# ecmwf-ifs/ectrans

Hardware: AMD Instinct MI355X
Metric: dir+inv transform-pairs/sec, TCo1279 137L x 10 fields; spectral-norm rel-error (higher is better)
Workload: dtype f64

## Files before the change

ectrans_amd/csrc/ectrans_mi.hip:

```cpp
#include <atomic>
#include <chrono>
#include <cmath>
#include <cstdarg>
#include <cstdio>
#include <map>
#include <memory>
#include <string>
#include <vector>

#include <fcntl.h>
#include <sys/mman.h>
#include <sys/stat.h>
#include <unistd.h>

#include "../../include/ectrans_mi.h"
#include "emi_kernels.h"
#include "emi_setup.h"
#include <dlfcn.h>

struct EmiRoctx {
  int (*push)(const char *) = nullptr;
  int (*pop)() = nullptr;
  bool tried = false;
  void load() {
    tried = true;
#ifndef EMI_CPU_EMU
    const char *e = getenv("EMI_ROCTX");
    if (e && atoi(e) == 0) return;
    void *h = dlopen("librocprofiler-sdk-roctx.so", RTLD_NOW | RTLD_GLOBAL);
    if (!h) h = dlopen("librocprofiler-sdk-roctx.so.1", RTLD_NOW | RTLD_GLOBAL);
    if (!h) h = dlopen("libroctx64.so", RTLD_NOW | RTLD_GLOBAL);
    if (!h) return;
    push = (int (*)(const char *))dlsym(h, "roctxRangePushA");
    pop = (int (*)())dlsym(h, "roctxRangePop");
    if (!push || !pop) push = nullptr, pop = nullptr;
#endif
  }
};
static EmiRoctx g_roctx;
struct EmiRange {
  bool on;
  explicit EmiRange(const char *label) {
    if (!g_roctx.tried) g_roctx.load();
    on = g_roctx.push != nullptr;
    if (on) g_roctx.push(label);
  }
  ~EmiRange() {
    if (on) g_roctx.pop();
  }
};
extern "C" int emi_roctx_active(void) {
  if (!g_roctx.tried) g_roctx.load();
  return g_roctx.push != nullptr;
}
static const char *const EMI_LBL_SETUP = "SETUP_TRANS    - Setup ecTrans handle", *const EMI_LBL_SULEG = "SULEG          - Comp. of Leg. poly.",
                         *const EMI_LBL_INV = "INV_TRANS      - Inverse transform", *const EMI_LBL_DIR = "DIR_TRANS      - Direct transform",
                         *const EMI_LBL_LTINV = "LTINV_CTL      - Inv. Legendre transform", *const EMI_LBL_LTDIR = "LTDIR_CTL      - Dir. Legendre transform",
                         *const EMI_LBL_FTDIR = "FTDIR_CTL      - Dir. Fourier transform", *const EMI_LBL_FTINV = "FTINV_CTL      - Inv. Fourier transform",
                         *const EMI_LBL_TRMTOL = "LTINV_CTL      - M to L transposition", *const EMI_LBL_TRLTOM = "LTDIR_CTL      - L to M transposition";

#ifdef EMI_CPU_EMU
thread_local EmuCtx *emu_ctx = nullptr;
#endif

static char g_err[1024] = "";
void emi_set_error(const char *fmt, ...) {
  va_list ap;
  va_start(ap, fmt);
  vsnprintf(g_err, sizeof(g_err), fmt, ap);
  va_end(ap);
}
extern "C" const char *emi_last_error(void) { return g_err; }

#define EMI_FAIL(code, ...)     \
  do {                          \
    emi_set_error(__VA_ARGS__); \
    return (code);              \
  } while (0)

#ifndef EMI_CPU_EMU
static void (*g_oom_hook)() = nullptr;
int emi_dev_malloc(void **p, size_t bytes) {
  if (hipMalloc(p, bytes ? bytes : 16) == hipSuccess) return 0;
  (void)hipGetLastError();
  if (g_oom_hook) g_oom_hook();
  EMI_CHECK(hipMalloc(p, bytes ? bytes : 16));
  return 0;
}
int emi_dev_free(void *p) {
  if (p) EMI_CHECK(hipFree(p));
  return 0;
}
int emi_dev_memset(void *p, int v, size_t bytes, emi_stream_t s) {
  EMI_CHECK(hipMemsetAsync(p, v, bytes, s));
  return 0;
}
int emi_h2d(void *d, const void *s, size_t b, emi_stream_t st) {
  EMI_CHECK(hipMemcpyAsync(d, s, b, hipMemcpyHostToDevice, st));
  return 0;
}
int emi_d2h(void *d, const void *s, size_t b, emi_stream_t st) {
  EMI_CHECK(hipMemcpyAsync(d, s, b, hipMemcpyDeviceToHost, st));
  return 0;
}
int emi_d2d(void *d, const void *s, size_t b, emi_stream_t st) {
  EMI_CHECK(hipMemcpyAsync(d, s, b, hipMemcpyDeviceToDevice, st));
  return 0;
}
int emi_stream_sync(emi_stream_t s) {
  EMI_CHECK(hipStreamSynchronize(s));
  return 0;
}
int emi_mem_info(size_t *f, size_t *t) {
  EMI_CHECK(hipMemGetInfo(f, t));
  return 0;
}
#else
int emi_dev_malloc(void **p, size_t bytes) {
  *p = aligned_alloc(64, ((bytes ? bytes : 16) + 63) / 64 * 64);
  return *p ? 0 : -1;
}
int emi_dev_free(void *p) {
  free(p);
  return 0;
}
int emi_dev_memset(void *p, int v, size_t bytes, emi_stream_t) {
  memset(p, v, bytes);
  return 0;
}
int emi_h2d(void *d, const void *s, size_t b, emi_stream_t) {
  memcpy(d, s, b);
  return 0;
}
int emi_d2h(void *d, const void *s, size_t b, emi_stream_t) {
  memcpy(d, s, b);
  return 0;
}
int emi_d2d(void *d, const void *s, size_t b, emi_stream_t) {
  memmove(d, s, b);
  return 0;
}
int emi_stream_sync(emi_stream_t) { return 0; }
int emi_mem_info(size_t *f, size_t *t) {
  *f = (size_t)8 << 30;
  *t = (size_t)8 << 30;
  return 0;
}
#endif

#include "emi_stage.h"
#ifndef EMI_CPU_EMU
static const bool g_oom_hook_set = (g_oom_hook = emi_stage::trim, true);
#endif

extern "C" int emi_ptr_space(const void *p) {
#ifdef EMI_CPU_EMU
  (void)p;
  return EMI_MEM_HOST;
#else
  if (!p) return EMI_MEM_HOST;
  hipPointerAttribute_t at;
  if (hipPointerGetAttributes(&at, p) != hipSuccess) {
    (void)hipGetLastError();
    return EMI_MEM_HOST;
  }
  return (at.type == hipMemoryTypeDevice || at.type == hipMemoryTypeManaged || at.type == hipMemoryTypeArray) ? EMI_MEM_DEVICE : EMI_MEM_HOST;
#endif
}
static int agree_on_mixed_arrays(const char *who, int ndev, int nhost);
static int resolve_space(const char *who, int mem_space, std::initializer_list<const void *> arrays, int *out, bool collective = false) {
  if (mem_space == EMI_MEM_HOST || mem_space == EMI_MEM_DEVICE) {
    *out = mem_space;
    return 0;
  }
  if (mem_space != EMI_MEM_AUTO) EMI_FAIL(EMI_ERR_ARG, "%s: mem_space = %d (EMI_MEM_HOST, EMI_MEM_DEVICE or EMI_MEM_AUTO)", who, mem_space);
  int ndev = 0, nhost = 0;
  for (const void *q : arrays)
    if (q) (emi_ptr_space(q) == EMI_MEM_DEVICE ? ndev : nhost)++;
  if (collective) {
    if (agree_on_mixed_arrays(who, ndev, nhost)) return EMI_ERR_ARG;
  } else if (ndev && nhost) {
    EMI_FAIL(EMI_ERR_ARG, "%s: %d ARRAYS OF THE CALL ARE IN DEVICE MEMORY AND %d IN HOST MEMORY (all of them must live in one place)", who, ndev, nhost);
  }
  *out = ndev ? EMI_MEM_DEVICE : EMI_MEM_HOST;
  return 0;
}

template <class T>
static int upload(const std::vector<T> &h, T **d) {
  void *p = nullptr;
  if (emi_dev_malloc(&p, h.size() * sizeof(T))) return -1;
  if ((!h.empty() && emi_h2d(p, h.data(), h.size() * sizeof(T), 0)) || emi_stream_sync(0)) {
    emi_dev_free(p);
    return -1;
  }
  *d = (T *)p;
  return 0;
}
struct DevAllocs {
  std::vector<void *> list;
  DevAllocs() = default;
  DevAllocs(const DevAllocs &) = delete;
  DevAllocs &operator=(const DevAllocs &) = delete;
  ~DevAllocs() {
    for (void *p : list) emi_dev_free(p);
  }
  int alloc(void **p, size_t bytes) {
    if (emi_dev_malloc(p, bytes)) return -1;
    list.push_back(*p);
    return 0;
  }
};
template <class T, class F>
static int upload(DevAllocs &owner, const std::vector<T> &h, F *field) {
  T *d = nullptr;
  if (upload(h, &d)) return -1;
  owner.list.push_back(d);
  *field = d;
  return 0;
}

#define EMI_LAUNCH_P(esz, kern, grid, block, lds, st, ...)                     \
  do {                                                                         \
    if ((esz) == 8) {                                                          \
      typedef double RT;                                                       \
      EMI_LAUNCH(emi_f64::kern, grid, block, lds, st, __VA_ARGS__);            \
    } else {                                                                   \
      typedef float RT;                                                        \
      EMI_LAUNCH(emi_f32::kern, grid, block, lds, st, __VA_ARGS__);            \
    }                                                                          \
  } while (0)

struct FftClass {
  int nthr = 0, fbk = 0;
  int hot = 0;
  int r16 = 0;
  int split = 0;
  int mr = 0;
  int gmem = 0;
  long long gm_elems = 0;
  std::vector<int> lats;
  int *d_lats = nullptr;
  FftRowDev *d_rows = nullptr;
  size_t lds = 0;
};
struct LegMaps {
  int2 *d_inv = nullptr, *d_dir = nullptr, *d_inv_wide = nullptr, *d_dir_wide = nullptr;
  long long n_inv = 0, n_dir = 0, n_inv_wide = 0, n_dir_wide = 0;
};

struct Plan {
  Plan() = default;
  Plan(const Plan &) = delete;
  Plan &operator=(const Plan &) = delete;
  ~Plan();
  int nsmax = 0, ndgl = 0, ndgnh = 0;
  bool reduced = false;
  bool ldll = false, shiftll = false;
  bool lam = false;
  int lam_n = 0, kdgux = 0;
  double exwn = 0.0, eywn = 0.0;
  std::vector<int> kntmp;
  std::vector<int> l_kntmp, nesm0;
  LamDev lamdev{};
  int lam_nthr = 0;
  size_t lam_lds = 0;
  double ra = 6371229.0;
  std::vector<int> nloen, nmen, ndglu, procm;
  std::vector<int> latlo;
  std::vector<double> rmu, rw, racthe, cos2;
  int ngptotg = 0, nspec2g = 0;
  int nproc = 1, me = 0;
  int nprv = 1, mev = 0;
  std::vector<int> vlat;
  int vfirst(int w, int v) const { return nprv > 1 ? vlat[(size_t)w * nprv + v] : latlo[w]; }
  int vlast(int w, int v) const { return nprv > 1 ? vlat[(size_t)w * nprv + v + 1] : latlo[w + 1]; }
  long long vpoints(int w, int v) const {
    long long c = 0;
    for (int j = vfirst(w, v); j < vlast(w, v); j++) c += nloen[j];
    return c;
  }
  long long voffset(int v) const {
    long long c = 0;
    for (int j = latlo[me]; j < vfirst(me, v); j++) c += nloen[j];
    return c;
  }
  int nump = 0, nlat = 0, lat0 = 0;
  int ngptot = 0, nspec2 = 0;
  std::vector<int> mval, nasm0;
  std::vector<int> l_nmen, l_gpoff, l_fbase;
  std::vector<int> wbase, wrows, ldp, ldk, lattile_pref, ktile_pref, lbase;
  std::vector<long long> offS, offA, offTS, offTA;
  long long frows = 0, lrows = 0, wrows_total = 0, p_elems = 0, pt_elems = 0;
  std::vector<long long> leg_rows, leg_disp, fft_rows, fft_disp;
  EmiGeomDev g{};
  DevAllocs dev_allocs;
  int esz = 8;
  char *d_P = nullptr, *d_PT = nullptr;
  std::vector<FftPlanDev> fplans;
  std::vector<int> planid;
  FftTabDev ftab{};
  std::vector<FftClass> fclass;
  std::map<int, LegMaps> legmaps;
  char *d_W = nullptr, *d_FBL = nullptr, *d_FBF = nullptr;
  size_t cap_W = 0, cap_FBL = 0, cap_FBF = 0;
  void *d_desc = nullptr;
  size_t cap_desc = 0;
  char *d_fftscr = nullptr;
  size_t cap_fftscr = 0;
#ifndef EMI_CPU_EMU
  hipEvent_t ev_done = nullptr;
#endif
  bool ev_valid = false;
};

Plan::~Plan() {
#ifndef EMI_CPU_EMU
  if (ev_done) (void)hipEventDestroy(ev_done);
#endif
  emi_dev_free(d_W);
  emi_dev_free(d_FBL);
  if (d_FBF != d_FBL) emi_dev_free(d_FBF);
  emi_dev_free(d_desc);
  emi_dev_free(d_fftscr);
}

static int roundup(int a, int b) { return (a + b - 1) / b * b; }
static int test_paths() {
  const char *e = getenv("EMI_TEST_PATHS");
  return e ? atoi(e) : 0;
}
static_assert(LG_LDS_BYTES_DIR + 1024 + 64 <= 65536, "k_leg_dir: stage image + epilogue table above 64 KiB, two workgroups per CU no longer fit");
static size_t leg_dir_lds_bytes(const Plan &P) {
  return (size_t)LG_LDS_BYTES_DIR * P.esz / 8 + 1024 + 64;
}

static int plan_begin(Plan &P, emi_stream_t st) {
#ifndef EMI_CPU_EMU
  if (P.ev_valid) EMI_CHECK(hipStreamWaitEvent(st, P.ev_done, 0));
#else
  (void)P;
  (void)st;
#endif
  return 0;
}
static int plan_end(Plan &P, emi_stream_t st) {
#ifndef EMI_CPU_EMU
  if (!P.ev_done) EMI_CHECK(hipEventCreateWithFlags(&P.ev_done, hipEventDisableTiming));
  EMI_CHECK(hipEventRecord(P.ev_done, st));
  P.ev_valid = true;
#else
  (void)P;
  (void)st;
#endif
  return 0;
}
static const char *emi_rt_errstr(int rc) {
#ifndef EMI_CPU_EMU
  return hipGetErrorString((hipError_t)rc);
#else
  (void)rc;
  return "";
#endif
}
static int plan_quiesce(Plan &P) {
#ifndef EMI_CPU_EMU
  if (P.ev_valid) return (int)hipEventSynchronize(P.ev_done);
#else
  (void)P;
#endif
  return 0;
}

static struct {
  bool init = false;
  int max_resol = 1;
  double ra = 6371229.0;
  int nproc = 1, myproc = 1;
  int nproc_all = 1, myproc_all = 1, nprtrv = 1, mysetv = 1, nprtrv_preset = 0;
  std::vector<std::unique_ptr<Plan>> plans;
  int max_batch = 0;
  int profile = 0;
  emi_alltoallv_fn a2a = nullptr;
  void *a2a_user = nullptr;
  emi_bcast_fn hc_bcast = nullptr;
  emi_allgatherv_fn hc_gather = nullptr;
  void *hc_user = nullptr;
} G;

static Plan *get_plan(int kresol) {
  if (!G.init || kresol < 1 || kresol > (int)G.plans.size()) return nullptr;
  return G.plans[kresol - 1].get();
}

extern "C" int emi_set_nprtrv(int nprtrv) {
  if (G.init) EMI_FAIL(EMI_ERR_STATE, "emi_set_nprtrv: after SETUP_TRANS0");
  if (nprtrv < 1) EMI_FAIL(EMI_ERR_ARG, "emi_set_nprtrv: NPRTRV = %d", nprtrv);
  G.nprtrv_preset = nprtrv;
  return EMI_SUCCESS;
}
extern "C" int emi_init(const emi_init_t *cfg) {
  if (G.init) return EMI_SUCCESS;
  emi_init_t c{};
  if (cfg) c = *cfg;
  G.max_resol = c.kmax_resol > 0 ? c.kmax_resol : 1;
  G.ra = c.prad > 0 ? c.prad : 6371229.0;
  G.nproc_all = c.nproc > 0 ? c.nproc : 1;
  G.myproc_all = c.myproc > 0 ? c.myproc : 1;
  if (G.myproc_all > G.nproc_all) EMI_FAIL(EMI_ERR_ARG, "emi_init: myproc %d > nproc %d", G.myproc_all, G.nproc_all);
  G.nprtrv = c.nprtrv > 0 ? c.nprtrv : (G.nprtrv_preset > 0 ? G.nprtrv_preset : 1);
  if (G.nproc_all % G.nprtrv != 0)
    EMI_FAIL(EMI_ERR_ARG, "SUMP_TRANS0: NPROC INCONSISTENT WITH NPRTRW (NPROC = %d is not a multiple of NPRTRV = %d)", G.nproc_all, G.nprtrv);
  G.nproc = G.nproc_all / G.nprtrv;
  G.myproc = (G.myproc_all - 1) / G.nprtrv + 1;
  G.mysetv = (G.myproc_all - 1) % G.nprtrv + 1;
#ifndef EMI_CPU_EMU
  int ndev = 0;
  if (hipGetDeviceCount(&ndev) != hipSuccess || ndev == 0)
    EMI_FAIL(EMI_ERR_RUNTIME, "emi_init: no HIP device visible -- libectrans_mi has no CPU path");
  if (c.device >= 0) EMI_CHECK(hipSetDevice(c.device));
#endif
  G.plans.clear();
  G.plans.resize(G.max_resol);
  const char *pe = getenv("EMI_PROFILE");
  G.profile = pe ? atoi(pe) : 0;
  const char *mb = getenv("EMI_MAX_BATCH");
  if (mb) G.max_batch = atoi(mb);
  G.init = true;
  return EMI_SUCCESS;
}


static double mr_radix_ops(int R) {
  switch (R) {
    case 2: return 4; case 3: return 14; case 4: return 16; case 5: return 36; case 7: return 66; case 11: return 150;
    case 13: return 204; case 17: return 336; case 19: return 414; case 23: return 594;
    case 6: return 3 * 4 + 2 * 14 + 12; case 8: return 4 * 4 + 2 * 16 + 18; case 9: return 6 * 14 + 24; case 10: return 5 * 4 + 2 * 36 + 24;
    case 12: return 4 * 14 + 3 * 16 + 36; case 14: return 7 * 4 + 2 * 66 + 36; case 15: return 5 * 14 + 3 * 36 + 48; case 16: return 8 * 16 + 54;
    case 18: return 9 * 4 + 2 * 108 + 48; case 20: return 5 * 16 + 4 * 36 + 72; case 21: return 7 * 14 + 3 * 66 + 72;
    default: return -1;
  }
}
static bool mr_choose(int sz, int esz, int fac[3], int &fbk, int &nthr) {
  std::vector<int> rs = {
#define EMI_MR_ROW(r_) r_,
      EMI_MR_RADICES(EMI_MR_ROW)
  };
#ifdef EMI_MR_RADICES_F32
  if (esz == 4)
    for (int r : {EMI_MR_RADICES_F32(EMI_MR_ROW)}) rs.push_back(r);
#endif
#undef EMI_MR_ROW
  double best = 1e300;
  bool found = false;
  auto consider = [&](int A, int B, int C) {
    const int P1 = (B * C) | 1;
    const size_t per_field = (size_t)A * P1 * 2 * esz;
    if (per_field > 160 * 1024 || A * P1 > 65535) return;
    int fb = 16;
    while (fb > 1 && fb * per_field > 40960) fb >>= 1;
    const int R[3] = {A, B, C};
    for (int nt = 128; nt <= 256; nt += 64) {
      double cost = 0;
      for (int ip = 0; ip < 3; ip++) {
        if (R[ip] == 1) continue;
        const long long nb = (long long)fb * (sz / R[ip]);
        const long long sweeps = (nb + nt - 1) / nt;
        cost += (double)(sweeps * nt) / (double)nb * (mr_radix_ops(R[ip]) / R[ip] + 15.0);
      }
      cost *= 1.0 + 0.5 * (256 - nt) / 64.0;
      if (cost < best * (1.0 - 1e-9) || (cost <= best * (1.0 + 1e-9) && nt > nthr)) {
        best = cost, found = true;
        fac[0] = A, fac[1] = B, fac[2] = C, fbk = fb, nthr = nt;
      }
    }
  };
  for (int A : rs) {
    if (sz % A) continue;
    const int m1 = sz / A;
    if (m1 == 1) consider(A, 1, 1);
    for (int B : rs) {
      if (m1 % B) continue;
      const int C = m1 / B;
      if (C == 1) consider(A, B, 1);
      for (int Cc : rs)
        if (Cc == C) consider(A, B, C);
    }
  }
  return found;
}

struct FftSwitches {
  bool mr, r16, r16s, hot;
  static bool off(const char *name) { return getenv(name) && atoi(getenv(name)) == 0; }
  FftSwitches() : mr(!off("EMI_FFT_MR")), r16(!off("EMI_FFT_R16")), r16s(!off("EMI_FFT_R16S")), hot(!getenv("EMI_FFT_NO_HOT")) {}
};
struct HotPlan {
  int pc, S, nfac, fac[5], nfl;
};
static const HotPlan g_hot_plans[] = {
#define EMI_HOT_ROW(pc_, S_, nf_, a_, b_, c_, d_, e_, nfl_) {pc_, S_, nf_, {a_, b_, c_, d_, e_}, nfl_},
    EMI_HOT_PLAN_LIST(EMI_HOT_ROW)
#undef EMI_HOT_ROW
};
#define EMI_LIST_ROW(r_) r_,
static const int g_r16_list[] = {EMI_R16_LIST(EMI_LIST_ROW)}, g_r16s_list[] = {EMI_R16S_LIST(EMI_LIST_ROW)};
#undef EMI_LIST_ROW

static int fft_fields_40k(size_t per_field) {
  int fbk = 16;
  while (fbk > 1 && fbk * per_field > 40960) fbk >>= 1;
  return fbk;
}
static int fft_threads(size_t lds_bytes) { return lds_bytes <= 40960 ? 256 : (lds_bytes <= 81920 ? 512 : 1024); }

struct FftChoice {
  FftPlanDev pl{};
  int nthr = 0;
  int hot = 0;
  bool gmem = false;
};
static int fft_choose(int n, int esz, const FftSwitches &sw, FftChoice &c) {
  FftPlanDev &pl = c.pl;
  pl.n = n;
  pl.cmode = (n % 2 != 0);
  pl.sz = pl.cmode ? n : n / 2;
  std::vector<int> fac;
  pl.blue = !emi::factorize_smooth(pl.sz, fac);
  pl.S = pl.sz;
  int mr_fbk = 0, mr_nthr = 0, mr_fac[3] = {1, 1, 1};
  if (!pl.cmode && pl.sz >= 2 && sw.mr) pl.mr = mr_choose(pl.sz, esz, mr_fac, mr_fbk, mr_nthr) ? 1 : 0;
  if (pl.mr) {
    pl.blue = 0;
    fac.assign(mr_fac, mr_fac + 3);
  }
  if (!pl.mr && !pl.cmode && sw.r16) {
    const int need = 2 * pl.sz - 1;
    if (need > 1536)
      for (int r : g_r16_list)
        if (!pl.r16 && 256 * r >= need) pl.r16 = r;
    if (!pl.r16 && need > 4096 && pl.sz % 2 == 0 && sw.r16s)
      for (int r : g_r16s_list)
        if (!pl.r16 && 256 * r >= pl.sz - 1) pl.r16 = r, pl.split = 2;
    if (pl.r16) pl.blue = 1;
  }
  if (pl.r16) {
    pl.S = 256 * pl.r16;
    fac.assign(1, pl.r16);
  } else if (pl.blue) {
    pl.S = emi::next_235(2 * pl.sz - 1);
    emi::factorize_smooth(pl.S, fac);
    if (!pl.cmode && sw.hot) {
      long long best = (long long)pl.S * (long long)(fac.size() + 1);
      const HotPlan *pick = nullptr;
      for (const HotPlan &r : g_hot_plans) {
        if (r.S < 2 * pl.sz - 1) continue;
        if (fft_fields_40k((size_t)FFT_LDS_ELEMS(r.S) * 2 * esz) < r.nfl) continue;
        const long long cost = (long long)r.S * (r.nfac + 1);
        if (cost <= best) {
          best = cost;
          pick = &r;
        }
      }
      if (pick) {
        pl.S = pick->S;
        fac.assign(pick->fac, pick->fac + pick->nfac);
      }
    }
  }
  if (pl.S > 65535 || fac.size() > 14) EMI_FAIL(EMI_ERR_UNSUPPORTED, "FFT length %d not supported (work size %d)", n, pl.S);
  pl.nfac = (int)fac.size();
  for (int i = 0; i < pl.nfac; i++) pl.fac[i] = fac[i];
  const size_t per_field = (size_t)FFT_LDS_ELEMS(pl.S) * 2 * esz;
  pl.fbk = fft_fields_40k(per_field);
  c.gmem = pl.fbk * per_field > 160 * 1024 && !pl.mr;
  c.nthr = fft_threads(pl.fbk * per_field);
  if (pl.r16) {
    pl.fbk = 1;
    c.nthr = 16 * pl.r16 > 256 ? roundup(16 * pl.r16, 64) : 256;
  } else if (pl.mr) {
    pl.fbk = mr_fbk;
    c.nthr = mr_nthr;
  } else if (pl.blue && !pl.cmode && !c.gmem && sw.hot) {
    int hot_fbk = 0;
    for (const HotPlan &r : g_hot_plans)
      if (r.S == pl.S && r.nfac == pl.nfac && r.nfl <= pl.fbk && std::equal(r.fac, r.fac + r.nfac, pl.fac)) c.hot = r.pc, hot_fbk = r.nfl;
    if (c.hot) {
      pl.fbk = hot_fbk;
      c.nthr = fft_threads(pl.fbk * per_field);
    }
  }
  for (int i = 0; i < pl.nfac; i++)
    if (!c.hot && !pl.r16 && !pl.mr && (pl.fac[i] == 6 || pl.fac[i] > 8)) EMI_FAIL(EMI_ERR_RUNTIME, "internal: composite FFT radix %d without a specialised kernel (length %d)", pl.fac[i], n);
  return 0;
}

struct FftShared {
  int S, tw_off, perm_off, ptw_off[14];
  std::vector<int> fac;
  int r16 = 0, mr = 0;
};
struct FftTabSizes { size_t tw = 0, ptw = 0, perm = 0, rtw = 0, chirp = 0, bhat = 0; };

static void fft_fill_shared(const FftShared &sh, std::vector<d2> &tw, std::vector<d2> &ptw, std::vector<uint16_t> &perm) {
  const int S = sh.S;
  if (sh.mr) {
    const int A = sh.fac[0], B = sh.fac[1], C = sh.fac[2], P1 = (B * C) | 1;
    auto w = [&](long long e) {
      long double a = 2.0L * (long double)M_PIl * (long double)(e % S) / (long double)S;
      return d2{(double)cosl(a), (double)-sinl(a)};
    };
    d2 *t1 = ptw.data() + sh.ptw_off[0], *t2 = ptw.data() + sh.ptw_off[1];
    for (int k1 = 0; k1 < A; k1++) t1[k1] = w((long long)C * k1);
    for (int q = 0; q < A * B; q++) t2[q] = w((long long)q);
    for (int k = 0; k < S; k++) perm[sh.perm_off + k] = (uint16_t)((k % A) * P1 + ((k / A) % B) * C + k / (A * B));
    return;
  }
  if (sh.r16) {
    d2 *dst = ptw.data() + sh.ptw_off[0];
    for (int row = 0; row < 7; row++) {
      const int mult = row < 3 ? row + 1 : 4 * (row - 2);
      for (int t = 0; t < 256; t++) {
        long double a = 2.0L * (long double)M_PIl * (long double)(((long long)t * mult) % S) / (long double)S;
        *dst++ = d2{(double)cosl(a), (double)-sinl(a)};
      }
    }
    return;
  }
  for (int k = 0; k < S; k++) {
    long double a = 2.0L * (long double)M_PIl * (long double)k / (long double)S;
    tw[sh.tw_off + k] = d2{(double)cosl(a), (double)-sinl(a)};
  }
  long long lenp = 1;
  for (size_t ip = 0; ip < sh.fac.size(); ip++) {
    const int R = sh.fac[ip];
    d2 *dst = ptw.data() + sh.ptw_off[ip];
    if (lenp > 1)
      for (int t = 1; t < R; t++)
        for (long long j = 0; j < lenp; j++) {
          long double a = 2.0L * (long double)M_PIl * (long double)((j * t) % (lenp * R)) / (long double)(lenp * R);
          *dst++ = d2{(double)cosl(a), (double)-sinl(a)};
        }
    lenp *= R;
  }
  std::vector<uint16_t> pm;
  emi::dit_positions(S, sh.fac, pm);
  std::copy(pm.begin(), pm.end(), perm.begin() + sh.perm_off);
}

static void fft_fill_length(const FftPlanDev &pl, const std::vector<uint16_t> &perm, std::vector<d2> &rtw, std::vector<d2> &chirp, std::vector<d2> &bhat) {
  const int n = pl.n;
  const double tpi = 2.0 * M_PI;
  for (int k = 0; k <= pl.sz; k++) {
    double a = tpi * (double)k / (double)n;
    rtw[pl.rtw_off + k] = d2{std::cos(a), -std::sin(a)};
  }
  if (!pl.blue) return;
  d2 *c = chirp.data() + pl.chirp_off;
  const int csz = pl.split ? pl.sz / 2 : pl.sz;
  for (int k = 0; k < csz; k++) {
    long long k2 = ((long long)k * k) % (2LL * csz);
    double a = M_PI * (double)k2 / (double)csz;
    c[k] = d2{std::cos(a), -std::sin(a)};
  }
  const int L = pl.S, r0 = pl.fac[0];
  const uint16_t *pm = pl.r16 ? nullptr : perm.data() + pl.perm_off;
  std::vector<long double> cr(L);
  for (int k = 0; k < L; k++) cr[k] = cosl(2.0L * (long double)M_PIl * (long double)k / (long double)L);
  d2 *bh = bhat.data() + pl.bhat_off;
  for (int k = 0; k < L; k++) {
    long double sr = c[0].x, si = -c[0].y;
    long long jk = 0;
    for (int jj = 1; jj < csz; jj++) {
      jk += k;
      if (jk >= L) jk -= L;
      long double cs = 2.0L * cr[jk];
      sr += (long double)c[jj].x * cs;
      si += -(long double)c[jj].y * cs;
    }
    if (pl.r16) {
      const int k0 = k % pl.r16, kk = k / pl.r16, k1 = kk % 16, k2 = kk / 16;
      bh[(size_t)k2 * (16 * pl.r16) + 16 * k0 + k1] = d2{(double)(sr / (long double)L), (double)(si / (long double)L)};
      continue;
    }
    const int p = pm[k];
    bh[(size_t)(p % r0) * (L / r0) + p / r0] = d2{(double)sr, (double)si};
  }
}

static const FftShared &fft_share_tables(const FftPlanDev &pl, std::map<int, int> &sidx, std::vector<FftShared> &shared, FftTabSizes &n) {
  const int skey = pl.S * 16 + (pl.r16 ? 15 : (pl.mr ? 14 : pl.nfac));
  auto si = sidx.find(skey);
  if (si != sidx.end()) return shared[si->second];
  FftShared sh{};
  sh.S = pl.S;
  sh.fac.assign(pl.fac, pl.fac + pl.nfac);
  sh.r16 = pl.r16;
  sh.mr = pl.mr;
  sh.tw_off = (int)n.tw;
  sh.perm_off = (int)n.perm;
  if (pl.mr) {
    const int A = pl.fac[0], B = pl.fac[1];
    sh.ptw_off[0] = (int)n.ptw;
    n.ptw += (size_t)A;
    sh.ptw_off[1] = (int)n.ptw;
    n.ptw += (size_t)A * B;
    sh.ptw_off[2] = (int)n.ptw;
    n.perm += pl.S;
  } else if (pl.r16) {
    sh.ptw_off[0] = (int)n.ptw;
    n.ptw += 7 * 256;
  } else {
    n.tw += pl.S;
    n.perm += pl.S;
    long long lenp = 1;
    for (int ip = 0; ip < pl.nfac; ip++) {
      sh.ptw_off[ip] = (int)n.ptw;
      if (lenp > 1) n.ptw += (size_t)(pl.fac[ip] - 1) * lenp;
      lenp *= pl.fac[ip];
    }
  }
  sidx.emplace(skey, (int)shared.size());
  shared.push_back(sh);
  return shared.back();
}

static int build_fft_plans(Plan &P) {
  const FftSwitches sw;
  std::map<int, int> idx;
  std::map<int, int> sidx;
  std::vector<FftShared> shared;
  FftTabSizes nt;
  P.planid.assign(P.nlat, 0);
  for (int j = 0; j < P.nlat; j++) {
    const int n = P.nloen[P.lat0 + j];
    auto it = idx.find(n);
    if (it != idx.end()) {
      P.planid[j] = it->second;
      continue;
    }
    FftChoice c;
    if (int rc = fft_choose(n, P.esz, sw, c)) return rc;
    FftPlanDev &pl = c.pl;
    const FftShared &sh = fft_share_tables(pl, sidx, shared, nt);
    pl.tw_off = sh.tw_off;
    pl.perm_off = sh.perm_off;
    for (int ip = 0; ip < pl.nfac; ip++) pl.ptw_off[ip] = sh.ptw_off[ip];
    pl.rtw_off = (int)nt.rtw;
    nt.rtw += pl.sz + 1;
    if (pl.blue) {
      pl.chirp_off = (int)nt.chirp;
      nt.chirp += pl.split ? pl.sz / 2 : pl.sz;
      pl.bhat_off = (int)nt.bhat;
      nt.bhat += pl.S;
    }
    if (nt.tw > 0x7fffffffULL || nt.ptw > 0x7fffffffULL || nt.bhat > 0x7fffffffULL) EMI_FAIL(EMI_ERR_UNSUPPORTED, "FFT tables too large");
    int cls = -1;
    for (size_t k = 0; k < P.fclass.size(); k++) {
      const FftClass &fc = P.fclass[k];
      if (fc.nthr == c.nthr && fc.fbk == pl.fbk && fc.hot == c.hot && fc.r16 == pl.r16 && fc.split == pl.split && fc.mr == pl.mr && fc.gmem == (int)c.gmem) cls = (int)k;
    }
    if (cls < 0) {
      cls = (int)P.fclass.size();
      P.fclass.emplace_back();
      FftClass &fc = P.fclass[cls];
      fc.nthr = c.nthr, fc.fbk = pl.fbk, fc.hot = c.hot, fc.r16 = pl.r16, fc.split = pl.split, fc.mr = pl.mr, fc.gmem = c.gmem;
    }
    pl.lds_class = cls;
    idx[n] = P.planid[j] = (int)P.fplans.size();
    P.fplans.push_back(pl);
  }
  if (P.lam) {
    FftPlanDev pl{};
    pl.n = pl.sz = pl.S = P.ndgl;
    pl.cmode = 1;
    std::vector<int> fac;
    pl.blue = !emi::factorize_smooth(pl.sz, fac);
    if (pl.blue) {
      pl.S = emi::next_235(2 * pl.sz - 1);
      emi::factorize_smooth(pl.S, fac);
    }
    const int fs = FFT_LDS_ELEMS(pl.S) + 1, fs_max = 160 * 1024 / (4 * P.esz);
    if (fs > fs_max || pl.S > 65535 || fac.size() > 14)
      EMI_FAIL(EMI_ERR_UNSUPPORTED,
               "ESETUP_TRANS: KDGL = %d NEEDS A WORK ARRAY OF %d COMPLEX NUMBERS PER FIELD (KDGL WHERE IT FACTORISES IN 2, 3, 5, 7, ELSE THE CONVOLUTION LENGTH ABOVE 2 KDGL); THE "
               "Y-DIRECTION KERNELS HOLD TWO FIELDS IN THE 160 KIB OF LDS: AT MOST %d",
               P.ndgl, fs, fs_max);
    pl.nfac = (int)fac.size();
    for (int i = 0; i < pl.nfac; i++) pl.fac[i] = fac[i];
    const size_t per_field = (size_t)fs * 2 * P.esz;
    pl.fbk = std::max(2, std::min(16, (int)(80 * 1024 / per_field) / 2 * 2));
    const FftShared &sh = fft_share_tables(pl, sidx, shared, nt);
    pl.tw_off = sh.tw_off;
    pl.perm_off = sh.perm_off;
    for (int ip = 0; ip < pl.nfac; ip++) pl.ptw_off[ip] = sh.ptw_off[ip];
    pl.rtw_off = (int)nt.rtw;
    nt.rtw += pl.sz + 1;
    if (pl.blue) {
      pl.chirp_off = (int)nt.chirp;
      nt.chirp += pl.sz;
      pl.bhat_off = (int)nt.bhat;
      nt.bhat += pl.S;
    }
    pl.lds_class = -1;
    P.lamdev.yplan = (int)P.fplans.size();
    P.lamdev.fbk = pl.fbk;
    P.lamdev.fs = fs;
    P.lam_lds = (size_t)pl.fbk * per_field;
    P.lam_nthr = std::min(512, fft_threads(P.lam_lds));
    P.fplans.push_back(pl);
  }
  std::vector<d2> tw(nt.tw), rtw(nt.rtw), chirp(nt.chirp), bhat(nt.bhat), ptw(nt.ptw);
  std::vector<uint16_t> perm(nt.perm);
  emi::parallel_for((int)shared.size(), [&](int is) { fft_fill_shared(shared[is], tw, ptw, perm); });
  std::vector<int> order(P.fplans.size());
  for (size_t i = 0; i < order.size(); i++) order[i] = (int)i;
  std::sort(order.begin(), order.end(), [&](int a, int b) { return P.fplans[a].n > P.fplans[b].n; });
  emi::parallel_for((int)order.size(), [&](int io) { fft_fill_length(P.fplans[order[io]], perm, rtw, chirp, bhat); });
  for (int j = 0; j < P.nlat; j++) {
    const FftPlanDev &pl = P.fplans[P.planid[j]];
    FftClass &fc = P.fclass[pl.lds_class];
    fc.lats.push_back(j);
    if (fc.gmem)
      fc.gm_elems = std::max(fc.gm_elems, (long long)pl.fbk * FFT_LDS_ELEMS(pl.S));
    else if (fc.mr)
      fc.lds = std::max(fc.lds, (size_t)pl.fbk * pl.fac[0] * ((pl.fac[1] * pl.fac[2]) | 1) * 2 * P.esz);
    else if (fc.r16)
      fc.lds = (size_t)fc.r16 * 272 * 8 + (size_t)((fc.split ? 128 * fc.r16 : 0) + 240) * 2 * P.esz;
    else
      fc.lds = std::max(fc.lds, (size_t)pl.fbk * FFT_LDS_ELEMS(pl.S) * 2 * P.esz);
  }
  std::vector<d2> tw256(15 * 16);
  for (int k1 = 1; k1 < 16; k1++)
    for (int c = 0; c < 16; c++) {
      long double a = 2.0L * (long double)M_PIl * (long double)(c * k1) / 256.0L;
      tw256[(k1 - 1) * 16 + c] = d2{(double)cosl(a), (double)-sinl(a)};
    }
  auto upload_c = [&](const std::vector<d2> &v, const void **d) {
    if (P.esz == 8) return upload(P.dev_allocs, v, d);
    std::vector<f2> w(v.size());
    for (size_t i = 0; i < v.size(); i++) w[i] = f2{(float)v[i].x, (float)v[i].y};
    return upload(P.dev_allocs, w, d);
  };
  FftTabDev &ft = P.ftab;
  if (upload_c(tw, &ft.tw) || upload_c(ptw, &ft.ptw) || upload_c(rtw, &ft.rtw) || upload_c(chirp, &ft.chirp) || upload_c(bhat, &ft.bhat) || upload_c(tw256, &ft.tw256) ||
      upload(P.dev_allocs, perm, &ft.perm) || upload(P.dev_allocs, P.fplans, &ft.plans) || upload(P.dev_allocs, P.planid, &ft.planid))
    return EMI_ERR_RUNTIME;
  for (FftClass &fc : P.fclass) {
    if (upload(P.dev_allocs, fc.lats, &fc.d_lats)) return EMI_ERR_RUNTIME;
    std::vector<FftRowDev> rows(fc.lats.size());
    for (size_t i = 0; i < fc.lats.size(); i++) {
      const int j = fc.lats[i];
      const FftPlanDev &pl = P.fplans[P.planid[j]];
      FftRowDev &r = rows[i];
      r.lat = j, r.planid = P.planid[j], r.n = pl.n, r.sz = pl.sz;
      r.nmen = P.l_nmen[j], r.fb0 = P.l_fbase[j], r.gpoff = P.l_gpoff[j], r.chirp_off = pl.chirp_off;
      r.rtw_off = pl.rtw_off, r.bhat_off = pl.bhat_off, r.ptw_off0 = pl.ptw_off[0];
      r.mr_abc = pl.mr ? (pl.fac[0] | (pl.fac[1] << 8) | (pl.fac[2] << 16) | (pl.fbk << 24)) : 0;
      r.racthe = P.racthe[P.lat0 + j], r.rw = P.rw[P.lat0 + j];
    }
    if (upload(P.dev_allocs, rows, &fc.d_rows)) return EMI_ERR_RUNTIME;
  }
  return 0;
}


struct LegpolSource {
  const char *base = nullptr;
  size_t len = 0;
  void *map = nullptr;
  size_t maplen = 0;
  std::vector<size_t> offA, offS;
  ~LegpolSource() {
    if (map) munmap(map, maplen);
  }
};

static int legpol_open(LegpolSource &src, const emi_legpol_io_t *io, bool membuf) {
  if (membuf) {
    if (!io->ptr) EMI_FAIL(EMI_ERR_ARG, "SETUP_TRANS: KLEGPOLPTR NULL POINTER");
    if (!io->len) EMI_FAIL(EMI_ERR_ARG, "SETUP_TRANS: KLEGPOLPTR_LEN ARGUMENT MISSING");
    src.base = (const char *)io->ptr;
    src.len = io->len;
    return 0;
  }
  if (!io->fname || !io->fname[0]) EMI_FAIL(EMI_ERR_ARG, "SETUP_TRANS: CDLEGPOLFNAME ARGUMENT MISSING");
  int fd = open(io->fname, O_RDONLY);
  struct stat st;
  if (fd < 0 || fstat(fd, &st) != 0) {
    if (fd >= 0) close(fd);
    EMI_FAIL(EMI_ERR_ARG, "READ_LEGPOL: BYTES_IO_OPEN FAILED (%s)", io->fname);
  }
  src.maplen = (size_t)st.st_size;
  src.map = src.maplen ? mmap(nullptr, src.maplen, PROT_READ, MAP_PRIVATE, fd, 0) : nullptr;
  close(fd);
  if (src.map == MAP_FAILED || !src.map) {
    src.map = nullptr;
    EMI_FAIL(EMI_ERR_ARG, "READ_LEGPOL:BYTES_IO_READ FAILED (%s)", io->fname);
  }
  src.base = (const char *)src.map;
  src.len = src.maplen;
  return 0;
}

static int legpol_index(LegpolSource &src, int nsmax, int ndgnh, const std::vector<int> &nloen, const std::vector<int> &nmen,
                        const std::vector<int> &ndglu) {
  const size_t head = 16 + (size_t)8 * ndgnh;
  if (src.len < 16) EMI_FAIL(EMI_ERR_ARG, "READ_LEGPOL:BYTES_IO_READ FAILED (segment shorter than its header)");
  int ib[4];
  memcpy(ib, src.base, 16);
  if (memcmp(src.base, "LEGPOL  ", 8) != 0) EMI_FAIL(EMI_ERR_ARG, "READ_LEGPOL:WRONG LABEL");
  if (ib[2] != nsmax) EMI_FAIL(EMI_ERR_ARG, "READ_LEGPOL:WRONG SPECTRAL TRUNCATION");
  if (ib[3] != ndgnh) EMI_FAIL(EMI_ERR_ARG, "READ_LEGPOL:WRONG NO OF GAUSSIAN LATITUDES");
  if (src.len < head) EMI_FAIL(EMI_ERR_ARG, "READ_LEGPOL:BYTES_IO_READ FAILED (segment shorter than its latitude table)");
  for (int j = 0; j < ndgnh; j++) {
    int v[2];
    memcpy(v, src.base + 16 + (size_t)8 * j, 8);
    if (v[0] != nloen[j]) EMI_FAIL(EMI_ERR_ARG, "READ_LEGPOL:WRONG NLOEN (latitude %d: %d, file %d)", j + 1, nloen[j], v[0]);
    if (v[1] != nmen[j]) EMI_FAIL(EMI_ERR_ARG, "READ_LEGPOL:WRONG NMEN (latitude %d: %d, file %d)", j + 1, nmen[j], v[1]);
  }
  size_t off = head;
  src.offA.assign(nsmax + 1, 0);
  src.offS.assign(nsmax + 1, 0);
  for (int m = 0; m <= nsmax; m++) {
    const size_t nd = (size_t)std::min(ndgnh, ndglu[m]);
    src.offA[m] = off;
    off += nd * (size_t)((nsmax - m + 2) / 2) * 8;
    src.offS[m] = off;
    off += nd * (size_t)((nsmax - m + 3) / 2) * 8;
  }
  if (off > src.len) EMI_FAIL(EMI_ERR_ARG, "READ_LEGPOL:BYTES_IO_READ FAILED (%zu bytes needed, %zu present)", off, src.len);
  return 0;
}

static int legpol_write(int kresol, const char *fname);

enum LegpolMode { LP_NONE, LP_READF, LP_WRITEF, LP_MEMBUF };
struct SetupTables {
  std::vector<int> ebase, rowm;
  std::vector<double> eps, specw, lapin, l_rw, l_racthe;
  std::vector<int> legN, legS, fftrow;
  bool rowtable = false;
};
struct SetupClock {
  const bool on = getenv("EMI_SETUP_TIMING") && atoi(getenv("EMI_SETUP_TIMING"));
  double t = now();
  static double now() { return std::chrono::duration<double>(std::chrono::steady_clock::now().time_since_epoch()).count(); }
  void phase(const char *what) {
    if (on) fprintf(stderr, "[emi_setup] %-28s %8.3f s\n", what, now() - t);
    t = now();
  }
};

static int setup_arguments(const emi_setup_t *cfg, const emi_legpol_io_t *io, LegpolMode *lp_mode) {
  if (!G.init) EMI_FAIL(EMI_ERR_STATE, "SETUP_TRANS: SETUP_TRANS0 HAS TO BE CALLED BEFORE SETUP_TRANS");
  if (!cfg) EMI_FAIL(EMI_ERR_ARG, "emi_setup: null config");
  if (cfg->kdgl <= 0 || cfg->kdgl % 2 != 0) EMI_FAIL(EMI_ERR_ARG, "SETUP_TRANS: KDGL IS NOT A POSITIVE, EVEN NUMBER");
  if (cfg->lduseflt) EMI_FAIL(EMI_ERR_UNSUPPORTED, "SETUP_TRANS: LDUSEFLT not supported (as gpu/external/setup_trans.F90:442)");
  if (cfg->ldshiftll && !cfg->ldll) EMI_FAIL(EMI_ERR_ARG, "SETUP_TRANS: LDSHIFTLL WITHOUT LDLL");
  if (cfg->ldll) {
    if (!cfg->kloen && cfg->kdlon <= 0) EMI_FAIL(EMI_ERR_ARG, "SETUP_TRANS: LDLL NEEDS KDLON (OR A UNIFORM KLOEN)");
    for (int j = 1; cfg->kloen && j < cfg->kdgl; j++)
      if (cfg->kloen[j] != cfg->kloen[0]) EMI_FAIL(EMI_ERR_ARG, "SETUP_TRANS: LDLL NEEDS ONE ROW LENGTH (KLOEN(%d) = %d, KLOEN(1) = %d)", j + 1, cfg->kloen[j], cfg->kloen[0]);
  }
  if (cfg->ldstretch) EMI_FAIL(EMI_ERR_UNSUPPORTED, "SETUP_TRANS: PSTRET stretching not supported");
  if (cfg->precision != 0 && cfg->precision != 8 && cfg->precision != 4)
    EMI_FAIL(EMI_ERR_ARG, "emi_setup: precision must be 8 (fp64, the _dp library) or 4 (fp32, _sp), got %d", cfg->precision);
  if (cfg->ksmax < 0) EMI_FAIL(EMI_ERR_ARG, "SETUP_TRANS: KSMAX < 0");
  *lp_mode = LP_NONE;
  if (io && io->io && io->io[0]) {
    std::string mode(io->io);
    while (!mode.empty() && mode.back() == ' ') mode.pop_back();
    if (G.nproc_all > 1) EMI_FAIL(EMI_ERR_UNSUPPORTED, "SETUP_TRANS:CDIO_LEGPOL OPTIONS ONLY FOR NPROC=1 ");
    if (cfg->ldll) EMI_FAIL(EMI_ERR_UNSUPPORTED, "SETUP_TRANS: CDIO_LEGPOL is not available with LDLL (the file format describes Gaussian latitudes)");
    if (mode == "readf" || mode == "READF")
      *lp_mode = LP_READF;
    else if (mode == "writef" || mode == "WRITEF")
      *lp_mode = LP_WRITEF;
    else if (mode == "membuf" || mode == "MEMBUF")
      *lp_mode = LP_MEMBUF;
    else
      EMI_FAIL(EMI_ERR_ARG, "SETUP_TRANS:CDIO_LEGPOL UNKNOWN METHOD (%s)", mode.c_str());
    if (*lp_mode != LP_MEMBUF && (!io->fname || !io->fname[0])) EMI_FAIL(EMI_ERR_ARG, "SETUP_TRANS: CDLEGPOLFNAME ARGUMENT MISSING");
  }
  return 0;
}

static int setup_geometry(const emi_setup_t *cfg, Plan &P, std::vector<long long> &cum) {
  const int L = P.ndgl;
  int ndlon = cfg->kdlon > 0 ? cfg->kdlon : 2 * L;
  P.nloen.assign(L, ndlon);
  if (P.ldll) {
    if (cfg->kloen) P.nloen.assign(L, cfg->kloen[0]);
    if (P.nloen[0] <= 0) EMI_FAIL(EMI_ERR_ARG, "SETUP_TRANS: KLOEN INVALID (ONE or MORE POINTS <= 0)");
  } else if (cfg->kloen) {
    ndlon = 0;
    for (int j = 0; j < L; j++) {
      if (cfg->kloen[j] <= 0) EMI_FAIL(EMI_ERR_ARG, "SETUP_TRANS: KLOEN INVALID (ONE or MORE POINTS <= 0)");
      ndlon = std::max(ndlon, cfg->kloen[j]);
    }
    for (int j = 0; j < L; j++) {
      P.nloen[j] = cfg->kloen[j];
      if (cfg->kloen[j] != ndlon) P.reduced = true;
    }
  }
  P.nspec2g = (P.nsmax + 1) * (P.nsmax + 2);
  cum.assign(L + 1, 0);
  for (int j = 0; j < L; j++) cum[j + 1] = cum[j] + P.nloen[j];
  if (cum[L] > 2000000000LL) EMI_FAIL(EMI_ERR_UNSUPPORTED, "grid too large for 32-bit point offsets");
  P.ngptotg = (int)cum[L];
  P.cos2.assign(L, 0.0);
  P.racthe.assign(L, 0.0);
  if (P.ldll) {
    const double pi = 2.0 * std::asin(1.0), eps = 1000.0 * 2.220446049250313e-16;
    P.rmu.assign(L, 0.0);
    P.rw.assign(L, 0.0);
    for (int j = 0; j < L / 2; j++) {
      const double th = P.shiftll ? ((double)j + 0.5) * pi / (double)L : (double)j * pi / (double)(L - 2);
      double mu = std::cos(th), c = std::sin(th);
      if (!P.shiftll && j == 0) mu = 1.0, c = 0.0;
      if (!P.shiftll && j == L / 2 - 1) mu = 0.0, c = 1.0;
      const double ract = c > 0.0 ? 1.0 / c / P.ra : 1.0 / eps / P.ra;
      P.rmu[j] = mu, P.rmu[L - 1 - j] = -mu;
      P.cos2[j] = P.cos2[L - 1 - j] = c * c;
      P.racthe[j] = P.racthe[L - 1 - j] = ract;
    }
  } else {
    emi::gauss_latitudes(L, P.rmu, P.rw);
    for (int j = 0; j < L; j++) {
      double th = std::asin(P.rmu[j]), c = std::cos(th);
      P.cos2[j] = c * c;
      P.racthe[j] = 1.0 / c / P.ra;
    }
  }
  emi::wavenumber_cutoffs(P.nsmax, L, P.nloen, P.reduced, P.cos2, P.nmen, P.ndglu);
  return 0;
}

static int setup_distribution(int N, int L, const std::vector<int> &nloen, const std::vector<long long> &cum, int nprw, int nprv,
                              std::vector<int> &procm, std::vector<int> &latlo, std::vector<int> &vlat) {
  procm.assign(N + 1, 0);
  int ik = 0, ind = 1;
  for (int m = 0; m <= N; m++) {
    ik += ind;
    if (ik > nprw) {
      ik = nprw;
      ind = -1;
    } else if (ik < 1) {
      ik = 1;
      ind = 1;
    }
    procm[m] = ik - 1;
  }
  std::vector<long long> wcum(L + 1, 0);
  for (int j = 0; j < L; j++) {
    const double n = (double)nloen[j];
    const double w = n * (n <= 1500.0 ? 20.0 : std::max(15.0, 20.0 - (n - 1500.0) * 0.00091)) + 1750.0;
    wcum[j + 1] = wcum[j] + (long long)(w + 0.5);
  }
  latlo.assign(nprw + 1, 0);
  for (int r = 1; r < nprw; r++) {
    long long target = wcum[L] * r / nprw;
    int j = (int)(std::lower_bound(wcum.begin(), wcum.end(), target) - wcum.begin());
    j = std::max(j, latlo[r - 1] + 1);
    j = std::min(j, L - (nprw - r));
    latlo[r] = j;
  }
  latlo[nprw] = L;
  if (nprv > 1) {
    vlat.assign((size_t)nprw * nprv + 1, L);
    for (int w = 0; w < nprw; w++) {
      const int a0 = latlo[w], a1 = latlo[w + 1];
      if (a1 - a0 < nprv) EMI_FAIL(EMI_ERR_ARG, "SETUP_TRANS: too many tasks: band %d has %d latitudes for %d V-sets", w + 1, a1 - a0, nprv);
      vlat[(size_t)w * nprv] = a0;
      for (int v = 1; v < nprv; v++) {
        const long long target = cum[a0] + (cum[a1] - cum[a0]) * v / nprv;
        int j = (int)(std::lower_bound(cum.begin() + a0, cum.begin() + a1, target) - cum.begin());
        j = std::max(j, vlat[(size_t)w * nprv + v - 1] + 1);
        j = std::min(j, a1 - (nprv - v));
        vlat[(size_t)w * nprv + v] = j;
      }
    }
  }
  return 0;
}

static void setup_local_tables(Plan &P, const std::vector<long long> &cum, SetupTables &T) {
  const int N = P.nsmax;
  P.lat0 = P.latlo[P.me];
  P.nlat = P.latlo[P.me + 1] - P.lat0;
  P.ngptot = (int)(cum[P.latlo[P.me + 1]] - cum[P.lat0]);
  for (int m = 0; m <= N; m++)
    if (P.procm[m] == P.me) P.mval.push_back(m);
  P.nump = (int)P.mval.size();
  const int NU = P.nump, NL = P.nlat;
  for (auto *v : {&P.nasm0, &P.wrows, &P.ldp, &P.ldk, &T.ebase}) v->assign(NU, 0);
  for (auto *v : {&P.wbase, &P.lbase, &P.lattile_pref, &P.ktile_pref}) v->assign(NU + 1, 0);
  for (auto *v : {&P.offS, &P.offA, &P.offTS, &P.offTA}) v->assign(NU, 0);
  int ipos = 0;
  long long poff = 0, ptoff = 0;
  for (int ml = 0; ml < NU; ml++) {
    const int m = P.mval[ml];
    P.nasm0[ml] = ipos;
    ipos += (N - m + 1) * 2;
    for (int n = m; n <= N; n++) {
      T.specw.push_back(m == 0 ? 1.0 : 2.0);
      T.specw.push_back(m == 0 ? 0.0 : 2.0);
    }
    P.wrows[ml] = roundup(N + 2 - m, P.esz == 4 ? 32 : 16);
    P.wbase[ml + 1] = P.wbase[ml] + P.wrows[ml];
    int nd = std::min(P.ndgnh, P.ndglu[m]);
    P.lbase[ml + 1] = P.lbase[ml] + nd;
    P.ldp[ml] = roundup(std::max(nd, 1), 64);
    long long pan = (long long)(P.wrows[ml] / 2) * P.ldp[ml];
    P.offS[ml] = poff;
    P.offA[ml] = poff + pan;
    poff += 2 * pan;
    P.ldk[ml] = roundup(P.wrows[ml] / 2, 128);
    long long pant = (long long)roundup(std::max(nd, 1), 16) * P.ldk[ml];
    P.offTS[ml] = ptoff;
    P.offTA[ml] = ptoff + pant;
    ptoff += 2 * pant;
    P.lattile_pref[ml + 1] = P.lattile_pref[ml] + (nd + 63) / 64;
    {
      const int nk = P.wrows[ml] / 2, r = nk % 128;
      P.ktile_pref[ml + 1] = P.ktile_pref[ml] + (P.esz == 4 ? (nk + 63) / 64 : 2 * (nk / 128) + (r == 0 ? 0 : r <= 64 ? 1 : 2));
    }
    T.ebase[ml] = (int)T.eps.size();
    for (int n = m; n <= N + 2; n++)
      T.eps.push_back(std::sqrt((double)(n * n - m * m) / (double)(4 * n * n - 1)));
  }
  P.nspec2 = ipos;
  P.p_elems = poff;
  P.pt_elems = P.ldll ? 0 : ptoff;
  P.wrows_total = P.wbase[NU];
  T.rowm.resize(P.wrows_total);
  for (int ml = 0; ml < NU; ml++)
    for (int r = 0; r < P.wrows[ml]; r++) T.rowm[P.wbase[ml] + r] = ml;
  P.l_nmen.assign(NL, 0);
  P.l_gpoff.assign(NL, 0);
  P.l_fbase.assign(NL + 1, 0);
  T.l_rw.resize(NL);
  T.l_racthe.resize(NL);
  for (int jl = 0; jl < NL; jl++) {
    const int j = P.lat0 + jl;
    P.l_nmen[jl] = P.nmen[j];
    P.l_gpoff[jl] = (int)(cum[j] - cum[P.lat0]);
    P.l_fbase[jl + 1] = P.l_fbase[jl] + P.nmen[j] + 1;
    T.l_rw[jl] = P.rw[j];
    T.l_racthe[jl] = P.racthe[j];
  }
  P.frows = P.l_fbase[NL];
  P.lrows = 2LL * P.lbase[NU];
  T.lapin.assign(N + 4, 0.0);
  for (int n = 1; n <= N + 2; n++) T.lapin[n + 1] = -(P.ra * P.ra / (double)(n * (n + 1)));
}

static int setup_row_tables(Plan &P, bool exchange_order, SetupTables &T) {
  const int N = P.nsmax, L = P.ndgl, NP = P.nproc, NU = P.nump, NL = P.nlat;
  std::vector<int> &legN = T.legN, &legS = T.legS, &fftrow = T.fftrow;
  legN.assign(std::max(P.lbase[NU], 1), 0);
  legS.assign(std::max(P.lbase[NU], 1), 0);
  fftrow.assign(P.frows, 0);
  T.rowtable = exchange_order;
// ... 648 lines not shown
        return EMI_ERR_RUNTIME;
      }
      buf.resize((size_t)nr * nc);
      if (emi_inq_legendre(kresol, m, sym, buf.data(), &nr, &nc)) {
        fclose(f);
        return EMI_ERR_RUNTIME;
      }
      ok = fwrite(buf.data(), 8, buf.size(), f) == buf.size();
    }
  ok = (fclose(f) == 0) && ok;
  if (!ok) EMI_FAIL(EMI_ERR_RUNTIME, "WRITE_LEGPOL:BYTES_IO_WRITE FAILED (%s)", fname);
  return EMI_SUCCESS;
}

struct HostStage {
  size_t esz;
  explicit HostStage(int e) : esz((size_t)e) {}
  std::vector<void *> dev;
  bool failed = false;
  std::vector<std::pair<void *, std::pair<void *, size_t>>> outs;
  ~HostStage() {
    for (void *p : dev) emi_stage::release(p);
  }
  const void *in(const void *h, size_t elems, bool host, emi_stream_t s) {
    if (!h || !host) return h;
    void *d = emi_stage::acquire(elems * esz);
    if (!d) {
      failed = true;
      return nullptr;
    }
    dev.push_back(d);
    if (emi_h2d(d, h, elems * esz, s)) failed = true;
    return d;
  }
  void *out(void *h, size_t elems, bool host, bool preload = false, emi_stream_t s = 0) {
    if (!h || !host) return h;
    void *d = emi_stage::acquire(elems * esz);
    if (!d) {
      failed = true;
      return nullptr;
    }
    dev.push_back(d);
    if (preload && emi_h2d(d, h, elems * esz, s)) failed = true;
    outs.push_back({d, {h, elems * esz}});
    return d;
  }
  void flush(emi_stream_t s) {
    for (auto &o : outs) emi_d2h(o.second.first, o.first, o.second.second, s);
    emi_stream_sync(s);
  }
};

static int grow(Plan &P, char **p, size_t *cap, size_t need, const char *what, emi_stream_t st) {
  if (need <= *cap) return 0;
  plan_quiesce(P);
  emi_stream_sync(0);
  emi_dev_free(*p);
  *p = nullptr;
  *cap = 0;
  void *q;
  if (emi_dev_malloc(&q, need)) EMI_FAIL(EMI_ERR_RUNTIME, "cannot allocate %.2f GiB %s", need / 1073741824.0, what);
  *p = (char *)q;
  *cap = need;
  emi_dev_memset(q, 0, need, st);
  return 0;
}

static int ensure_work(Plan &P, int bfpad, int nfb, emi_stream_t st) {
  const size_t rowb = (size_t)2 * bfpad * P.esz;
  if (grow(P, &P.d_W, &P.cap_W, (size_t)P.wrows_total * rowb, "packed-spectral work buffer", st)) return -1;
  if (P.nproc == 1) {
    if (grow(P, &P.d_FBL, &P.cap_FBL, (size_t)nfb * (P.frows + 1) * rowb, "Fourier work buffer", st)) return -1;
    P.d_FBF = P.d_FBL;
    P.cap_FBF = P.cap_FBL;
  } else {
    if (grow(P, &P.d_FBL, &P.cap_FBL, (size_t)nfb * (P.lrows + 1) * rowb, "Fourier (Legendre-side) exchange buffer", st)) return -1;
    if (grow(P, &P.d_FBF, &P.cap_FBF, (size_t)nfb * P.frows * rowb, "Fourier (FFT-side) exchange buffer", st)) return -1;
  }
  return 0;
}

struct PhaseTimer {
  static const int MAXIV = 4096;
  int n = 0, ncreated = 0;
  bool on = false;
  int kinds[MAXIV];
  double xbytes = 0;
  long long fft_kernels = 0;
#ifndef EMI_CPU_EMU
  hipEvent_t e0[MAXIV], e1[MAXIV];
  void begin(bool on_, bool keep = false) {
    on = on_;
    if (!keep) n = 0, xbytes = 0, fft_kernels = 0;
  }
  int start(int kind, emi_stream_t s) {
    if (!on || n >= MAXIV) return -1;
    if (n >= ncreated) {
      (void)hipEventCreate(&e0[n]);
      (void)hipEventCreate(&e1[n]);
      ncreated = n + 1;
    }
    kinds[n] = kind;
    (void)hipEventRecord(e0[n], s);
    return n++;
  }
  void stop(int iv, emi_stream_t s) {
    if (iv >= 0) (void)hipEventRecord(e1[iv], s);
  }
  void resolve(double *ms3, int *launches) {
    for (int i = 0; i < 4; i++) ms3[i] = 0, launches[i] = 0;
    if (!on) return;
    for (int i = 0; i < n; i++) {
      (void)hipEventSynchronize(e1[i]);
      float ms = 0;
      (void)hipEventElapsedTime(&ms, e0[i], e1[i]);
      ms3[kinds[i]] += ms;
      launches[kinds[i]]++;
    }
  }
#else
  void begin(bool, bool = false) {}
  int start(int, emi_stream_t) { return -1; }
  void stop(int, emi_stream_t) {}
  void resolve(double *ms3, int *launches) {
    for (int i = 0; i < 4; i++) ms3[i] = 0, launches[i] = 0;
  }
#endif
};
static PhaseTimer g_pt;

static int hook_alltoallv(const void *sb, const std::vector<long long> &psc, void *rb, const std::vector<long long> &prc, int npeers, int stride, int first,
                          emi_stream_t st) {
  const int NA = G.nproc_all;
  std::vector<long long> sc(NA, 0), sd(NA, 0), rc(NA, 0), rd(NA, 0);
  for (int k = 0; k < npeers; k++) sc[first + k * stride] = psc[k], rc[first + k * stride] = prc[k];
  for (int r = 1; r < NA; r++) sd[r] = sd[r - 1] + sc[r - 1], rd[r] = rd[r - 1] + rc[r - 1];
  const int iv = g_pt.start(3, st);
  for (int r = 0; r < NA; r++)
    if (g_pt.on && r != G.myproc_all - 1) g_pt.xbytes += (double)sc[r];
  const int rc_hook = G.a2a(G.a2a_user, sb, sc.data(), sd.data(), rb, rc.data(), rd.data(), NA, (void *)st);
  g_pt.stop(iv, st);
  if (rc_hook != 0) EMI_FAIL(EMI_ERR_RUNTIME, "all-to-all-v hook failed");
  return 0;
}
static int exchange(Plan &P, bool to_fft, int ldf, emi_stream_t st, char *FBl, char *FBf) {
  if (P.nproc == 1) return 0;
  const int NP = P.nproc;
  std::vector<long long> sc(NP), rc(NP);
  const long long rowb = (long long)ldf * P.esz;
  for (int r = 0; r < NP; r++) {
    const long long lr = P.leg_rows[r] * rowb, fr = P.fft_rows[r] * rowb;
    sc[r] = to_fft ? lr : fr;
    rc[r] = to_fft ? fr : lr;
  }
  const void *sb = to_fft ? FBl : FBf;
  void *rb = to_fft ? FBf : FBl;
  return hook_alltoallv(sb, sc, rb, rc, NP, P.nprv, P.mev, st);
}

static int ensure_desc(Plan &P, size_t bytes);
static int upload_desc(Plan &P, const std::vector<char> &hd, emi_stream_t st) {
  if (ensure_desc(P, hd.size())) return EMI_ERR_RUNTIME;
#ifdef EMI_CPU_EMU
  emi_h2d(P.d_desc, hd.data(), hd.size(), st);
  return 0;
#else
  static struct {
    void *h[4] = {nullptr, nullptr, nullptr, nullptr};
    size_t cap[4] = {0, 0, 0, 0};
    hipEvent_t ev[4];
    bool init[4] = {false, false, false, false};
    unsigned next = 0;
  } ring;
  const int k = (int)(ring.next++ & 3u);
  if (ring.init[k]) {
    EMI_CHECK(hipEventSynchronize(ring.ev[k]));
  } else {
    EMI_CHECK(hipEventCreateWithFlags(&ring.ev[k], hipEventDisableTiming));
    ring.init[k] = true;
  }
  if (ring.cap[k] < hd.size()) {
    if (ring.h[k]) (void)hipHostFree(ring.h[k]);
    ring.h[k] = nullptr;
    ring.cap[k] = 0;
    const size_t cap = std::max(hd.size(), (size_t)1 << 16);
    EMI_CHECK(hipHostMalloc(&ring.h[k], cap, hipHostMallocDefault));
    ring.cap[k] = cap;
  }
  memcpy(ring.h[k], hd.data(), hd.size());
  EMI_CHECK(hipMemcpyAsync(P.d_desc, ring.h[k], hd.size(), hipMemcpyHostToDevice, (hipStream_t)st));
  EMI_CHECK(hipEventRecord(ring.ev[k], (hipStream_t)st));
  return 0;
#endif
}

static int ensure_desc(Plan &P, size_t bytes) {
  if (bytes <= P.cap_desc) return 0;
  plan_quiesce(P);
  emi_stream_sync(0);
  emi_dev_free(P.d_desc);
  P.d_desc = nullptr;
  size_t cap = std::max(bytes, (size_t)1 << 16);
  if (emi_dev_malloc(&P.d_desc, cap)) return EMI_ERR_RUNTIME;
  P.cap_desc = cap;
  return 0;
}

static int build_tilemap(Plan &P, const std::vector<int> &pref, int nct, int2 **d_map, long long *nblocks, int which = 0) {
  const int nx = 8;
  int gx = 1;
  while (gx * 2 <= std::min(nct, nx)) gx *= 2;
  const int gy = nx / gx;
  std::vector<std::vector<int2>> per(8);
  for (int ml = 0; ml < P.nump; ml++) {
    const bool wide = P.esz == 4 && P.mval[ml] == 0;
    if ((which == 1 && wide) || (which == 2 && !wide)) continue;
    const int nrt = pref[ml + 1] - pref[ml];
    for (int x = 0; x < nx; x++) {
      const int xc = (x + ml) % gx, xl = (x / gx + ml) % gy;
      const int c0 = (int)((long long)xc * nct / gx), c1 = (int)((long long)(xc + 1) * nct / gx);
      for (int rt = xl; rt < nrt; rt += gy)
        for (int ct = c0; ct < c1; ct++) per[x].push_back(int2{ml, (rt << 16) | ct});
    }
  }
  size_t mx = 0;
  for (auto &v : per) mx = std::max(mx, v.size());
  std::vector<int2> map(mx * 8, int2{-1, 0});
  for (int x = 0; x < 8; x++)
    for (size_t k = 0; k < per[x].size(); k++) map[k * 8 + x] = per[x][k];
  *nblocks = (long long)map.size();
  if (map.empty()) {
    *d_map = nullptr;
    return 0;
  }
  return upload(P.dev_allocs, map, d_map);
}

static int leg_tilemaps(Plan &P, int nct, LegMaps **out) {
  auto it = P.legmaps.find(nct);
  if (it == P.legmaps.end()) {
    LegMaps lm;
    const bool split = P.esz == 4;
    if (build_tilemap(P, P.lattile_pref, nct, &lm.d_inv, &lm.n_inv, split ? 1 : 0) || build_tilemap(P, P.ktile_pref, nct, &lm.d_dir, &lm.n_dir, split ? 1 : 0) ||
        (split && (build_tilemap(P, P.lattile_pref, nct, &lm.d_inv_wide, &lm.n_inv_wide, 2) || build_tilemap(P, P.ktile_pref, nct, &lm.d_dir_wide, &lm.n_dir_wide, 2))))
      return EMI_ERR_RUNTIME;
    it = P.legmaps.emplace(nct, lm).first;
  }
  *out = &it->second;
  return 0;
}

static int pick_batch(Plan &P, int nfields, int depth) {
  size_t fr = 0, tot = 0;
  emi_mem_info(&fr, &tot);
  size_t have = fr + P.cap_W + P.cap_FBL + (P.nproc > 1 ? P.cap_FBF : 0) + emi_stage::idle_bytes();
  const int nfb = depth > 1 ? 2 : 1;
  double per_field = (double)(P.wrows_total + nfb * P.frows + (P.nproc > 1 ? nfb * P.lrows : 0)) * 2.0 * P.esz;
  long long cap = (long long)((double)have * 0.85 / per_field);
  cap = cap / 64 * 64;
  if (cap < 64) cap = 64;
  if (G.max_batch > 0) cap = std::min<long long>(cap, std::max(64, roundup(G.max_batch, 64)));
  long long want = roundup((nfields + depth - 1) / depth, 64);
  return (int)std::min(cap, std::max(64LL, want));
}


static int launch_fft(Plan &P, bool inverse, bool adj, const GridFld *d_flds, int nfld, char *FB, int ldf, int nproma,
                       emi_stream_t st) {
  for (size_t c = 0; c < P.fclass.size(); c++) {
    FftClass &fc = P.fclass[c];
    if (fc.lats.empty() || nfld <= 0) continue;
    const int nchunk = (nfld + fc.fbk - 1) / fc.fbk;
    const long long nblocks = (long long)fc.lats.size() * nchunk;
    FftLaunchDev lc{fc.d_lats, (int)fc.lats.size(), nchunk, nblocks, adj ? 1 : 0, fc.d_rows};
    const int nthr = fc.nthr;
    if (g_pt.on) g_pt.fft_kernels++;
    if (fc.gmem) {
      const size_t needb = (size_t)nblocks * fc.gm_elems * 2 * P.esz;
      if (needb > P.cap_fftscr) {
        plan_quiesce(P);
        emi_stream_sync(0);
        emi_dev_free(P.d_fftscr);
        P.d_fftscr = nullptr;
        P.cap_fftscr = 0;
        void *q = nullptr;
        if (emi_dev_malloc(&q, needb)) EMI_FAIL(EMI_ERR_RUNTIME, "cannot allocate %.2f GiB of FFT scratch for the rows that exceed the LDS", needb / 1073741824.0);
        P.d_fftscr = (char *)q;
        P.cap_fftscr = needb;
      }
      if (inverse) {
        if (P.esz == 8)
          EMI_LAUNCH(emi_f64::k_fft_inv_gm, nblocks, nthr, 0, st, P.g, P.ftab, lc, d_flds, nfld, (const double *)FB, ldf, nproma, (d2 *)P.d_fftscr, fc.gm_elems);
        else
          EMI_LAUNCH(emi_f32::k_fft_inv_gm, nblocks, nthr, 0, st, P.g, P.ftab, lc, d_flds, nfld, (const float *)FB, ldf, nproma, (f2 *)P.d_fftscr, fc.gm_elems);
      } else {
        if (P.esz == 8)
          EMI_LAUNCH(emi_f64::k_fft_dir_gm, nblocks, nthr, 0, st, P.g, P.ftab, lc, d_flds, nfld, (double *)FB, ldf, nproma, (d2 *)P.d_fftscr, fc.gm_elems);
        else
          EMI_LAUNCH(emi_f32::k_fft_dir_gm, nblocks, nthr, 0, st, P.g, P.ftab, lc, d_flds, nfld, (float *)FB, ldf, nproma, (f2 *)P.d_fftscr, fc.gm_elems);
      }
      continue;
    }
    if (fc.mr) {
      if (inverse)
        EMI_LAUNCH_P(P.esz, k_fft_inv_mr, nblocks, nthr, fc.lds, st, P.g, P.ftab, lc, d_flds, nfld, (const RT *)FB, ldf, nproma);
      else
        EMI_LAUNCH_P(P.esz, k_fft_dir_mr, nblocks, nthr, fc.lds, st, P.g, P.ftab, lc, d_flds, nfld, (RT *)FB, ldf, nproma);
      continue;
    }
    if (fc.r16 && fc.split) {
      switch (fc.r16) {
#define EMI_R16P_LAUNCH(r_)                                                                                                                 \
  case r_:                                                                                                                                  \
    if (inverse)                                                                                                                            \
      EMI_LAUNCH_P(P.esz, k_fft_inv_r16p<r_>, nblocks, nthr, fc.lds, st, P.g, P.ftab, lc, d_flds, nfld, (const RT *)FB, ldf, nproma);      \
    else                                                                                                                                    \
      EMI_LAUNCH_P(P.esz, k_fft_dir_r16p<r_>, nblocks, nthr, fc.lds, st, P.g, P.ftab, lc, d_flds, nfld, (RT *)FB, ldf, nproma);            \
    break;
        EMI_R16S_LIST(EMI_R16P_LAUNCH)
#undef EMI_R16P_LAUNCH
        default: EMI_FAIL(EMI_ERR_RUNTIME, "internal: no k_fft_*_r16p kernel for R1 = %d", fc.r16);
      }
      continue;
    }
    if (fc.r16) {
      switch (fc.r16) {
#define EMI_R16_LAUNCH(r_)                                                                                                                  \
  case r_:                                                                                                                                  \
    if (inverse)                                                                                                                            \
      EMI_LAUNCH_P(P.esz, k_fft_inv_r16<r_>, nblocks, nthr, fc.lds, st, P.g, P.ftab, lc, d_flds, nfld, (const RT *)FB, ldf, nproma);       \
    else                                                                                                                                    \
      EMI_LAUNCH_P(P.esz, k_fft_dir_r16<r_>, nblocks, nthr, fc.lds, st, P.g, P.ftab, lc, d_flds, nfld, (RT *)FB, ldf, nproma);             \
    break;
        EMI_R16_LIST(EMI_R16_LAUNCH)
#undef EMI_R16_LAUNCH
        default: EMI_FAIL(EMI_ERR_RUNTIME, "internal: no k_fft_*_r16 kernel for R1 = %d", fc.r16);
      }
      continue;
    }
    switch (fc.hot) {
#define EMI_HOT_LAUNCH(pc_, S_, nf_, a_, b_, c_, d_, e_, nfl_)                                                                                       \
  case pc_:                                                                                                                                    \
    if (inverse)                                                                                                                               \
      EMI_LAUNCH_P(P.esz, k_fft_inv_hot<pc_>, nblocks, nthr, fc.lds, st, P.g, P.ftab, lc, d_flds, nfld, (const RT *)FB, ldf, nproma);         \
    else                                                                                                                                       \
      EMI_LAUNCH_P(P.esz, k_fft_dir_hot<pc_>, nblocks, nthr, fc.lds, st, P.g, P.ftab, lc, d_flds, nfld, (RT *)FB, ldf, nproma);               \
    break;
      EMI_HOT_PLAN_LIST(EMI_HOT_LAUNCH)
#undef EMI_HOT_LAUNCH
      default:
        if (inverse)
          EMI_LAUNCH_P(P.esz, k_fft_inv, nblocks, nthr, fc.lds, st, P.g, P.ftab, lc, d_flds, nfld, (const RT *)FB, ldf, nproma);
        else
          EMI_LAUNCH_P(P.esz, k_fft_dir, nblocks, nthr, fc.lds, st, P.g, P.ftab, lc, d_flds, nfld, (RT *)FB, ldf, nproma);
    }
  }
  return 0;
}

struct Pipeline {
#ifndef EMI_CPU_EMU
  hipStream_t sA = nullptr, sB = nullptr, sX = nullptr;
  std::vector<hipEvent_t> ev;
  hipEvent_t fork = nullptr, joinA = nullptr, joinB = nullptr, joinX = nullptr;
  int init() {
    if (sA) return 0;
    EMI_CHECK(hipStreamCreateWithFlags(&sA, hipStreamNonBlocking));
    EMI_CHECK(hipStreamCreateWithFlags(&sB, hipStreamNonBlocking));
    EMI_CHECK(hipStreamCreateWithFlags(&sX, hipStreamNonBlocking));
    EMI_CHECK(hipEventCreateWithFlags(&fork, hipEventDisableTiming));
    EMI_CHECK(hipEventCreateWithFlags(&joinA, hipEventDisableTiming));
    EMI_CHECK(hipEventCreateWithFlags(&joinB, hipEventDisableTiming));
    EMI_CHECK(hipEventCreateWithFlags(&joinX, hipEventDisableTiming));
    return 0;
  }
  hipEvent_t event(size_t i) {
    while (ev.size() <= i) {
      hipEvent_t e;
      (void)hipEventCreateWithFlags(&e, hipEventDisableTiming);
      ev.push_back(e);
    }
    return ev[i];
  }
  void begin(emi_stream_t user) {
    (void)hipEventRecord(fork, user);
    (void)hipStreamWaitEvent(sA, fork, 0);
    (void)hipStreamWaitEvent(sB, fork, 0);
    (void)hipStreamWaitEvent(sX, fork, 0);
  }
  void end(emi_stream_t user) {
    (void)hipEventRecord(joinA, sA);
    (void)hipEventRecord(joinB, sB);
    (void)hipEventRecord(joinX, sX);
    (void)hipStreamWaitEvent(user, joinA, 0);
    (void)hipStreamWaitEvent(user, joinB, 0);
    (void)hipStreamWaitEvent(user, joinX, 0);
  }
  void signal(size_t i, emi_stream_t s) { (void)hipEventRecord(event(i), s); }
  void wait(size_t i, emi_stream_t s) { (void)hipStreamWaitEvent(s, event(i), 0); }
#else
  void *sA = nullptr, *sB = nullptr, *sX = nullptr;
  int init() { return 0; }
  void begin(emi_stream_t) {}
  void end(emi_stream_t) {}
  void signal(size_t, emi_stream_t) {}
  void wait(size_t, emi_stream_t) {}
#endif
};
static Pipeline g_pipe;

static int pipeline_depth(const Plan &P, int nfields) {
  const int cfg = (test_paths() & 2) ? 4 : 1;
#ifdef EMI_CPU_EMU
  (void)P;
  (void)nfields;
  return 1;
#else
  if (nfields < 256) return 1;
  if (P.nproc > 1) {
    static int dcfg = -1;
    if (dcfg < 0) {
      const char *e = getenv("EMI_PIPELINE_DIST");
      dcfg = e ? atoi(e) : 4;
      if (dcfg < 1) dcfg = 1;
    }
    return dcfg;
  }
  return cfg;
#endif
}

#ifndef EMI_CPU_EMU
static int set_lds_attrs() {
  static bool done = false;
  if (done) return 0;
  EMI_CHECK(hipFuncSetAttribute((const void *)emi_f64::k_leg_dir, hipFuncAttributeMaxDynamicSharedMemorySize, 80 * 1024));
  EMI_CHECK(hipFuncSetAttribute((const void *)emi_f32::k_leg_dir, hipFuncAttributeMaxDynamicSharedMemorySize, 80 * 1024));
#define EMI_HOT_ATTR(pc_, S_, nf_, a_, b_, c_, d_, e_, nfl_)                                                                                  \
  EMI_CHECK(hipFuncSetAttribute((const void *)emi_f64::k_fft_inv_hot<pc_>, hipFuncAttributeMaxDynamicSharedMemorySize, 160 * 1024));  \
  EMI_CHECK(hipFuncSetAttribute((const void *)emi_f64::k_fft_dir_hot<pc_>, hipFuncAttributeMaxDynamicSharedMemorySize, 160 * 1024));  \
  EMI_CHECK(hipFuncSetAttribute((const void *)emi_f32::k_fft_inv_hot<pc_>, hipFuncAttributeMaxDynamicSharedMemorySize, 160 * 1024));  \
  EMI_CHECK(hipFuncSetAttribute((const void *)emi_f32::k_fft_dir_hot<pc_>, hipFuncAttributeMaxDynamicSharedMemorySize, 160 * 1024));
  EMI_HOT_PLAN_LIST(EMI_HOT_ATTR)
#undef EMI_HOT_ATTR
  EMI_CHECK(hipFuncSetAttribute((const void *)emi_f64::k_lam_inv, hipFuncAttributeMaxDynamicSharedMemorySize, 160 * 1024));
  EMI_CHECK(hipFuncSetAttribute((const void *)emi_f64::k_lam_dir, hipFuncAttributeMaxDynamicSharedMemorySize, 160 * 1024));
  EMI_CHECK(hipFuncSetAttribute((const void *)emi_f32::k_lam_inv, hipFuncAttributeMaxDynamicSharedMemorySize, 160 * 1024));
  EMI_CHECK(hipFuncSetAttribute((const void *)emi_f32::k_lam_dir, hipFuncAttributeMaxDynamicSharedMemorySize, 160 * 1024));
  EMI_CHECK(hipFuncSetAttribute((const void *)emi_f64::k_fft_inv, hipFuncAttributeMaxDynamicSharedMemorySize, 160 * 1024));
  EMI_CHECK(hipFuncSetAttribute((const void *)emi_f64::k_fft_dir, hipFuncAttributeMaxDynamicSharedMemorySize, 160 * 1024));
  EMI_CHECK(hipFuncSetAttribute((const void *)emi_f32::k_fft_inv, hipFuncAttributeMaxDynamicSharedMemorySize, 160 * 1024));
  EMI_CHECK(hipFuncSetAttribute((const void *)emi_f32::k_fft_dir, hipFuncAttributeMaxDynamicSharedMemorySize, 160 * 1024));
  EMI_CHECK(hipFuncSetAttribute((const void *)emi_f64::k_fft_inv_mr, hipFuncAttributeMaxDynamicSharedMemorySize, 160 * 1024));
  EMI_CHECK(hipFuncSetAttribute((const void *)emi_f64::k_fft_dir_mr, hipFuncAttributeMaxDynamicSharedMemorySize, 160 * 1024));
  EMI_CHECK(hipFuncSetAttribute((const void *)emi_f32::k_fft_inv_mr, hipFuncAttributeMaxDynamicSharedMemorySize, 160 * 1024));
  EMI_CHECK(hipFuncSetAttribute((const void *)emi_f32::k_fft_dir_mr, hipFuncAttributeMaxDynamicSharedMemorySize, 160 * 1024));
#define EMI_R16_ATTR(r_)                                                                                                                     \
  EMI_CHECK(hipFuncSetAttribute((const void *)emi_f64::k_fft_inv_r16<r_>, hipFuncAttributeMaxDynamicSharedMemorySize, 160 * 1024));  \
  EMI_CHECK(hipFuncSetAttribute((const void *)emi_f64::k_fft_dir_r16<r_>, hipFuncAttributeMaxDynamicSharedMemorySize, 160 * 1024));  \
  EMI_CHECK(hipFuncSetAttribute((const void *)emi_f32::k_fft_inv_r16<r_>, hipFuncAttributeMaxDynamicSharedMemorySize, 160 * 1024));  \
  EMI_CHECK(hipFuncSetAttribute((const void *)emi_f32::k_fft_dir_r16<r_>, hipFuncAttributeMaxDynamicSharedMemorySize, 160 * 1024));
  EMI_R16_LIST(EMI_R16_ATTR)
#undef EMI_R16_ATTR
#define EMI_R16P_ATTR(r_)                                                                                                                    \
  EMI_CHECK(hipFuncSetAttribute((const void *)emi_f64::k_fft_inv_r16p<r_>, hipFuncAttributeMaxDynamicSharedMemorySize, 160 * 1024)); \
  EMI_CHECK(hipFuncSetAttribute((const void *)emi_f64::k_fft_dir_r16p<r_>, hipFuncAttributeMaxDynamicSharedMemorySize, 160 * 1024)); \
  EMI_CHECK(hipFuncSetAttribute((const void *)emi_f32::k_fft_inv_r16p<r_>, hipFuncAttributeMaxDynamicSharedMemorySize, 160 * 1024)); \
  EMI_CHECK(hipFuncSetAttribute((const void *)emi_f32::k_fft_dir_r16p<r_>, hipFuncAttributeMaxDynamicSharedMemorySize, 160 * 1024));
  EMI_R16S_LIST(EMI_R16P_ATTR)
#undef EMI_R16P_ATTR
  done = true;
  return 0;
}
#else
static int set_lds_attrs() { return 0; }
#endif

struct ScalarRef {
  int arr;
  int lev, var;
};

template <class ARGS>
static int enumerate_scalars(const ARGS &a, const char *who, std::vector<ScalarRef> &sc) {
  sc.clear();
  if (a.spscalar) {
    if (a.spsc3a || a.spsc3b || a.spsc2) EMI_FAIL(EMI_ERR_ARG, "%s : PSPSCALAR AND PSPSC3A/PSPSC3B/PSPSC2 BOTH PRESENT", who);
    for (int i = 0; i < a.nf_scalar; i++) sc.push_back({0, i, 0});
  } else {
    if (a.spsc2)
      for (int i = 0; i < a.nf_sc2; i++) sc.push_back({1, i, 0});
    if (a.spsc3a)
      for (int v = 0; v < a.sc3a_nvar; v++)
        for (int l = 0; l < a.sc3a_nlev; l++) sc.push_back({2, l, v});
    if (a.spsc3b)
      for (int v = 0; v < a.sc3b_nvar; v++)
        for (int l = 0; l < a.sc3b_nlev; l++) sc.push_back({3, l, v});
  }
  return 0;
}

template <class ARGS>
static int check_extents(const char *who, const ARGS &a, int nspec2, int nproma, int ngpblks, int nuv, int nvar_uv, int dmul,
                         int *uv_dim3) {
  *uv_dim3 = nvar_uv;
  const emi_extents_t *e = a.ext;
  if (!e) return 0;
  if (e->sp_dim2 > 0 && e->sp_dim2 < nspec2)
    EMI_FAIL(EMI_ERR_ARG, "%s : SECOND DIMENSION OF A SPECTRAL ARRAY TOO SMALL (%d < NSPEC2 = %d)", who, e->sp_dim2, nspec2);
  auto lead = [&](const char *nm, int d1) {
    if (d1 < nproma) {
      emi_set_error("%s:FIRST DIMENSION OF %s TOO SMALL (%d < %d)", who, nm, d1, nproma);
      return -1;
    }
    if (d1 != nproma) {
      emi_set_error("%s: first extent of %s is %d, NPROMA is %d: pass a packed copy at the C-ABI (the Fortran shim does)", who, nm, d1, nproma);
      return -1;
    }
    return 0;
  };
  if (a.gp) {
    if (lead("PGP", e->gp[0])) return EMI_ERR_ARG;
    if (e->gp[1] != a.gp_nfld) EMI_FAIL(EMI_ERR_ARG, "%s: gp_nfld (%d) is not the second extent of PGP (%d)", who, a.gp_nfld, e->gp[1]);
    if (e->gp[2] < ngpblks) EMI_FAIL(EMI_ERR_ARG, "%s:THIRD DIMENSION OF PGP TOO SMALL (%d < %d)", who, e->gp[2], ngpblks);
  }
  if (a.gpuv) {
    if (lead("PGPUV", e->gpuv[0])) return EMI_ERR_ARG;
    if (e->gpuv[1] != a.nf_uv) EMI_FAIL(EMI_ERR_ARG, "%s:SEC. DIMENSION OF PGPUV INCONSISTENT (%d, IF_UV_G = %d)", who, e->gpuv[1], a.nf_uv);
    if (e->gpuv[2] < nvar_uv) EMI_FAIL(EMI_ERR_ARG, "%s:THIRD DIMENSION OF PGPUV TOO SMALL (%d < %d)", who, e->gpuv[2], nvar_uv);
    if (e->gpuv[3] < ngpblks) EMI_FAIL(EMI_ERR_ARG, "%s:FOURTH DIMENSION OF PGPUV TOO SMALL (%d < %d)", who, e->gpuv[3], ngpblks);
    *uv_dim3 = e->gpuv[2];
    (void)nuv;
  }
  if (a.gp2 && a.nf_sc2 > 0) {
    if (lead("PGP2", e->gp2[0])) return EMI_ERR_ARG;
    if (e->gp2[1] != a.nf_sc2 * dmul) EMI_FAIL(EMI_ERR_ARG, "%s:SEC. DIMENSION OF PGP2 INCONSISTENT (%d, IF_SC2_G = %d)", who, e->gp2[1], a.nf_sc2 * dmul);
    if (e->gp2[2] < ngpblks) EMI_FAIL(EMI_ERR_ARG, "%s:THIRD DIMENSION OF PGP2 TOO SMALL (%d < %d)", who, e->gp2[2], ngpblks);
  }
  if (a.gp3a && a.sc3a_nlev * a.sc3a_nvar > 0) {
    if (lead("PGP3A", e->gp3a[0])) return EMI_ERR_ARG;
    if (e->gp3a[1] != a.sc3a_nlev) EMI_FAIL(EMI_ERR_ARG, "%s:SEC. DIMENSION OF PGP3A INCONSISTENT (%d, IF_SC3A_G2 = %d)", who, e->gp3a[1], a.sc3a_nlev);
    if (e->gp3a[2] != a.sc3a_nvar * dmul)
      EMI_FAIL(EMI_ERR_ARG, "%s:THIRD DIMENSION OF PGP3A INCONSISTENT (%d, IF_SC3A_G3 = %d)", who, e->gp3a[2], a.sc3a_nvar * dmul);
    if (e->gp3a[3] < ngpblks) EMI_FAIL(EMI_ERR_ARG, "%s:FOURTH DIMENSION OF PGP3A TOO SMALL (%d < %d)", who, e->gp3a[3], ngpblks);
  }
  if (a.gp3b && a.sc3b_nlev * a.sc3b_nvar > 0) {
    if (lead("PGP3B", e->gp3b[0])) return EMI_ERR_ARG;
    if (e->gp3b[1] != a.sc3b_nlev) EMI_FAIL(EMI_ERR_ARG, "%s:SEC. DIMENSION OF PGP3B INCONSISTENT (%d, IF_SC3B_G2 = %d)", who, e->gp3b[1], a.sc3b_nlev);
    if (e->gp3b[2] != a.sc3b_nvar * dmul)
      EMI_FAIL(EMI_ERR_ARG, "%s:THIRD DIMENSION OF PGP3B INCONSISTENT (%d, IF_SC3B_G3 = %d)", who, e->gp3b[2], a.sc3b_nvar * dmul);
    if (e->gp3b[3] < ngpblks) EMI_FAIL(EMI_ERR_ARG, "%s:FOURTH DIMENSION OF PGP3B TOO SMALL (%d < %d)", who, e->gp3b[3], ngpblks);
  }
  return 0;
}

struct Call {
  int mem_space;
  emi_stream_t stream;
  const emi_extents_t *ext;
  const emi_vsets_t *vsets;
  int kproma;
  void *spvor, *spdiv, *spscalar, *spsc3a, *spsc3b, *spsc2;
  int nf_uv, nf_scalar, sc3a_nlev, sc3a_nvar, sc3b_nlev, sc3b_nvar, nf_sc2;
  void *gp, *gpuv, *gp3a, *gp3b, *gp2;
  int gp_nfld;
  int ldscders, ldvorgp, lddivgp, lduvder;
  int ldlatlon;
  void *meanu, *meanv;
};
template <class A>
static Call to_call(const A &a) {
  Call c{a.mem_space, (emi_stream_t)a.stream, a.ext, a.vsets, a.kproma,
         (void *)a.spvor, (void *)a.spdiv, (void *)a.spscalar, (void *)a.spsc3a, (void *)a.spsc3b, (void *)a.spsc2,
         a.nf_uv, a.nf_scalar, a.sc3a_nlev, a.sc3a_nvar, a.sc3b_nlev, a.sc3b_nvar, a.nf_sc2,
         (void *)a.gp, (void *)a.gpuv, (void *)a.gp3a, (void *)a.gp3b, (void *)a.gp2, a.gp_nfld, 0, 0, 0, 0, 0, nullptr, nullptr};
  if constexpr (std::is_same<A, emi_invtrans_t>::value)
    c.ldscders = a.ldscders, c.ldvorgp = a.ldvorgp, c.lddivgp = a.lddivgp, c.lduvder = a.lduvder, c.ldlatlon = a.ldlatlon;
  return c;
}

struct VGroups {
  int nuv_g = 0;
  std::vector<int> ouv;
  std::vector<ScalarRef> sc_g;
  std::vector<int> osc;
  int nsc_g[4] = {0, 0, 0, 0};
  int nvar3a = 0, nvar3b = 0;
};

struct Fields {
  int nuv = 0;
  std::vector<ScalarRef> sc;
  int nf2 = 0, nlev3a = 0, nvar3a = 0, nlev3b = 0, nvar3b = 0;
  bool scders = false, vorgp = false, divgp = false, uvder = false;
  int nvar_uv = 2, dmul = 1, if_gp = 0;
};
static int account(const Call &c, const char *who, bool inverse, const VGroups *vg, Fields &f) {
  int need[4];
  if (vg) {
    f.nuv = vg->nuv_g, f.sc = vg->sc_g;
    f.nf2 = vg->nsc_g[1], f.nlev3a = vg->nsc_g[2], f.nvar3a = vg->nvar3a, f.nlev3b = vg->nsc_g[3], f.nvar3b = vg->nvar3b;
    need[0] = vg->nsc_g[0], need[1] = f.nf2, need[2] = f.nlev3a * f.nvar3a, need[3] = f.nlev3b * f.nvar3b;
  } else {
    f.nuv = (c.spvor || c.spdiv) ? c.nf_uv : 0;
    if (inverse && f.nuv > 0 && !c.spvor) EMI_FAIL(EMI_ERR_ARG, "%s : IF_UV > 0 BUT PSPVOR MISSING", who);
    if (inverse && f.nuv > 0 && !c.spdiv) EMI_FAIL(EMI_ERR_ARG, "%s : IF_UV > 0 BUT PSPDIV MISSING", who);
    if (!inverse && f.nuv > 0 && (!c.spvor || !c.spdiv)) EMI_FAIL(EMI_ERR_ARG, "%s : IF_UV > 0 BUT PSPVOR OR PSPDIV MISSING", who);
    if (enumerate_scalars(c, who, f.sc)) return EMI_ERR_ARG;
    f.nf2 = c.nf_sc2, f.nlev3a = c.sc3a_nlev, f.nvar3a = c.sc3a_nvar, f.nlev3b = c.sc3b_nlev, f.nvar3b = c.sc3b_nvar;
    need[0] = c.spscalar ? (int)f.sc.size() : 0, need[1] = c.spsc2 ? f.nf2 : 0;
    need[2] = c.spsc3a ? f.nlev3a * f.nvar3a : 0, need[3] = c.spsc3b ? f.nlev3b * f.nvar3b : 0;
  }
  const int nuv = f.nuv, nsc = (int)f.sc.size();
  f.scders = c.ldscders && nsc > 0;
  f.vorgp = c.ldvorgp && nuv > 0;
  f.divgp = (c.lddivgp || c.ldvorgp) && nuv > 0;
  f.uvder = c.lduvder && nuv > 0;
  f.nvar_uv = 2 + (f.vorgp ? 1 : 0) + (f.divgp ? 1 : 0) + (f.uvder ? 2 : 0);
  f.dmul = f.scders ? 3 : 1;
  f.if_gp = nuv * f.nvar_uv + nsc * f.dmul;
  if (vg && f.if_gp == 0) return 0;
  if (c.gp) {
    if (c.gpuv || c.gp3a || c.gp3b || c.gp2) EMI_FAIL(EMI_ERR_ARG, "%s:PGP AND PGPUV/PGP3A/PGP3B/PGP2 CAN NOT BOTH BE PRESENT", who);
    if (c.gp_nfld < f.if_gp) EMI_FAIL(EMI_ERR_ARG, "%s:SECOND DIMENSION OF PGP TOO SMALL (%d < %d)", who, c.gp_nfld, f.if_gp);
  } else {
    if (nuv > 0 && !c.gpuv) EMI_FAIL(EMI_ERR_ARG, "%s:PGPUV MISSING", who);
    if (need[0] > 0) EMI_FAIL(EMI_ERR_ARG, "%s:PGP MISSING (PSPSCALAR needs PGP)", who);
    if (need[1] > 0 && !c.gp2) EMI_FAIL(EMI_ERR_ARG, "%s:PGP2 MISSING", who);
    if (need[2] > 0 && !c.gp3a) EMI_FAIL(EMI_ERR_ARG, "%s:PGP3A MISSING", who);
    if (need[3] > 0 && !c.gp3b) EMI_FAIL(EMI_ERR_ARG, "%s:PGP3B MISSING", who);
  }
  return 0;
}

enum { GF_VOR, GF_DIV, GF_U, GF_V, GF_SC, GF_NSD, GF_UEW, GF_VEW, GF_SCEW, GF_N };
static bool gf_uv(int grp) { return grp != GF_SC && grp != GF_NSD && grp != GF_SCEW; }
struct GridRef {
  GridFld g;
  int grp, i;
};
static void grid_fields(const Fields &f, const Call &d, int uv_dim3, std::vector<GridRef> &out) {
  out.clear();
  const int nuv = f.nuv;
  int uvvar = 0;
  auto add = [&](int grp, int i, int mode, void *base, int nf_arr, int fidx) {
    GridFld g{};
    if (d.gp) base = d.gp, nf_arr = d.gp_nfld, fidx = (int)out.size();
    g.base = base, g.nf_arr = nf_arr, g.fidx = fidx, g.mode = mode;
    out.push_back({g, grp, i});
  };
  auto uv = [&](int grp, int mode) {
    for (int i = 0; i < nuv; i++) add(grp, i, mode, d.gpuv, nuv * uv_dim3, uvvar * nuv + i);
    uvvar++;
  };
  auto sc = [&](int grp, int kder, int mode) {
    for (int i = 0; i < (int)f.sc.size(); i++) {
      const ScalarRef &r = f.sc[i];
      if (r.arr == 1) add(grp, i, mode, d.gp2, f.nf2 * f.dmul, r.lev + kder * f.nf2);
      else if (r.arr == 2) add(grp, i, mode, d.gp3a, f.nlev3a * f.nvar3a * f.dmul, (r.var + kder * f.nvar3a) * f.nlev3a + r.lev);
      else add(grp, i, mode, d.gp3b, f.nlev3b * f.nvar3b * f.dmul, (r.var + kder * f.nvar3b) * f.nlev3b + r.lev);
    }
  };
  if (f.vorgp) uv(GF_VOR, GM_PLAIN);
  if (f.divgp) uv(GF_DIV, GM_PLAIN);
  uv(GF_U, GM_ACOS);
  uv(GF_V, GM_ACOS);
  sc(GF_SC, 0, GM_PLAIN);
  if (f.scders) sc(GF_NSD, 1, GM_ACOS);
  if (f.uvder) uv(GF_UEW, GM_EWDER_UV), uv(GF_VEW, GM_EWDER_UV);
  if (f.scders) sc(GF_SCEW, 2, GM_EWDER);
}

static int stage(const Plan &P, HostStage &hs, const Call &c, const char *who, bool inverse, bool uv_sp, const Fields &f, size_t gsz, bool gpad,
                 int uv_dim3, Call &d) {
  const bool host = c.mem_space == EMI_MEM_HOST;
  const emi_stream_t st = c.stream;
  const size_t ns2 = P.nspec2;
  auto sp = [&](void *h, size_t nf, bool on) { return inverse ? (void *)hs.in(h, ns2 * nf, on, st) : hs.out(h, ns2 * nf, on, false, st); };
  auto gr = [&](void *h, size_t nf, bool on, bool pre) { return inverse ? hs.out(h, gsz * nf, on, pre, st) : (void *)hs.in(h, gsz * nf, on, st); };
  d = c;
  d.mem_space = EMI_MEM_DEVICE;
  d.spvor = sp(c.spvor, c.nf_uv, uv_sp), d.spdiv = sp(c.spdiv, c.nf_uv, uv_sp);
  d.spscalar = sp(c.spscalar, c.nf_scalar, host), d.spsc2 = sp(c.spsc2, c.nf_sc2, host);
  d.spsc3a = sp(c.spsc3a, (size_t)c.sc3a_nlev * c.sc3a_nvar, host), d.spsc3b = sp(c.spsc3b, (size_t)c.sc3b_nlev * c.sc3b_nvar, host);
  d.gp = gr(c.gp, c.gp_nfld, host, gpad || c.gp_nfld > f.if_gp);
  d.gpuv = gr(c.gpuv, (size_t)f.nuv * uv_dim3, host && f.nuv, gpad || uv_dim3 > f.nvar_uv);
  d.gp2 = gr(c.gp2, (size_t)f.nf2 * f.dmul, host, gpad);
  d.gp3a = gr(c.gp3a, (size_t)f.nlev3a * f.nvar3a * f.dmul, host, gpad);
  d.gp3b = gr(c.gp3b, (size_t)f.nlev3b * f.nvar3b * f.dmul, host, gpad);
  if (hs.failed) EMI_FAIL(EMI_ERR_RUNTIME, "%s: cannot stage the host arrays through device memory (%s)", who, emi_last_error());
  return 0;
}

struct Batch {
  int ldw = 0, ntiles = 0;
  size_t off_g = 0, off_s = 0, off_f = 0;
  int ng = 0, ns = 0;
  LegMaps *maps = nullptr;
};
template <class T>
static size_t append_desc(std::vector<char> &hdesc, const T *p, size_t n) {
  const size_t off = hdesc.size();
  hdesc.resize(off + (n * sizeof(T) + 255) / 256 * 256);
  if (n) memcpy(hdesc.data() + off, p, n * sizeof(T));
  return off;
}

template <class First, class Last>
static int run_batches(Plan &P, emi_stream_t st, bool inverse, bool piped, int bfpad, std::vector<Batch> &bats, const std::vector<char> &hdesc,
                       First first, Last last) {
  if (ensure_work(P, bfpad, piped ? 2 : 1, st)) return EMI_ERR_RUNTIME;
  for (Batch &bt : bats)
    if (!P.lam && leg_tilemaps(P, bt.ntiles, &bt.maps)) return EMI_ERR_RUNTIME;
  if (upload_desc(P, hdesc, st)) return EMI_ERR_RUNTIME;
  emi_stream_t sA = st, sB = st, sX = st;
  if (piped) {
    if (g_pipe.init()) return EMI_ERR_RUNTIME;
    sA = (emi_stream_t)g_pipe.sA;
    sB = (emi_stream_t)g_pipe.sB;
    sX = (emi_stream_t)g_pipe.sX;
    g_pipe.begin(st);
  }
  g_pt.begin(G.profile != 0, G.profile == 2);
  const emi_stream_t s1 = inverse ? sA : sB, s2 = inverse ? sB : sA;
  const bool dist = P.nproc > 1;
  const int ldw_max = 2 * bfpad;
  const size_t lstride = (size_t)((dist ? P.lrows : P.frows) + 1) * ldw_max * P.esz, fstride = (size_t)P.frows * ldw_max * P.esz;
  int rc = EMI_SUCCESS;
  for (int ib = 0; ib < (int)bats.size(); ib++) {
    const Batch &bt = bats[ib];
    char *FBl = P.d_FBL + (piped ? (size_t)(ib & 1) * lstride : 0);
    char *FBf = dist ? P.d_FBF + (piped ? (size_t)(ib & 1) * fstride : 0) : FBl;
    if (piped && ib >= 2) g_pipe.wait(3 * (ib - 2) + (dist ? 2 : 1), s1);
    if (first(bt, s1, FBl, FBf)) {
      rc = EMI_ERR_RUNTIME;
      break;
    }
    if (piped) g_pipe.signal(3 * ib, s1);
    if (dist) {
      if (piped) g_pipe.wait(3 * ib, sX);
      if (piped && ib >= 2) g_pipe.wait(3 * (ib - 2) + 1, sX);
      EmiRange rg(inverse ? EMI_LBL_TRMTOL : EMI_LBL_TRLTOM);
      if (exchange(P, inverse, bt.ldw, sX, FBl, FBf)) {
        rc = EMI_ERR_RUNTIME;
        break;
      }
      if (piped) g_pipe.signal(3 * ib + 2, sX);
    }
    if (piped) g_pipe.wait(3 * ib + (dist ? 2 : 0), s2);
    auto done = [&] {
      if (piped) g_pipe.signal(3 * ib + 1, s2);
    };
    if (last(bt, s2, FBl, FBf, done)) {
      rc = EMI_ERR_RUNTIME;
      break;
    }
  }
  if (piped) g_pipe.end(st);
  return rc;
// ... 1089 lines not shown
```

ectrans_amd/csrc/emi_mr_body.h:

```cpp

#if defined(EMI_MR_STAMP) && !defined(EMI_LEG_STAMP) && !defined(EMI_CPU_EMU)
#define MR_STAMP_BEGIN()                  \
  unsigned long long st_acc[10] = {0};    \
  unsigned long long st_prev = __builtin_readcyclecounter()
#define MR_STAMP(i_)                                                  \
  do {                                                                \
    const unsigned long long st_now = __builtin_readcyclecounter();   \
    st_acc[i_] += st_now - st_prev;                                   \
    st_prev = st_now;                                                 \
  } while (0)
#define MR_STAMP_END()                                                                \
  do {                                                                                \
    if (EMI_TID == 0) {                                                               \
      for (int i_ = 0; i_ < 10; i_++) atomicAdd(&emi_mr_stamp[i_ < 7 ? i_ : i_ + 1], st_acc[i_]); \
      atomicAdd(&emi_mr_stamp[7], 1ull);                                              \
    }                                                                                 \
  } while (0)
#else
#define MR_STAMP_BEGIN() ((void)0)
#define MR_STAMP(i_) ((void)0)
#define MR_STAMP_END() ((void)0)
#endif

template <int I, int N, class F>
EMI_DEVFN void mr_for(F &&f) {
  if constexpr (I < N) {
    f(std::integral_constant<int, I>{});
    mr_for<I + 1, N>(f);
  }
}

template <int R, int T>
EMI_DEVFN void mr_mulw(real_t &xr, real_t &xi) {
  constexpr int t = ((T % R) + R) % R;
  if constexpr (t == 0) {
  } else if constexpr (4 * t == R) {
    const real_t a = xr;
    xr = xi, xi = -a;
  } else if constexpr (2 * t == R) {
    xr = -xr, xi = -xi;
  } else if constexpr (4 * t == 3 * R) {
    const real_t a = xr;
    xr = -xi, xi = a;
  } else if constexpr (8 * t == R) {
    constexpr real_t h = (real_t)0.70710678118654752440;
    const real_t a = (xr + xi) * h;
    xi = (xi - xr) * h, xr = a;
  } else if constexpr (8 * t == 3 * R) {
    constexpr real_t h = (real_t)0.70710678118654752440;
    const real_t a = (xi - xr) * h;
    xi = -(xr + xi) * h, xr = a;
  } else if constexpr (8 * t == 5 * R) {
    constexpr real_t h = (real_t)0.70710678118654752440;
    const real_t a = -(xr + xi) * h;
    xi = (xr - xi) * h, xr = a;
  } else if constexpr (8 * t == 7 * R) {
    constexpr real_t h = (real_t)0.70710678118654752440;
    const real_t a = (xr - xi) * h;
    xi = (xr + xi) * h, xr = a;
  } else {
    constexpr real_t c = (real_t)mr_cos<R>(t), s = (real_t)mr_sin<R>(t);
    const real_t a = xr * c + xi * s;
    xi = xi * c - xr * s, xr = a;
  }
}

EMI_DEVFN constexpr int mr_split_a(int R) {
  return R == 6 ? 2 : R == 8 ? 2 : R == 9 ? 3 : R == 10 ? 2 : R == 12 ? 3 : R == 14 ? 2 : R == 15 ? 3 : R == 16 ? 4 : R == 18 ? 2 : R == 20 ? 4 : R == 21 ? 3 : 0;
}

template <int R>
struct MrDft {
  template <class Emit>
  static EMI_DEVFN void run(const real_t *xr, const real_t *xi, Emit &&emit) {
    constexpr int SA = mr_split_a(R);
    if constexpr (R == 1) {
      emit(std::integral_constant<int, 0>{}, xr[0], xi[0]);
    } else if constexpr (R == 2) {
      emit(std::integral_constant<int, 0>{}, xr[0] + xr[1], xi[0] + xi[1]);
      emit(std::integral_constant<int, 1>{}, xr[0] - xr[1], xi[0] - xi[1]);
    } else if constexpr (R == 4) {
      const real_t ar = xr[0] + xr[2], ai = xi[0] + xi[2], br = xr[0] - xr[2], bi = xi[0] - xi[2];
      const real_t cr = xr[1] + xr[3], ci = xi[1] + xi[3], dr = xr[1] - xr[3], di = xi[1] - xi[3];
      emit(std::integral_constant<int, 0>{}, ar + cr, ai + ci);
      emit(std::integral_constant<int, 1>{}, br + di, bi - dr);
      emit(std::integral_constant<int, 2>{}, ar - cr, ai - ci);
      emit(std::integral_constant<int, 3>{}, br - di, bi + dr);
    } else if constexpr (SA == 0) {
      constexpr int M = (R - 1) / 2;
      real_t sr[M], si[M], dr[M], di[M];
      real_t y0r = xr[0], y0i = xi[0];
      mr_for<0, M>([&](auto jc) {
        constexpr int j = decltype(jc)::value;
        sr[j] = xr[j + 1] + xr[R - 1 - j], si[j] = xi[j + 1] + xi[R - 1 - j];
        dr[j] = xr[j + 1] - xr[R - 1 - j], di[j] = xi[j + 1] - xi[R - 1 - j];
        y0r += sr[j], y0i += si[j];
      });
      emit(std::integral_constant<int, 0>{}, y0r, y0i);
      mr_for<1, M + 1>([&](auto kc) {
        constexpr int k = decltype(kc)::value;
        real_t ar = xr[0], ai = xi[0], br = 0, bi = 0;
        mr_for<0, M>([&](auto jc) {
          constexpr int j = decltype(jc)::value;
          constexpr int t = ((j + 1) * k) % R;
          constexpr real_t c = (real_t)mr_cos<R>(t), s = (real_t)mr_sin<R>(t);
          ar += c * sr[j], ai += c * si[j];
          if constexpr (j == 0)
            br = s * dr[j], bi = s * di[j];
          else
            br += s * dr[j], bi += s * di[j];
        });
        emit(std::integral_constant<int, k>{}, ar + bi, ai - br);
        emit(std::integral_constant<int, R - k>{}, ar - bi, ai + br);
      });
    } else {
      constexpr int SB = R / SA;
      real_t tr[R], ti[R];
      mr_for<0, SB>([&](auto nbc) {
        constexpr int nb = decltype(nbc)::value;
        real_t ir[SA], ii[SA];
        mr_for<0, SA>([&](auto nac) {
          constexpr int na = decltype(nac)::value;
          ir[na] = xr[na * SB + nb], ii[na] = xi[na * SB + nb];
        });
        MrDft<SA>::run(ir, ii, [&](auto kac, real_t re, real_t im) {
          constexpr int ka = decltype(kac)::value;
          mr_mulw<R, nb * ka>(re, im);
          tr[nb * SA + ka] = re, ti[nb * SA + ka] = im;
        });
      });
      mr_for<0, SA>([&](auto kac) {
        constexpr int ka = decltype(kac)::value;
        real_t ir[SB], ii[SB];
        mr_for<0, SB>([&](auto nbc) {
          constexpr int nb = decltype(nbc)::value;
          ir[nb] = tr[nb * SA + ka], ii[nb] = ti[nb * SA + ka];
        });
        MrDft<SB>::run(ir, ii, [&](auto kbc, real_t re, real_t im) {
          constexpr int kb = decltype(kbc)::value;
          emit(std::integral_constant<int, ka + SA * kb>{}, re, im);
        });
      });
    }
  }
};

EMI_DEVFN unsigned mr_magic(unsigned D) { return D > 1 ? 0xFFFFFFFFu / D + 1u : 0u; }
EMI_DEVFN unsigned mr_div(unsigned j, unsigned m) { return m ? (unsigned)(((unsigned long long)j * m) >> 32) : j; }

struct MrPassArgs {
  int cnt;
  unsigned mcnt, mD;
  int D, SU, SV, ES;
  const real2 *tw;
  int tw_by_u;
};

EMI_DEVFN real_t *mr_row(const GridFld &gf, long long blk0, unsigned rem0, int nproma) {
  return (real_t *)gf.base + (blk0 * gf.nf_arr + gf.fidx) * (long long)nproma + rem0;
}
EMI_DEVFN bool mr_row_flat(const GridFld &gf, long long blk0, unsigned rem0, int nproma, int n) {
  return (rem0 + (unsigned)n <= (unsigned)nproma) && ((((uintptr_t)mr_row(gf, blk0, rem0, nproma)) & (2 * sizeof(real_t) - 1)) == 0);
}

template <int R, int IO>
EMI_DEVFN void mr_pass(real2 *a, int fs, int nfl, const MrPassArgs &pa, const GridFld *flds, long long blk0, unsigned rem0, int nproma) {
  const int ntot = nfl * pa.cnt;
  for (int gi = EMI_TID; gi < ntot; gi += EMI_NTHREADS) {
    const int f = nfl > 1 ? (int)mr_div((unsigned)gi, pa.mcnt) : 0;
    const int j = gi - f * pa.cnt;
    const int u = pa.D > 1 ? (int)mr_div((unsigned)j, pa.mD) : j;
    const int v = j - u * pa.D;
    real2 *p = a + (long long)f * fs + u * pa.SU + v * pa.SV;
    real_t xr[R], xi[R];
    real2 w = mk2(1, 0);
    if (IO != 1 && pa.tw) {
      EMI_GLOBAL_AS const real2 *tw = (EMI_GLOBAL_AS const real2 *)pa.tw + (pa.tw_by_u ? u : j);
      w = mk2(tw->x, tw->y);
    }
    EMI_GLOBAL_AS real2 *row = nullptr;
    if constexpr (IO != 0) row = (EMI_GLOBAL_AS real2 *)mr_row(flds[f], blk0, rem0, nproma) + j;
    if constexpr (IO == 1) {
      mr_for<0, R>([&](auto rc) {
        constexpr int r = decltype(rc)::value;
        xr[r] = row[pa.cnt * r].x, xi[r] = row[pa.cnt * r].y;
      });
    } else {
      mr_for<0, R>([&](auto rc) {
        constexpr int r = decltype(rc)::value;
        const real2 z = p[r * pa.ES];
        xr[r] = z.x, xi[r] = z.y;
      });
    }
    if (IO != 1 && pa.tw) {
      if constexpr (sizeof(real_t) == 4 && (R > 8)) {
        real_t qr[4], qi[4];
        qr[1] = w.x, qi[1] = w.y;
        mr_for<1, R>([&](auto rc) {
          constexpr int r = decltype(rc)::value;
          if constexpr (r == 2) {
            qr[2] = w.x * w.x - w.y * w.y, qi[2] = 2 * w.x * w.y;
          } else if constexpr (r == 3) {
            qr[3] = qr[2] * w.x - qi[2] * w.y, qi[3] = qr[2] * w.y + qi[2] * w.x;
          } else if constexpr (r == 4) {
            qr[0] = qr[2] * qr[2] - qi[2] * qi[2], qi[0] = 2 * qr[2] * qi[2];
            w = mk2(qr[0], qi[0]);
          } else if constexpr (r > 4) {
            const real_t t0 = qr[r & 3] * w.x - qi[r & 3] * w.y;
            qi[r & 3] = qr[r & 3] * w.y + qi[r & 3] * w.x, qr[r & 3] = t0;
          }
          const real_t t1 = xr[r] * qr[r & 3] - xi[r] * qi[r & 3];
          xi[r] = xr[r] * qi[r & 3] + xi[r] * qr[r & 3], xr[r] = t1;
        });
      } else {
        real_t cr = w.x, ci = w.y;
        mr_for<1, R>([&](auto rc) {
          constexpr int r = decltype(rc)::value;
          if constexpr (r > 1) {
            const real_t t0 = cr * w.x - ci * w.y;
            ci = cr * w.y + ci * w.x, cr = t0;
          }
          const real_t t1 = xr[r] * cr - xi[r] * ci;
          xi[r] = xr[r] * ci + xi[r] * cr, xr[r] = t1;
        });
      }
    }
    MrDft<R>::run(xr, xi, [&](auto kc, real_t re, real_t im) {
      constexpr int k = decltype(kc)::value;
      if constexpr (IO == 2)
        row[pa.cnt * k].x = re, row[pa.cnt * k].y = -im;
      else
        p[k * pa.ES] = mk2(re, im);
    });
  }
}

template <int IO>
EMI_DEVFN void mr_pass_any(int R, real2 *a, int fs, int nfl, const MrPassArgs &pa, const GridFld *flds, long long blk0, unsigned rem0, int nproma) {
  switch (R) {
#define EMI_MR_CASE(r_) \
  case r_: mr_pass<r_, IO>(a, fs, nfl, pa, flds, blk0, rem0, nproma); break;
    EMI_MR_RADICES(EMI_MR_CASE)
    EMI_MR_EXTRA(EMI_MR_CASE)
#undef EMI_MR_CASE
    default: break;
  }
}

struct MrGeom {
  int A, B, C, P1, fs;
};
EMI_DEVFN MrGeom mr_geom(int abc) {
  MrGeom m;
  m.A = abc & 255, m.B = (abc >> 8) & 255, m.C = (abc >> 16) & 255;
  const int bc = m.B * m.C;
  m.P1 = bc | 1;
  m.fs = m.A * m.P1;
  return m;
}
EMI_DEVFN MrPassArgs mr_args(const MrGeom &m, int ip, const real2 *tw1, const real2 *tw2) {
  MrPassArgs pa;
  if (ip == 0) {
    pa.cnt = m.B * m.C, pa.D = 1, pa.SU = 1, pa.SV = 0, pa.ES = m.P1, pa.tw = nullptr, pa.tw_by_u = 0;
  } else if (ip == 1) {
    pa.cnt = m.A * m.C, pa.D = m.C, pa.SU = m.P1, pa.SV = 1, pa.ES = m.C, pa.tw = tw1, pa.tw_by_u = 1;
  } else {
    pa.cnt = m.A * m.B, pa.D = m.A, pa.SU = m.C, pa.SV = m.P1, pa.ES = 1, pa.tw = tw2, pa.tw_by_u = 0;
  }
  pa.mcnt = mr_magic((unsigned)pa.cnt);
  pa.mD = mr_magic((unsigned)pa.D);
  return pa;
}

EMI_KERNEL_MR(4) void k_fft_dir_mr(EmiGeomDev g, FftTabDev T, FftLaunchDev Lc, const GridFld *flds, int nfld, real_t *FB, int ldf,
                                                  int nproma) {
  EMI_LDS_DECL;
  real2 *a = (real2 *)EMI_LDS_PTR;
  const int bid = (int)xcd_swizzle(EMI_BID, Lc.nblocks, 8);
  const int li = bid / Lc.nchunk;
  const FftRowDev rw_ = Lc.rows[li];
  const FftPlanDev &pl = T.plans[rw_.planid];
  const int fbk = (int)((unsigned)rw_.mr_abc >> 24);
  const int f0 = (bid - li * Lc.nchunk) * fbk;
  const int nfl = (nfld - f0) < fbk ? (nfld - f0) : fbk;
  const int n = rw_.n, sz = rw_.sz, nmen = rw_.nmen;
  const MrGeom m = mr_geom(rw_.mr_abc);
  const int fb0 = rw_.fb0;
  const int *frow = g.fftrow ? g.fftrow + fb0 : nullptr;
  const real2 *rtw = (const real2 *)T.rtw + rw_.rtw_off;
  const real2 *tw1 = (const real2 *)T.ptw + rw_.ptw_off0, *tw2 = tw1 + m.A;
  const long long gp0 = rw_.gpoff;
  const long long blk0 = gp0 / nproma;
  const unsigned rem0 = (unsigned)(gp0 - blk0 * nproma);
  bool flat = true;
  for (int fl = 0; fl < nfl; fl++) flat = flat && mr_row_flat(flds[f0 + fl], blk0, rem0, nproma, n);
  MR_STAMP_BEGIN();
  if (flat) {
    mr_pass_any<1>(m.A, a, m.fs, nfl, mr_args(m, 0, tw1, tw2), flds + f0, blk0, rem0, nproma);
    MR_STAMP(0);
  } else {
    const int bc = m.B * m.C, pad = m.P1 - bc;
    const unsigned mbc = mr_magic((unsigned)bc);
    for (int fl = 0; fl < nfl; fl++) {
      const GridRow gr = grid_row(flds[f0 + fl], gp0, nproma);
      real2 *af = a + (long long)fl * m.fs;
      for (int l = EMI_TID; l < sz; l += EMI_NTHREADS) {
        real2 z;
        if (grid_pair_ok(gr, 2u * l)) {
          z = *(const real2 *)grid_ptr(gr, 2u * l);
        } else {
          z.x = *grid_ptr(gr, 2u * l);
          z.y = *grid_ptr(gr, 2u * l + 1);
        }
        af[l + (pad && bc > 1 ? (int)mr_div((unsigned)l, mbc) * pad : 0)] = z;
      }
    }
    EMI_SYNC();
    mr_pass_any<0>(m.A, a, m.fs, nfl, mr_args(m, 0, tw1, tw2), flds + f0, blk0, rem0, nproma);
  }
  if (m.B > 1) {
    EMI_SYNC();
    MR_STAMP(1);
    mr_pass_any<0>(m.B, a, m.fs, nfl, mr_args(m, 1, tw1, tw2), flds + f0, blk0, rem0, nproma);
    MR_STAMP(2);
  }
  if (m.C > 1) {
    EMI_SYNC();
    MR_STAMP(3);
    mr_pass_any<0>(m.C, a, m.fs, nfl, mr_args(m, 2, tw1, tw2), flds + f0, blk0, rem0, nproma);
    MR_STAMP(4);
  }
  EMI_SYNC();
  MR_STAMP(5);
  {
    const int nk = nmen + 1, ntot = nfl * nk, NT = EMI_NTHREADS;
    const unsigned mnf = mr_magic((unsigned)nfl), mA = mr_magic((unsigned)m.A), mAB = mr_magic((unsigned)(m.A * m.B));
    const real_t sc0 = (real_t)0.5 * (Lc.adj ? (real_t)1.0 : (real_t)(rw_.rw / (double)n)), racthe = (real_t)rw_.racthe;
    auto pos = [&](int k) {
      const int q1 = m.A > 1 ? (int)mr_div((unsigned)k, mA) : k;
      const int k3 = (int)mr_div((unsigned)k, mAB);
      return (k - q1 * m.A) * m.P1 + (q1 - k3 * m.B) * m.C + k3;
    };
    for (int g0 = EMI_TID; g0 < ntot; g0 += 4 * NT) {
      real2 za[4], zb[4], w4[4];
      int kk[4], ff[4];
      real_t sc[4];
#pragma unroll
      for (int e = 0; e < 4; e++) {
        const int gi = g0 + e * NT;
        if (gi < ntot) {
          const int k = nfl > 1 ? (int)mr_div((unsigned)gi, mnf) : gi, fl = gi - k * nfl;
          const real2 *af = a + (long long)fl * m.fs;
          kk[e] = k, ff[e] = fl;
          w4[e] = rtw[k];
          sc[e] = sc0 * fft_dir_mode_scale(flds[f0 + fl].mode, racthe);
          za[e] = af[pos(k)], zb[e] = af[pos(k == 0 ? 0 : sz - k)];
        }
      }
#if defined(EMI_MR_STAMP) && !defined(EMI_LEG_STAMP) && !defined(EMI_CPU_EMU)
      if (w4[0].x + za[0].x + zb[0].x + sc[0] == (real_t)1.2345e300) kk[0] = 0;
      MR_STAMP(7);
#endif
#pragma unroll
      for (int e = 0; e < 4; e++) {
        if (g0 + e * NT < ntot) {
          const real2 s1 = cadd(za[e], cconj(zb[e])), d1 = csub(za[e], cconj(zb[e]));
          const real2 tt = cmuli(cmul(w4[e], d1));
          *(real2 *)(FB + (unsigned long long)(unsigned)FROW(kk[e]) * (unsigned)ldf + 2 * (f0 + ff[e])) = mk2((s1.x - tt.x) * sc[e], (s1.y - tt.y) * sc[e]);
        }
      }
      MR_STAMP(8);
    }
  }
  MR_STAMP(6);
  MR_STAMP_END();
}

EMI_KERNEL_MR(4) void k_fft_inv_mr(EmiGeomDev g, FftTabDev T, FftLaunchDev Lc, const GridFld *flds, int nfld, const real_t *FB,
                                                  int ldf, int nproma) {
  EMI_LDS_DECL;
  real2 *a = (real2 *)EMI_LDS_PTR;
  const int bid = (int)xcd_swizzle(EMI_BID, Lc.nblocks, 8);
  const int li = bid / Lc.nchunk;
  const int lat = Lc.lats[li];
  const FftPlanDev &pl = T.plans[T.planid[lat]];
  const int fbk = pl.fbk;
  const int f0 = (bid - li * Lc.nchunk) * fbk;
  const int nfl = (nfld - f0) < fbk ? (nfld - f0) : fbk;
  const int n = pl.n, sz = pl.sz, nmen = g.nmen[lat];
  MrGeom m;
  m.A = pl.fac[0], m.B = pl.fac[1], m.C = pl.fac[2];
  m.P1 = (m.B * m.C) | 1;
  m.fs = m.A * m.P1;
  const real_t racthe = (real_t)g.racthe[lat];
  const real_t adjw = (real_t)(g.rw[lat] / (double)pl.n);
  const int fb0 = g.fbase[lat];
  const int *frow = g.fftrow ? g.fftrow + fb0 : nullptr;
  const real2 *rtw = (const real2 *)T.rtw + pl.rtw_off;
  const real2 *tw1 = (const real2 *)T.ptw + pl.ptw_off[0], *tw2 = (const real2 *)T.ptw + pl.ptw_off[1];
  const long long gp0 = g.gpoff[lat];
  const long long blk0 = gp0 / nproma;
  const unsigned rem0 = (unsigned)(gp0 - blk0 * nproma);
  {
    const int bc = m.B * m.C, pad = (bc > 1) ? m.P1 - bc : 0;
    const unsigned mbc = mr_magic((unsigned)bc);
    const int npair = sz / 2 + 1, ntot = nfl * npair, NT = EMI_NTHREADS;
    const unsigned mnf = mr_magic((unsigned)nfl);
    if (fbk == 1) {
      constexpr unsigned SZ2 = sizeof(real2);
      const GridFld gf = flds[f0];
      const unsigned rowb = (unsigned)ldf * (unsigned)sizeof(real_t);
      const EmiBuf b_fb = emi_buf(FB + (unsigned long long)(unsigned)fb0 * (unsigned)ldf + 2 * gf.src, (unsigned)nmen * rowb + SZ2);
      const EmiBuf b_rtw = emi_buf(rtw, (unsigned)(sz + 1) * SZ2);
      real_t fa, fb;
      fin_factors(gf.mode, racthe, fa, fb);
      const real_t fsc = Lc.adj ? adjw : (real_t)1.0;
      for (unsigned g0 = (unsigned)EMI_TID; g0 < (unsigned)npair; g0 += 4u * (unsigned)NT) {
        real2 xa[4], xb[4], w4[4];
#pragma unroll
        for (int e = 0; e < 4; e++) {
          const unsigned k = g0 + (unsigned)(e * NT), k2 = (unsigned)sz - k;
          if (!frow) {
            xa[e] = emi_buf_ld<real2>(b_fb, k * rowb, 0);
            xb[e] = emi_buf_ld<real2>(b_fb, k2 * rowb, 0);
          } else {
            const unsigned ka = k < (unsigned)nmen ? k : (unsigned)nmen, kb = k2 < (unsigned)nmen ? k2 : (unsigned)nmen;
            const real2 va = fin_raw(FB, frow[ka], ldf, gf.src), vb = fin_raw(FB, frow[kb], ldf, gf.src);
            xa[e] = k <= (unsigned)nmen ? va : mk2(0, 0);
            xb[e] = k2 <= (unsigned)nmen ? vb : mk2(0, 0);
          }
          w4[e] = emi_buf_ld<real2>(b_rtw, k * SZ2, 0);
        }
#pragma unroll
        for (int e = 0; e < 4; e++) {
          const unsigned k = g0 + (unsigned)(e * NT), k2 = (unsigned)sz - k;
          if (k < (unsigned)npair) {
            real2 zk, zk2;
            fin_pair(xa[e], xb[e], k, k2, fa, fb, fsc, cconj(w4[e]), mk2((real_t)1.0, (real_t)0.0), mk2((real_t)1.0, (real_t)0.0), zk, zk2);
            a[k + (pad ? mr_div(k, mbc) * (unsigned)pad : 0u)] = cconj(zk);
            if (k2 != k && k2 < (unsigned)sz) a[k2 + (pad ? mr_div(k2, mbc) * (unsigned)pad : 0u)] = cconj(zk2);
          }
        }
      }
    } else
    for (int g0 = EMI_TID; g0 < ntot; g0 += 4 * NT) {
      real2 xa[4], xb[4], w4[4];
      real_t fa4[4], fb4[4];
      int kk[4], ff[4];
#pragma unroll
      for (int e = 0; e < 4; e++) {
        const int gi = g0 + e * NT;
        if (gi < ntot) {
          const int k = nfl > 1 ? (int)mr_div((unsigned)gi, mnf) : gi, fl = gi - k * nfl, k2 = sz - k;
          const GridFld gf = flds[f0 + fl];
          kk[e] = k, ff[e] = fl;
          xa[e] = (k <= nmen) ? fin_raw(FB, FROW(k), ldf, gf.src) : mk2(0, 0);
          xb[e] = (k2 <= nmen) ? fin_raw(FB, FROW(k2), ldf, gf.src) : mk2(0, 0);
          w4[e] = rtw[k];
          fin_factors(gf.mode, racthe, fa4[e], fb4[e]);
        }
      }
#pragma unroll
      for (int e = 0; e < 4; e++) {
        if (g0 + e * NT < ntot) {
          const int k = kk[e], k2 = sz - k;
          real2 *af = a + (long long)ff[e] * m.fs;
          real2 zk, zk2;
          fin_pair(xa[e], xb[e], (unsigned)k, (unsigned)k2, fa4[e], fb4[e], Lc.adj ? adjw : (real_t)1.0, cconj(w4[e]), mk2((real_t)1.0, (real_t)0.0), mk2((real_t)1.0, (real_t)0.0), zk, zk2);
          af[k + (pad ? (int)mr_div((unsigned)k, mbc) * pad : 0)] = cconj(zk);
          if (k2 != k && k2 < sz) af[k2 + (pad ? (int)mr_div((unsigned)k2, mbc) * pad : 0)] = cconj(zk2);
        }
      }
    }
  }
  EMI_SYNC();
  bool flat = true;
  for (int fl = 0; fl < nfl; fl++) flat = flat && mr_row_flat(flds[f0 + fl], blk0, rem0, nproma, n);
  const int last = m.C > 1 ? 2 : (m.B > 1 ? 1 : 0);
  if (last == 0 && flat)
    mr_pass_any<2>(m.A, a, m.fs, nfl, mr_args(m, 0, tw1, tw2), flds + f0, blk0, rem0, nproma);
  else
    mr_pass_any<0>(m.A, a, m.fs, nfl, mr_args(m, 0, tw1, tw2), flds + f0, blk0, rem0, nproma);
  if (m.B > 1) {
    EMI_SYNC();
    if (last == 1 && flat)
      mr_pass_any<2>(m.B, a, m.fs, nfl, mr_args(m, 1, tw1, tw2), flds + f0, blk0, rem0, nproma);
    else
      mr_pass_any<0>(m.B, a, m.fs, nfl, mr_args(m, 1, tw1, tw2), flds + f0, blk0, rem0, nproma);
  }
  if (m.C > 1) {
    EMI_SYNC();
    if (flat)
      mr_pass_any<2>(m.C, a, m.fs, nfl, mr_args(m, 2, tw1, tw2), flds + f0, blk0, rem0, nproma);
    else
      mr_pass_any<0>(m.C, a, m.fs, nfl, mr_args(m, 2, tw1, tw2), flds + f0, blk0, rem0, nproma);
  }
  if (!flat) {
    EMI_SYNC();
    const unsigned short *perm = T.perm + pl.perm_off;
    for (int fl = 0; fl < nfl; fl++) {
      const GridRow gr = grid_row(flds[f0 + fl], gp0, nproma);
      const real2 *af = a + (long long)fl * m.fs;
      for (int i = EMI_TID; i < sz; i += EMI_NTHREADS) {
        const real2 y = af[perm[i]];
        if (grid_pair_ok(gr, 2u * i)) {
          *(real2 *)grid_ptr(gr, 2u * i) = mk2(y.x, -y.y);
        } else {
          *grid_ptr(gr, 2u * i) = y.x;
          *grid_ptr(gr, 2u * i + 1) = -y.y;
        }
      }
    }
  }
}
```

ectrans_amd/csrc/emi_rt.h:

```cpp
#pragma once
#include <cstddef>
#include <cstdint>
#include <cstdio>
#include <cstdlib>
#include <cstring>
#include <cmath>

#ifndef EMI_CPU_EMU
#include <hip/hip_runtime.h>

#define EMI_KERNEL __global__
#define EMI_KERNEL_LB(T) __global__ __launch_bounds__(T)
#define EMI_KERNEL_FFT(W) __global__ __attribute__((amdgpu_flat_work_group_size(64, 1024), amdgpu_waves_per_eu(W, W)))
#define EMI_KERNEL_MR(W) __global__ __attribute__((amdgpu_flat_work_group_size(64, 256), amdgpu_waves_per_eu(W, W)))
#define EMI_KERNEL_LB2(T, W) __global__ __attribute__((amdgpu_flat_work_group_size(T, T), amdgpu_waves_per_eu(W, W)))
#define EMI_KERNEL_LAM(W) __global__ __attribute__((amdgpu_flat_work_group_size(64, 512), amdgpu_waves_per_eu(W, W)))
#define EMI_DEVFN __device__ __forceinline__
#define EMI_TID ((int)threadIdx.x)
#define EMI_BID ((int)blockIdx.x)
#define EMI_NTHREADS ((int)blockDim.x)
#define EMI_SYNC() __syncthreads()
#define EMI_WAVE_SYNC()                                   \
  do {                                                    \
    __builtin_amdgcn_fence(__ATOMIC_RELEASE, "wavefront"); \
    __builtin_amdgcn_wave_barrier();                      \
    __builtin_amdgcn_fence(__ATOMIC_ACQUIRE, "wavefront"); \
  } while (0)
#define EMI_GLOBAL_AS __attribute__((address_space(1)))
#define EMI_LDS_DECL extern __shared__ __attribute__((aligned(16))) char emi_lds_raw[]
#define EMI_LDS_SYNC() __asm__ volatile("s_waitcnt lgkmcnt(0)\n\ts_barrier" ::: "memory")
#define EMI_WAVE_FENCE() __asm__ volatile("" ::: "memory")
#define EMI_SCHED_FENCE() __builtin_amdgcn_sched_barrier(0)
#define EMI_FP_STRICT() _Pragma("clang fp contract(off)")

struct EmiBuf {
  __amdgpu_buffer_rsrc_t r;
};
typedef int emi_v4i __attribute__((ext_vector_type(4)));
typedef int emi_v2i __attribute__((ext_vector_type(2)));
EMI_DEVFN EmiBuf emi_buf(const void *p, unsigned bytes) {
  EmiBuf b;
  b.r = __builtin_amdgcn_make_buffer_rsrc((void *)p, 0, bytes, 0x00020000);
  return b;
}
EMI_DEVFN EmiBuf emi_buf_all(const void *p) { return emi_buf(p, 0xFFFFFFFCu); }
template <class V>
EMI_DEVFN V emi_buf_ld(const EmiBuf &b, unsigned voff, unsigned soff) {
  static_assert(sizeof(V) == 16 || sizeof(V) == 8, "emi_buf_ld: 8- or 16-byte values");
  if constexpr (sizeof(V) == 16)
    return __builtin_bit_cast(V, __builtin_amdgcn_raw_buffer_load_b128(b.r, voff, soff, 0));
  else
    return __builtin_bit_cast(V, __builtin_amdgcn_raw_buffer_load_b64(b.r, voff, soff, 0));
}
template <class V>
EMI_DEVFN void emi_buf_st(const EmiBuf &b, unsigned voff, unsigned soff, V v) {
  static_assert(sizeof(V) == 16 || sizeof(V) == 8, "emi_buf_st: 8- or 16-byte values");
  if constexpr (sizeof(V) == 16)
    __builtin_amdgcn_raw_buffer_store_b128(__builtin_bit_cast(emi_v4i, v), b.r, voff, soff, 0);
  else
    __builtin_amdgcn_raw_buffer_store_b64(__builtin_bit_cast(emi_v2i, v), b.r, voff, soff, 0);
}
EMI_DEVFN int emi_uniform(int x) { return __builtin_amdgcn_readfirstlane(x); }
EMI_DEVFN const char *emi_uniform_ptr(const void *p) {
  const unsigned long long a = (unsigned long long)p;
  const unsigned lo = __builtin_amdgcn_readfirstlane((unsigned)a), hi = __builtin_amdgcn_readfirstlane((unsigned)(a >> 32));
  return (const char *)(((unsigned long long)hi << 32) | lo);
}
template <class V>
EMI_DEVFN V emi_ld_sv(const char *ubase, unsigned voff) {
  return *(const EMI_GLOBAL_AS V *)((const EMI_GLOBAL_AS char *)ubase + voff);
}
EMI_DEVFN int emi_ld_const(const int *tab, int idx) { return ((const __attribute__((address_space(4))) int *)tab)[idx]; }
#define EMI_PRIO_HI() __builtin_amdgcn_s_setprio(1)
#define EMI_PRIO_LO() __builtin_amdgcn_s_setprio(0)
#define EMI_OPAQUE(x) __asm__ volatile("" : "+v"(x))
#define EMI_LDS_PTR (emi_lds_raw)

typedef double v4d __attribute__((ext_vector_type(4)));
typedef double d2 __attribute__((ext_vector_type(2)));
typedef float v4f __attribute__((ext_vector_type(4)));
typedef float f2 __attribute__((ext_vector_type(2)));

EMI_DEVFN v4d emi_mfma_f64(double a, double b, v4d c) {
  return __builtin_amdgcn_mfma_f64_16x16x4f64(a, b, c, 0, 0, 0);
}
EMI_DEVFN v4f emi_mfma_f32(float a, float b, v4f c) {
  return __builtin_amdgcn_mfma_f32_16x16x4f32(a, b, c, 0, 0, 0);
}

typedef hipStream_t emi_stream_t;

#define EMI_CHECK(expr)                                                                 \
  do {                                                                                  \
    hipError_t e_ = (expr);                                                             \
    if (e_ != hipSuccess) {                                                             \
      emi_set_error("%s failed: %s (%s:%d)", #expr, hipGetErrorString(e_), __FILE__, __LINE__); \
      return -1;                                                                        \
    }                                                                                   \
  } while (0)

#define EMI_LAUNCH(kernel, grid, block, lds, stream, ...) \
  hipLaunchKernelGGL(kernel, dim3((unsigned)(grid)), dim3((unsigned)(block)), (size_t)(lds), (stream), __VA_ARGS__)

#else
#include <omp.h>
#include <vector>

#define EMI_KERNEL
#define EMI_KERNEL_LB(T)
#define EMI_KERNEL_FFT(W)
#define EMI_KERNEL_LB2(T, W)
#define EMI_KERNEL_LAM(W)
#define EMI_KERNEL_MR(W)
#define EMI_DEVFN inline
struct EmuCtx {
  int tid, bid, nthreads;
  char *lds;
  double *sa, *sb;
};
extern thread_local EmuCtx *emu_ctx;
#define EMI_TID (emu_ctx->tid)
#define EMI_BID (emu_ctx->bid)
#define EMI_NTHREADS (emu_ctx->nthreads)
static inline void emu_barrier() {
#pragma omp barrier
}
#define EMI_SYNC() emu_barrier()
#define EMI_WAVE_SYNC() emu_barrier()
#define EMI_LDS_SYNC() emu_barrier()
#define EMI_WAVE_FENCE() emu_barrier()
#define EMI_SCHED_FENCE() ((void)0)
#define EMI_FP_STRICT()
struct EmiBuf {
  const char *p;
  unsigned bytes;
};
inline EmiBuf emi_buf(const void *p, unsigned bytes) { return EmiBuf{(const char *)p, bytes}; }
inline EmiBuf emi_buf_all(const void *p) { return emi_buf(p, 0xFFFFFFFCu); }
template <class V>
inline V emi_buf_ld(const EmiBuf &b, unsigned voff, unsigned soff) {
  V v;
  memset(&v, 0, sizeof(V));
  if ((size_t)voff + sizeof(V) <= b.bytes) memcpy(&v, b.p + voff + soff, sizeof(V));
  return v;
}
template <class V>
inline void emi_buf_st(const EmiBuf &b, unsigned voff, unsigned soff, V v) {
  if ((size_t)voff + sizeof(V) <= b.bytes) memcpy((char *)b.p + voff + soff, &v, sizeof(V));
}
inline int emi_uniform(int x) { return x; }
inline const char *emi_uniform_ptr(const void *p) { return (const char *)p; }
inline int emi_ld_const(const int *tab, int idx) { return tab[idx]; }
template <class V>
inline V emi_ld_sv(const char *ubase, unsigned voff) {
  V v;
  memcpy(&v, ubase + voff, sizeof(V));
  return v;
}
#define EMI_GLOBAL_AS
#define EMI_LDS_DECL
#define EMI_OPAQUE(x) ((void)0)
#define EMI_PRIO_HI() ((void)0)
#define EMI_PRIO_LO() ((void)0)
#define EMI_LDS_PTR (emu_ctx->lds)

typedef double v4d __attribute__((vector_size(32)));
struct __attribute__((aligned(16))) d2 {
  double x, y;
};
struct int2 {
  int x, y;
};
typedef float v4f __attribute__((vector_size(16)));
struct __attribute__((aligned(8))) f2 {
  float x, y;
};

inline v4d emi_mfma_f64(double a, double b, v4d c) {
  EmuCtx *x = emu_ctx;
  int w = x->tid >> 6, l = x->tid & 63;
  x->sa[w * 64 + l] = a;
  x->sb[w * 64 + l] = b;
#pragma omp barrier
  for (int i = 0; i < 4; i++) {
    int row = (l >> 4) + 4 * i, col = l & 15;
    double s = c[i];
    for (int k = 0; k < 4; k++) s += x->sa[w * 64 + k * 16 + row] * x->sb[w * 64 + k * 16 + col];
    c[i] = s;
  }
#pragma omp barrier
  return c;
}
inline v4f emi_mfma_f32(float a, float b, v4f c) {
  EmuCtx *x = emu_ctx;
  int w = x->tid >> 6, l = x->tid & 63;
  x->sa[w * 64 + l] = a;
  x->sb[w * 64 + l] = b;
#pragma omp barrier
  for (int i = 0; i < 4; i++) {
    int row = 4 * (l >> 4) + i, col = l & 15;
    float s = c[i];
    for (int k = 0; k < 4; k++) s = fmaf((float)x->sa[w * 64 + k * 16 + row], (float)x->sb[w * 64 + k * 16 + col], s);
    c[i] = s;
  }
#pragma omp barrier
  return c;
}

typedef void *emi_stream_t;
typedef int hipError_t;
#define hipSuccess 0

template <class F, class... A>
static void emu_launch(F f, long grid, int block, size_t lds, A... a) {
  std::vector<char> sh(lds + 64);
  std::vector<double> sa((block / 64 + 1) * 64), sb((block / 64 + 1) * 64);
  char *ldsp = (char *)(((uintptr_t)sh.data() + 15) & ~(uintptr_t)15);
  for (long b = 0; b < grid; b++) {
#pragma omp parallel num_threads(block)
    {
      EmuCtx c{omp_get_thread_num(), (int)b, block, ldsp, sa.data(), sb.data()};
      emu_ctx = &c;
      f(a...);
    }
  }
}
#define EMI_LAUNCH(kernel, grid, block, lds, stream, ...) emu_launch(kernel, (long)(grid), (int)(block), (size_t)(lds), __VA_ARGS__)
#define EMI_CHECK(expr) \
  do {                  \
    (void)(expr);       \
  } while (0)
#endif

void emi_set_error(const char *fmt, ...);

int emi_dev_malloc(void **p, size_t bytes);
int emi_dev_free(void *p);
int emi_dev_memset(void *p, int v, size_t bytes, emi_stream_t s);
int emi_h2d(void *dst, const void *src, size_t bytes, emi_stream_t s);
int emi_d2h(void *dst, const void *src, size_t bytes, emi_stream_t s);
int emi_d2d(void *dst, const void *src, size_t bytes, emi_stream_t s);
int emi_stream_sync(emi_stream_t s);
int emi_mem_info(size_t *free_b, size_t *total_b);
```

ectrans_amd/csrc/emi_types.h:

```cpp
#pragma once
#include "emi_rt.h"

struct EmiGeomDev {
  int nsmax, nump, nlat, ngptot;
  int m0_wide;
  const int *mval;
  const int *nmen, *gpoff;
  const int *nasm0;
  const int *fbase;
  const int *fftrow;
  const int *lbase;
  const int *legN, *legS;
  const int *wbase;
  const int *wrows;
  const int *rowm;
  const int *ebase;
  const double *eps;
  const double *lapin;
  const double *rw, *racthe;
  const void *P;
  const long long *offS, *offA;
  const int *ldp;
  const void *PT;
  const long long *offTS, *offTA;
  const int *ldk;
  const int *lattile_pref;
  const int *ktile_pref;
  const double *specw;
  const double *llphase;
};

struct Vd2uvDev {
  const int *pairm;
  const int *mval;
  const int *nasm0;
  const int *ebase;
  const double *eps, *lapin;
  int nsmax, nspec2, nfld;
  double rra;
};

struct LegPolDev {
  const double *mu;
  const double *dcl, *ddl;
  const double *zfac;
  const int *blk;
  int ndgnh, nmax;
  int nofloor;
};

enum { SPK_COPY = 0, SPK_U = 1, SPK_V = 2, SPK_NSD = 3, SPK_U_AD = 4, SPK_V_AD = 5 };
struct SpecSrc {
  const void *a, *b;
  int sa, ia, sb, ib;
  int kind, pad_;
};
enum { SPO_COPY = 0, SPO_VOR = 1, SPO_DIV = 2, SPO_VOR_AD = 3, SPO_DIV_AD = 4, SPO_SC_AD = 5 };
struct SpecDst {
  void *dst;
  int stride, idx;
  int kind, src0, src1;
  int src2, src3, src4;
};
struct FuseDst {
  void *dst;
  int stride, idx;
};
struct LamDev {
  int ndgl, yplan;
  int fbk, fs;
  double exwn, eywn;
  const int *kntmp;
  const int *nesm0;
  const int *rowbase;
};
enum { GM_PLAIN = 0, GM_ACOS = 1, GM_EWDER = 2, GM_EWDER_UV = 3 };
struct GridFld {
  void *base;
  int nf_arr, fidx;
  int mode, src;
};

struct FftPlanDev {
  int n;
  int sz;
  int S;
  int cmode;
  int blue;
  int nfac;
  int fac[14];
  int tw_off, perm_off, rtw_off, chirp_off, bhat_off;
  int ptw_off[14];
  int fbk;
  int lds_class;
  int mr;
  int r16;
  int split;
};
struct FftTabDev {
  const void *tw;
  const void *ptw;
  const unsigned short *perm;
  const void *rtw;
  const void *chirp;
  const void *bhat;
  const void *tw256;
  const FftPlanDev *plans;
  const int *planid;
};

struct FftRowDev {
  int lat, planid, n, sz;
  int nmen, fb0, gpoff, chirp_off;
  int rtw_off, bhat_off, ptw_off0;
  int mr_abc;
  double racthe, rw;
};
struct FftLaunchDev {
  const int *lats;
  int nlat;
  int nchunk;
  long long nblocks;
  int adj;
  const FftRowDev *rows;
};


#define LG_THREADS 256
#define LG_BN 128
#define LG_LDA 80
#define LG_LDB 144
#define LG_LDS_BYTES ((2 * 8 * LG_LDA + 2 * 8 * LG_LDB) * 8)
#define LG_LDS_BYTES_DIR (2 * LG_LDS_BYTES)
#define FPAD(i) ((i) ^ (((i) >> 3) & 15))
#define FFT_LDS_ELEMS(S) (((S) + 15) & ~15)
#define EMI_R16_LIST(X) X(8) X(10) X(12) X(16)
#define EMI_R16S_LIST(X) X(10) X(12) X(16)
#ifndef EMI_MR_RADICES
#define EMI_MR_RADICES(X) X(2) X(3) X(4) X(5) X(6) X(7) X(8) X(9) X(10) X(11) X(12) X(13) X(14) X(15) X(16) X(17) X(19) X(23)
#define EMI_MR_RADICES_F32(X) X(18) X(20) X(21)
#endif

#define EMI_HOT_PLAN_LIST(X)          \
  X(1, 2048, 4, 8, 8, 8, 4, 1, 1)     \
  X(2, 2560, 4, 8, 8, 8, 5, 1, 1)     \
  X(4, 4096, 4, 8, 8, 8, 8, 1, 1)     \
  X(7, 1536, 4, 8, 8, 8, 3, 1, 1)     \
  X(8, 1280, 4, 8, 8, 4, 5, 1, 2)     \
  X(9, 6144, 5, 8, 8, 8, 4, 3, 1)     \
  X(10, 7680, 5, 8, 8, 8, 3, 5, 1)    \
  X(11, 8192, 5, 8, 8, 8, 8, 2, 1)    \
  X(12, 10240, 5, 8, 8, 8, 4, 5, 1)   \
  X(13, 1024, 4, 8, 8, 8, 2, 1, 2)    \
  X(14, 960, 4, 8, 8, 3, 5, 1, 2)     \
  X(15, 768, 4, 8, 8, 4, 3, 1, 2)     \
  X(18, 512, 3, 8, 8, 8, 1, 1, 4)     \
  X(20, 320, 3, 8, 8, 5, 1, 1, 8)     \
  X(21, 256, 3, 8, 8, 4, 1, 1, 8)     \
  X(22, 3072, 4, 8, 8, 8, 6, 1, 1)    \
  X(23, 4608, 4, 8, 8, 8, 9, 1, 1)    \
  X(24, 5120, 4, 8, 8, 8, 10, 1, 1)   \
  X(25, 640, 3, 8, 8, 10, 1, 1, 4)    \
  X(26, 576, 3, 8, 8, 9, 1, 1, 4)     \
  X(27, 384, 3, 8, 8, 6, 1, 1, 4)
```

Measured before the change: 3.006.

## Precompute mixed-radix FFT geometry per row and specialize single-field blocks

```diff
diff --git a/ectrans_amd/csrc/ectrans_mi.hip b/ectrans_amd/csrc/ectrans_mi.hip
--- a/ectrans_amd/csrc/ectrans_mi.hip
+++ b/ectrans_amd/csrc/ectrans_mi.hip
@@ -242,6 +242,7 @@
   std::vector<int> lats;
   int *d_lats = nullptr;
   FftRowDev *d_rows = nullptr;
+  MrRowDev *d_mrrows = nullptr;
   size_t lds = 0;
 };
 struct LegMaps {
@@ -725,6 +726,38 @@
   return shared.back();
 }
 
+static unsigned mr_magic(unsigned D) { return D > 1 ? 0xFFFFFFFFu / D + 1u : 0u; }
+static unsigned long long mr_magic64(unsigned d) { return d > 1 ? ~0ull / d + 1ull : 0ull; }
+static void mr_fill_row(MrRowDev &mr, const FftPlanDev &pl, int nthr, double rw) {
+  MrGeomDev &m = mr.m;
+  m.A = pl.fac[0], m.B = pl.fac[1], m.C = pl.fac[2];
+  m.bc = m.B * m.C;
+  m.P1 = m.bc | 1;
+  m.fs = m.A * m.P1;
+  m.fbk = pl.fbk;
+  m.pad = m.P1 - m.bc;
+  m.mbc = mr_magic((unsigned)m.bc), m.mA = mr_magic((unsigned)m.A), m.mAB = mr_magic((unsigned)(m.A * m.B));
+  m.npass = m.C > 1 ? 3 : (m.B > 1 ? 2 : 1);
+  m.perm_off = pl.perm_off;
+  m.nthr = nthr;
+  m.wn = rw / (double)pl.n;
+  for (int ip = 0; ip < 3; ip++) {
+    MrPassDev &pa = mr.p[ip];
+    memset(&pa, 0, sizeof(pa));
+    if (ip == 0) {
+      pa.cnt = m.B * m.C, pa.D = 1, pa.SU = 1, pa.SV = 0, pa.ES = m.P1, pa.tw_off = -1, pa.tw_by_u = 0;
+    } else if (ip == 1) {
+      pa.cnt = m.A * m.C, pa.D = m.C, pa.SU = m.P1, pa.SV = 1, pa.ES = m.C, pa.tw_off = pl.ptw_off[0], pa.tw_by_u = 1;
+    } else {
+      pa.cnt = m.A * m.B, pa.D = m.A, pa.SU = m.C, pa.SV = m.P1, pa.ES = 1, pa.tw_off = pl.ptw_off[1], pa.tw_by_u = 0;
+    }
+    pa.mcnt = mr_magic((unsigned)pa.cnt), pa.mD = mr_magic((unsigned)pa.D);
+    pa.du = nthr / pa.D, pa.dv = nthr % pa.D;
+    pa.st = pa.du * pa.SU + pa.dv * pa.SV;
+    pa.wr = pa.SU - pa.D * pa.SV;
+  }
+}
+
 static int build_fft_plans(Plan &P) {
   const FftSwitches sw;
   std::map<int, int> idx;
@@ -860,6 +893,14 @@
       r.racthe = P.racthe[P.lat0 + j], r.rw = P.rw[P.lat0 + j];
     }
     if (upload(P.dev_allocs, rows, &fc.d_rows)) return EMI_ERR_RUNTIME;
+    if (fc.mr) {
+      std::vector<MrRowDev> mrows(fc.lats.size());
+      for (size_t i = 0; i < fc.lats.size(); i++) {
+        mrows[i].r = rows[i];
+        mr_fill_row(mrows[i], P.fplans[P.planid[fc.lats[i]]], fc.nthr, rows[i].rw);
+      }
+      if (upload(P.dev_allocs, mrows, &fc.d_mrrows)) return EMI_ERR_RUNTIME;
+    }
   }
   return 0;
 }
@@ -2114,10 +2155,20 @@
       continue;
     }
     if (fc.mr) {
-      if (inverse)
-        EMI_LAUNCH_P(P.esz, k_fft_inv_mr, nblocks, nthr, fc.lds, st, P.g, P.ftab, lc, d_flds, nfld, (const RT *)FB, ldf, nproma);
-      else
-        EMI_LAUNCH_P(P.esz, k_fft_dir_mr, nblocks, nthr, fc.lds, st, P.g, P.ftab, lc, d_flds, nfld, (RT *)FB, ldf, nproma);
+      lc.rows = (const FftRowDev *)fc.d_mrrows;
+      const unsigned long long mchunk = mr_magic64((unsigned)nchunk), mnpr = mr_magic64((unsigned)nproma);
+      if (nblocks > 0xFFFFFFFFLL) EMI_FAIL(EMI_ERR_UNSUPPORTED, "internal: %lld workgroups in one FFT launch", nblocks);
+      if (inverse) {
+        if (fc.fbk == 1)
+          EMI_LAUNCH_P(P.esz, k_fft_inv_mr<1>, nblocks, nthr, fc.lds, st, P.g, P.ftab, lc, d_flds, nfld, (const RT *)FB, ldf, nproma, mchunk, mnpr);
+        else
+          EMI_LAUNCH_P(P.esz, k_fft_inv_mr<0>, nblocks, nthr, fc.lds, st, P.g, P.ftab, lc, d_flds, nfld, (const RT *)FB, ldf, nproma, mchunk, mnpr);
+      } else {
+        if (fc.fbk == 1)
+          EMI_LAUNCH_P(P.esz, k_fft_dir_mr<1>, nblocks, nthr, fc.lds, st, P.g, P.ftab, lc, d_flds, nfld, (RT *)FB, ldf, nproma, mchunk, mnpr);
+        else
+          EMI_LAUNCH_P(P.esz, k_fft_dir_mr<0>, nblocks, nthr, fc.lds, st, P.g, P.ftab, lc, d_flds, nfld, (RT *)FB, ldf, nproma, mchunk, mnpr);
+      }
       continue;
     }
     if (fc.r16 && fc.split) {
@@ -2263,10 +2314,14 @@
   EMI_CHECK(hipFuncSetAttribute((const void *)emi_f64::k_fft_dir, hipFuncAttributeMaxDynamicSharedMemorySize, 160 * 1024));
   EMI_CHECK(hipFuncSetAttribute((const void *)emi_f32::k_fft_inv, hipFuncAttributeMaxDynamicSharedMemorySize, 160 * 1024));
   EMI_CHECK(hipFuncSetAttribute((const void *)emi_f32::k_fft_dir, hipFuncAttributeMaxDynamicSharedMemorySize, 160 * 1024));
-  EMI_CHECK(hipFuncSetAttribute((const void *)emi_f64::k_fft_inv_mr, hipFuncAttributeMaxDynamicSharedMemorySize, 160 * 1024));
-  EMI_CHECK(hipFuncSetAttribute((const void *)emi_f64::k_fft_dir_mr, hipFuncAttributeMaxDynamicSharedMemorySize, 160 * 1024));
-  EMI_CHECK(hipFuncSetAttribute((const void *)emi_f32::k_fft_inv_mr, hipFuncAttributeMaxDynamicSharedMemorySize, 160 * 1024));
-  EMI_CHECK(hipFuncSetAttribute((const void *)emi_f32::k_fft_dir_mr, hipFuncAttributeMaxDynamicSharedMemorySize, 160 * 1024));
+#define EMI_MR_ATTR(one_)                                                                                                                    \
+  EMI_CHECK(hipFuncSetAttribute((const void *)emi_f64::k_fft_inv_mr<one_>, hipFuncAttributeMaxDynamicSharedMemorySize, 160 * 1024));  \
+  EMI_CHECK(hipFuncSetAttribute((const void *)emi_f64::k_fft_dir_mr<one_>, hipFuncAttributeMaxDynamicSharedMemorySize, 160 * 1024));  \
+  EMI_CHECK(hipFuncSetAttribute((const void *)emi_f32::k_fft_inv_mr<one_>, hipFuncAttributeMaxDynamicSharedMemorySize, 160 * 1024));  \
+  EMI_CHECK(hipFuncSetAttribute((const void *)emi_f32::k_fft_dir_mr<one_>, hipFuncAttributeMaxDynamicSharedMemorySize, 160 * 1024));
+  EMI_MR_ATTR(0)
+  EMI_MR_ATTR(1)
+#undef EMI_MR_ATTR
 #define EMI_R16_ATTR(r_)                                                                                                                     \
   EMI_CHECK(hipFuncSetAttribute((const void *)emi_f64::k_fft_inv_r16<r_>, hipFuncAttributeMaxDynamicSharedMemorySize, 160 * 1024));  \
   EMI_CHECK(hipFuncSetAttribute((const void *)emi_f64::k_fft_dir_r16<r_>, hipFuncAttributeMaxDynamicSharedMemorySize, 160 * 1024));  \
diff --git a/ectrans_amd/csrc/emi_mr_body.h b/ectrans_amd/csrc/emi_mr_body.h
--- a/ectrans_amd/csrc/emi_mr_body.h
+++ b/ectrans_amd/csrc/emi_mr_body.h
@@ -145,101 +145,163 @@
   }
 };
 
-EMI_DEVFN unsigned mr_magic(unsigned D) { return D > 1 ? 0xFFFFFFFFu / D + 1u : 0u; }
 EMI_DEVFN unsigned mr_div(unsigned j, unsigned m) { return m ? (unsigned)(((unsigned long long)j * m) >> 32) : j; }
-
-struct MrPassArgs {
-  int cnt;
-  unsigned mcnt, mD;
-  int D, SU, SV, ES;
-  const real2 *tw;
-  int tw_by_u;
-};
-
-EMI_DEVFN real_t *mr_row(const GridFld &gf, long long blk0, unsigned rem0, int nproma) {
-  return (real_t *)gf.base + (blk0 * gf.nf_arr + gf.fidx) * (long long)nproma + rem0;
-}
-EMI_DEVFN bool mr_row_flat(const GridFld &gf, long long blk0, unsigned rem0, int nproma, int n) {
+EMI_DEVFN unsigned mr_div64(unsigned x, unsigned long long M) {
+  if (!M) return x;
+  const unsigned long long lo = (unsigned long long)x * (unsigned)M, hi = (unsigned long long)x * (unsigned)(M >> 32);
+  return (unsigned)((hi + (lo >> 32)) >> 32);
+}
+EMI_DEVFN unsigned mr_magic_nf(int nfl) {
+  static constexpr unsigned m[17] = {0u, 0u, 0x80000000u, 0x55555556u, 0x40000000u, 0x33333334u, 0x2AAAAAABu, 0x24924925u, 0x20000000u,
+                                     0x1C71C71Du, 0x1999999Au, 0x1745D175u, 0x15555556u, 0x13B13B14u, 0x12492493u, 0x11111112u, 0x10000000u};
+  return m[nfl];
+}
+
+EMI_DEVFN real_t *mr_row(const GridFld &gf, unsigned blk0, unsigned rem0, int nproma) {
+  return (real_t *)gf.base + ((long long)blk0 * gf.nf_arr + gf.fidx) * (long long)nproma + rem0;
+}
+EMI_DEVFN bool mr_row_flat(const GridFld &gf, unsigned blk0, unsigned rem0, int nproma, int n) {
   return (rem0 + (unsigned)n <= (unsigned)nproma) && ((((uintptr_t)mr_row(gf, blk0, rem0, nproma)) & (2 * sizeof(real_t) - 1)) == 0);
 }
-
-template <int R, int IO>
-EMI_DEVFN void mr_pass(real2 *a, int fs, int nfl, const MrPassArgs &pa, const GridFld *flds, long long blk0, unsigned rem0, int nproma) {
-  const int ntot = nfl * pa.cnt;
-  for (int gi = EMI_TID; gi < ntot; gi += EMI_NTHREADS) {
-    const int f = nfl > 1 ? (int)mr_div((unsigned)gi, pa.mcnt) : 0;
-    const int j = gi - f * pa.cnt;
-    const int u = pa.D > 1 ? (int)mr_div((unsigned)j, pa.mD) : j;
-    const int v = j - u * pa.D;
-    real2 *p = a + (long long)f * fs + u * pa.SU + v * pa.SV;
-    real_t xr[R], xi[R];
-    real2 w = mk2(1, 0);
-    if (IO != 1 && pa.tw) {
-      EMI_GLOBAL_AS const real2 *tw = (EMI_GLOBAL_AS const real2 *)pa.tw + (pa.tw_by_u ? u : j);
-      w = mk2(tw->x, tw->y);
+EMI_DEVFN GridRow mr_grid_row(const GridFld &gf, unsigned blk0, unsigned rem0, int nproma) {
+  GridRow r;
+  r.rem0 = rem0;
+  r.np = (unsigned)nproma;
+  r.bstride = (long long)gf.nf_arr * nproma;
+  r.p0 = (real_t *)gf.base + ((long long)blk0 * gf.nf_arr + gf.fidx) * (long long)nproma;
+  return r;
+}
+EMI_DEVFN real_t *mr_grid_ptr(const GridRow &r, unsigned o, unsigned long long mnpr) {
+  const unsigned q = r.rem0 + o;
+  if (q < r.np) return r.p0 + q;
+  const unsigned b = mr_div64(q, mnpr);
+  return r.p0 + (long long)b * r.bstride + (q - b * r.np);
+}
+
+template <int R>
+EMI_DEVFN void mr_twiddle(real_t *xr, real_t *xi, real2 w) {
+  if constexpr (sizeof(real_t) == 4 && (R > 8)) {
+    real_t qr[4], qi[4];
+    qr[1] = w.x, qi[1] = w.y;
+    mr_for<1, R>([&](auto rc) {
+      constexpr int r = decltype(rc)::value;
+      if constexpr (r == 2) {
+        qr[2] = w.x * w.x - w.y * w.y, qi[2] = 2 * w.x * w.y;
+      } else if constexpr (r == 3) {
+        qr[3] = qr[2] * w.x - qi[2] * w.y, qi[3] = qr[2] * w.y + qi[2] * w.x;
+      } else if constexpr (r == 4) {
+        qr[0] = qr[2] * qr[2] - qi[2] * qi[2], qi[0] = 2 * qr[2] * qi[2];
+        w = mk2(qr[0], qi[0]);
+      } else if constexpr (r > 4) {
+        const real_t t0 = qr[r & 3] * w.x - qi[r & 3] * w.y;
+        qi[r & 3] = qr[r & 3] * w.y + qi[r & 3] * w.x, qr[r & 3] = t0;
+      }
+      const real_t t1 = xr[r] * qr[r & 3] - xi[r] * qi[r & 3];
+      xi[r] = xr[r] * qi[r & 3] + xi[r] * qr[r & 3], xr[r] = t1;
+    });
+  } else {
+    real_t cr = w.x, ci = w.y;
+    mr_for<1, R>([&](auto rc) {
+      constexpr int r = decltype(rc)::value;
+      if constexpr (r > 1) {
+        const real_t t0 = cr * w.x - ci * w.y;
+        ci = cr * w.y + ci * w.x, cr = t0;
+      }
+      const real_t t1 = xr[r] * cr - xi[r] * ci;
+      xi[r] = xr[r] * ci + xi[r] * cr, xr[r] = t1;
+    });
+  }
+}
+
+template <int R, int IO, int ONE>
+EMI_DEVFN void mr_pass(EMI_LDS_AS real2 *a, int fs, int nfl, const MrPassDev &pa, const real2 *ptw, const GridFld *flds, const real_t *row0, unsigned blk0, unsigned rem0,
+                       int nproma) {
+  constexpr unsigned SZ2 = (unsigned)sizeof(real2);
+  const bool has_tw = IO != 1 && pa.tw_off >= 0;
+  if constexpr (ONE) {
+    EMI_LDS_AS char *ab = (EMI_LDS_AS char *)a;
+    const unsigned NT = (unsigned)EMI_NTHREADS, esb = (unsigned)pa.ES * SZ2, cntb = (unsigned)pa.cnt * SZ2;
+    unsigned j = (unsigned)EMI_TID;
+    unsigned u = mr_div(j, pa.mD), v = j - u * (unsigned)pa.D;
+    unsigned offb = (u * (unsigned)pa.SU + v * (unsigned)pa.SV) * SZ2;
+    const unsigned stb = (unsigned)pa.st * SZ2, wrb = (unsigned)pa.wr * SZ2;
+    const EmiBuf b_tw = emi_buf_all(ptw + (has_tw ? pa.tw_off : 0));
+    const EmiBuf b_row = emi_buf_all(row0);
+    for (; j < (unsigned)pa.cnt; j += NT) {
+      real_t xr[R], xi[R];
+      real2 w = mk2(1, 0);
+      if (has_tw) w = emi_buf_ld<real2>(b_tw, (pa.tw_by_u ? u : j) * SZ2, 0);
+      if constexpr (IO == 1) {
+        mr_for<0, R>([&](auto rc) {
+          constexpr int r = decltype(rc)::value;
+          const real2 z = emi_buf_ld<real2>(b_row, j * SZ2, cntb * r);
+          xr[r] = z.x, xi[r] = z.y;
+        });
+      } else {
+        mr_for<0, R>([&](auto rc) {
+          constexpr int r = decltype(rc)::value;
+          const real2 z = *(EMI_LDS_AS const real2 *)(ab + (offb + esb * r));
+          xr[r] = z.x, xi[r] = z.y;
+        });
+      }
+      if (has_tw) mr_twiddle<R>(xr, xi, w);
+      MrDft<R>::run(xr, xi, [&](auto kc, real_t re, real_t im) {
+        constexpr int k = decltype(kc)::value;
+        if constexpr (IO == 2)
+          emi_buf_st<real2>(b_row, j * SZ2 + cntb * k, 0, mk2(re, -im));
+        else
+          *(EMI_LDS_AS real2 *)(ab + (offb + esb * k)) = mk2(re, im);
+      });
+      u += (unsigned)pa.du, v += (unsigned)pa.dv, offb += stb;
+      if (v >= (unsigned)pa.D) u += 1, v -= (unsigned)pa.D, offb += wrb;
     }
-    EMI_GLOBAL_AS real2 *row = nullptr;
-    if constexpr (IO != 0) row = (EMI_GLOBAL_AS real2 *)mr_row(flds[f], blk0, rem0, nproma) + j;
-    if constexpr (IO == 1) {
-      mr_for<0, R>([&](auto rc) {
-        constexpr int r = decltype(rc)::value;
-        xr[r] = row[pa.cnt * r].x, xi[r] = row[pa.cnt * r].y;
-      });
-    } else {
-      mr_for<0, R>([&](auto rc) {
-        constexpr int r = decltype(rc)::value;
-        const real2 z = p[r * pa.ES];
-        xr[r] = z.x, xi[r] = z.y;
+  } else {
+    const int ntot = nfl * pa.cnt;
+    for (int gi = EMI_TID; gi < ntot; gi += EMI_NTHREADS) {
+      const unsigned f = nfl > 1 ? mr_div((unsigned)gi, pa.mcnt) : 0u;
+      const unsigned j = (unsigned)gi - f * (unsigned)pa.cnt;
+      const unsigned u = mr_div(j, pa.mD);
+      const unsigned v = j - u * (unsigned)pa.D;
+      EMI_LDS_AS real2 *p = a + (f * (unsigned)fs + u * (unsigned)pa.SU + v * (unsigned)pa.SV);
+      real_t xr[R], xi[R];
+      real2 w = mk2(1, 0);
+      if (has_tw) {
+        EMI_GLOBAL_AS const real2 *tw = (EMI_GLOBAL_AS const real2 *)ptw + pa.tw_off + (pa.tw_by_u ? u : j);
+        w = mk2(tw->x, tw->y);
+      }
+      EMI_GLOBAL_AS real2 *row = nullptr;
+      if constexpr (IO != 0) row = (EMI_GLOBAL_AS real2 *)mr_row(flds[f], blk0, rem0, nproma) + j;
+      if constexpr (IO == 1) {
+        mr_for<0, R>([&](auto rc) {
+          constexpr int r = decltype(rc)::value;
+          xr[r] = row[pa.cnt * r].x, xi[r] = row[pa.cnt * r].y;
+        });
+      } else {
+        mr_for<0, R>([&](auto rc) {
+          constexpr int r = decltype(rc)::value;
+          const real2 z = p[(unsigned)(r * pa.ES)];
+          xr[r] = z.x, xi[r] = z.y;
+        });
+      }
+      if (has_tw) mr_twiddle<R>(xr, xi, w);
+      MrDft<R>::run(xr, xi, [&](auto kc, real_t re, real_t im) {
+        constexpr int k = decltype(kc)::value;
+        if constexpr (IO == 2)
+          row[pa.cnt * k].x = re, row[pa.cnt * k].y = -im;
+        else
+          p[(unsigned)(k * pa.ES)] = mk2(re, im);
       });
     }
-    if (IO != 1 && pa.tw) {
-      if constexpr (sizeof(real_t) == 4 && (R > 8)) {
-        real_t qr[4], qi[4];
-        qr[1] = w.x, qi[1] = w.y;
-        mr_for<1, R>([&](auto rc) {
-          constexpr int r = decltype(rc)::value;
-          if constexpr (r == 2) {
-            qr[2] = w.x * w.x - w.y * w.y, qi[2] = 2 * w.x * w.y;
-          } else if constexpr (r == 3) {
-            qr[3] = qr[2] * w.x - qi[2] * w.y, qi[3] = qr[2] * w.y + qi[2] * w.x;
-          } else if constexpr (r == 4) {
-            qr[0] = qr[2] * qr[2] - qi[2] * qi[2], qi[0] = 2 * qr[2] * qi[2];
-            w = mk2(qr[0], qi[0]);
-          } else if constexpr (r > 4) {
-            const real_t t0 = qr[r & 3] * w.x - qi[r & 3] * w.y;
-            qi[r & 3] = qr[r & 3] * w.y + qi[r & 3] * w.x, qr[r & 3] = t0;
-          }
-          const real_t t1 = xr[r] * qr[r & 3] - xi[r] * qi[r & 3];
-          xi[r] = xr[r] * qi[r & 3] + xi[r] * qr[r & 3], xr[r] = t1;
-        });
-      } else {
-        real_t cr = w.x, ci = w.y;
-        mr_for<1, R>([&](auto rc) {
-          constexpr int r = decltype(rc)::value;
-          if constexpr (r > 1) {
-            const real_t t0 = cr * w.x - ci * w.y;
-            ci = cr * w.y + ci * w.x, cr = t0;
-          }
-          const real_t t1 = xr[r] * cr - xi[r] * ci;
-          xi[r] = xr[r] * ci + xi[r] * cr, xr[r] = t1;
-        });
-      }
-    }
-    MrDft<R>::run(xr, xi, [&](auto kc, real_t re, real_t im) {
-      constexpr int k = decltype(kc)::value;
-      if constexpr (IO == 2)
-        row[pa.cnt * k].x = re, row[pa.cnt * k].y = -im;
-      else
-        p[k * pa.ES] = mk2(re, im);
-    });
-  }
-}
-
-template <int IO>
-EMI_DEVFN void mr_pass_any(int R, real2 *a, int fs, int nfl, const MrPassArgs &pa, const GridFld *flds, long long blk0, unsigned rem0, int nproma) {
+  }
+}
+
+template <int IO, int ONE>
+EMI_DEVFN void mr_pass_any(int R, EMI_LDS_AS real2 *a, int fs, int nfl, const MrPassDev *pp, const real2 *ptw, const GridFld *flds, const real_t *row0, unsigned blk0,
+                           unsigned rem0, int nproma) {
+  const MrPassDev pa = emi_ld_const_rec(pp);
   switch (R) {
 #define EMI_MR_CASE(r_) \
-  case r_: mr_pass<r_, IO>(a, fs, nfl, pa, flds, blk0, rem0, nproma); break;
+  case r_: mr_pass<r_, IO, ONE>(a, fs, nfl, pa, ptw, flds, row0, blk0, rem0, nproma); break;
     EMI_MR_RADICES(EMI_MR_CASE)
     EMI_MR_EXTRA(EMI_MR_CASE)
 #undef EMI_MR_CASE
@@ -247,168 +309,196 @@
   }
 }
 
-struct MrGeom {
-  int A, B, C, P1, fs;
+EMI_DEVFN real2 mr_fout(real2 za, real2 zb, real2 w, real_t sc) {
+  const real2 s1 = cadd(za, cconj(zb)), d1 = csub(za, cconj(zb));
+  const real2 tt = cmuli(cmul(w, d1));
+  return mk2((s1.x - tt.x) * sc, (s1.y - tt.y) * sc);
+}
+
+struct MrBlock {
+  int li, f0, nfl;
+  unsigned blk0, rem0;
 };
-EMI_DEVFN MrGeom mr_geom(int abc) {
-  MrGeom m;
-  m.A = abc & 255, m.B = (abc >> 8) & 255, m.C = (abc >> 16) & 255;
-  const int bc = m.B * m.C;
-  m.P1 = bc | 1;
-  m.fs = m.A * m.P1;
-  return m;
-}
-EMI_DEVFN MrPassArgs mr_args(const MrGeom &m, int ip, const real2 *tw1, const real2 *tw2) {
-  MrPassArgs pa;
-  if (ip == 0) {
-    pa.cnt = m.B * m.C, pa.D = 1, pa.SU = 1, pa.SV = 0, pa.ES = m.P1, pa.tw = nullptr, pa.tw_by_u = 0;
-  } else if (ip == 1) {
-    pa.cnt = m.A * m.C, pa.D = m.C, pa.SU = m.P1, pa.SV = 1, pa.ES = m.C, pa.tw = tw1, pa.tw_by_u = 1;
+template <int ONE>
+EMI_DEVFN MrBlock mr_block(const FftLaunchDev &Lc, unsigned long long mchunk, int nfld) {
+  MrBlock b;
+  const unsigned bid = (unsigned)xcd_swizzle(EMI_BID, Lc.nblocks, 8);
+  b.li = (int)mr_div64(bid, mchunk);
+  b.f0 = (int)(bid - (unsigned)b.li * (unsigned)Lc.nchunk);
+  b.nfl = 1, b.blk0 = 0, b.rem0 = 0;
+  return b;
+}
+EMI_DEVFN void mr_block_grid(MrBlock &b, unsigned gp0, int n, int nproma, unsigned long long mnpr) {
+  if (gp0 + (unsigned)n <= (unsigned)nproma) {
+    b.blk0 = 0, b.rem0 = gp0;
   } else {
-    pa.cnt = m.A * m.B, pa.D = m.A, pa.SU = m.C, pa.SV = m.P1, pa.ES = 1, pa.tw = tw2, pa.tw_by_u = 0;
-  }
-  pa.mcnt = mr_magic((unsigned)pa.cnt);
-  pa.mD = mr_magic((unsigned)pa.D);
-  return pa;
-}
-
-EMI_KERNEL_MR(4) void k_fft_dir_mr(EmiGeomDev g, FftTabDev T, FftLaunchDev Lc, const GridFld *flds, int nfld, real_t *FB, int ldf,
-                                                  int nproma) {
+    b.blk0 = mr_div64(gp0, mnpr);
+    b.rem0 = gp0 - b.blk0 * (unsigned)nproma;
+  }
+}
+
+template <int ONE>
+EMI_KERNEL_MR(4) void k_fft_dir_mr(EmiGeomDev g, FftTabDev T, FftLaunchDev Lc, const GridFld *flds, int nfld, real_t *FB, int ldf, int nproma,
+                                   unsigned long long mchunk, unsigned long long mnpr) {
   EMI_LDS_DECL;
-  real2 *a = (real2 *)EMI_LDS_PTR;
-  const int bid = (int)xcd_swizzle(EMI_BID, Lc.nblocks, 8);
-  const int li = bid / Lc.nchunk;
-  const FftRowDev rw_ = Lc.rows[li];
-  const FftPlanDev &pl = T.plans[rw_.planid];
-  const int fbk = (int)((unsigned)rw_.mr_abc >> 24);
-  const int f0 = (bid - li * Lc.nchunk) * fbk;
-  const int nfl = (nfld - f0) < fbk ? (nfld - f0) : fbk;
+  EMI_LDS_AS real2 *a = (EMI_LDS_AS real2 *)EMI_LDS_PTR;
+  constexpr unsigned SZ2 = (unsigned)sizeof(real2);
+  MrBlock bk = mr_block<ONE>(Lc, mchunk, nfld);
+  const MrRowDev *rp = (const MrRowDev *)Lc.rows + bk.li;
+  const FftRowDev rw_ = emi_ld_const_rec(&rp->r);
+  const MrGeomDev m = emi_ld_const_rec(&rp->m);
+  const int f0 = ONE ? bk.f0 : bk.f0 * m.fbk;
+  const int nfl = ONE ? 1 : ((nfld - f0) < m.fbk ? (nfld - f0) : m.fbk);
   const int n = rw_.n, sz = rw_.sz, nmen = rw_.nmen;
-  const MrGeom m = mr_geom(rw_.mr_abc);
   const int fb0 = rw_.fb0;
   const int *frow = g.fftrow ? g.fftrow + fb0 : nullptr;
   const real2 *rtw = (const real2 *)T.rtw + rw_.rtw_off;
-  const real2 *tw1 = (const real2 *)T.ptw + rw_.ptw_off0, *tw2 = tw1 + m.A;
-  const long long gp0 = rw_.gpoff;
-  const long long blk0 = gp0 / nproma;
-  const unsigned rem0 = (unsigned)(gp0 - blk0 * nproma);
+  const real2 *ptw = (const real2 *)T.ptw;
+  mr_block_grid(bk, (unsigned)rw_.gpoff, n, nproma, mnpr);
+  const unsigned blk0 = bk.blk0, rem0 = bk.rem0;
+  const GridFld gf0 = emi_ld_const_rec(flds + (ONE ? f0 : 0));
+  const real_t *row0 = mr_row(gf0, blk0, rem0, nproma);
   bool flat = true;
-  for (int fl = 0; fl < nfl; fl++) flat = flat && mr_row_flat(flds[f0 + fl], blk0, rem0, nproma, n);
+  if constexpr (ONE)
+    flat = mr_row_flat(gf0, blk0, rem0, nproma, n);
+  else
+    for (int fl = 0; fl < nfl; fl++) flat = flat && mr_row_flat(flds[f0 + fl], blk0, rem0, nproma, n);
   MR_STAMP_BEGIN();
   if (flat) {
-    mr_pass_any<1>(m.A, a, m.fs, nfl, mr_args(m, 0, tw1, tw2), flds + f0, blk0, rem0, nproma);
+    mr_pass_any<1, ONE>(m.A, a, m.fs, nfl, &rp->p[0], ptw, flds + f0, row0, blk0, rem0, nproma);
     MR_STAMP(0);
   } else {
-    const int bc = m.B * m.C, pad = m.P1 - bc;
-    const unsigned mbc = mr_magic((unsigned)bc);
     for (int fl = 0; fl < nfl; fl++) {
-      const GridRow gr = grid_row(flds[f0 + fl], gp0, nproma);
-      real2 *af = a + (long long)fl * m.fs;
+      const GridRow gr = mr_grid_row(flds[f0 + fl], blk0, rem0, nproma);
+      EMI_LDS_AS real2 *af = a + (unsigned)(fl * m.fs);
       for (int l = EMI_TID; l < sz; l += EMI_NTHREADS) {
         real2 z;
         if (grid_pair_ok(gr, 2u * l)) {
-          z = *(const real2 *)grid_ptr(gr, 2u * l);
+          z = *(const real2 *)mr_grid_ptr(gr, 2u * l, mnpr);
         } else {
-          z.x = *grid_ptr(gr, 2u * l);
-          z.y = *grid_ptr(gr, 2u * l + 1);
-        }
-        af[l + (pad && bc > 1 ? (int)mr_div((unsigned)l, mbc) * pad : 0)] = z;
+          z.x = *mr_grid_ptr(gr, 2u * l, mnpr);
+          z.y = *mr_grid_ptr(gr, 2u * l + 1, mnpr);
+        }
+        af[(unsigned)l + (m.pad ? mr_div((unsigned)l, m.mbc) * (unsigned)m.pad : 0u)] = z;
       }
     }
     EMI_SYNC();
-    mr_pass_any<0>(m.A, a, m.fs, nfl, mr_args(m, 0, tw1, tw2), flds + f0, blk0, rem0, nproma);
+    mr_pass_any<0, ONE>(m.A, a, m.fs, nfl, &rp->p[0], ptw, flds + f0, row0, blk0, rem0, nproma);
   }
   if (m.B > 1) {
     EMI_SYNC();
     MR_STAMP(1);
-    mr_pass_any<0>(m.B, a, m.fs, nfl, mr_args(m, 1, tw1, tw2), flds + f0, blk0, rem0, nproma);
+    mr_pass_any<0, ONE>(m.B, a, m.fs, nfl, &rp->p[1], ptw, flds + f0, row0, blk0, rem0, nproma);
     MR_STAMP(2);
   }
   if (m.C > 1) {
     EMI_SYNC();
     MR_STAMP(3);
-    mr_pass_any<0>(m.C, a, m.fs, nfl, mr_args(m, 2, tw1, tw2), flds + f0, blk0, rem0, nproma);
+    mr_pass_any<0, ONE>(m.C, a, m.fs, nfl, &rp->p[2], ptw, flds + f0, row0, blk0, rem0, nproma);
     MR_STAMP(4);
   }
   EMI_SYNC();
   MR_STAMP(5);
   {
-    const int nk = nmen + 1, ntot = nfl * nk, NT = EMI_NTHREADS;
-    const unsigned mnf = mr_magic((unsigned)nfl), mA = mr_magic((unsigned)m.A), mAB = mr_magic((unsigned)(m.A * m.B));
-    const real_t sc0 = (real_t)0.5 * (Lc.adj ? (real_t)1.0 : (real_t)(rw_.rw / (double)n)), racthe = (real_t)rw_.racthe;
-    auto pos = [&](int k) {
-      const int q1 = m.A > 1 ? (int)mr_div((unsigned)k, mA) : k;
-      const int k3 = (int)mr_div((unsigned)k, mAB);
-      return (k - q1 * m.A) * m.P1 + (q1 - k3 * m.B) * m.C + k3;
+    const int nk = nmen + 1, NT = EMI_NTHREADS;
+    const real_t sc0 = (real_t)0.5 * (Lc.adj ? (real_t)1.0 : (real_t)m.wn), racthe = (real_t)rw_.racthe;
+    auto pos = [&](unsigned k) {
+      const unsigned q1 = mr_div(k, m.mA);
+      const unsigned k3 = mr_div(k, m.mAB);
+      return (k - q1 * (unsigned)m.A) * (unsigned)m.P1 + (q1 - k3 * (unsigned)m.B) * (unsigned)m.C + k3;
     };
-    for (int g0 = EMI_TID; g0 < ntot; g0 += 4 * NT) {
-      real2 za[4], zb[4], w4[4];
-      int kk[4], ff[4];
-      real_t sc[4];
-#pragma unroll
-      for (int e = 0; e < 4; e++) {
-        const int gi = g0 + e * NT;
-        if (gi < ntot) {
-          const int k = nfl > 1 ? (int)mr_div((unsigned)gi, mnf) : gi, fl = gi - k * nfl;
-          const real2 *af = a + (long long)fl * m.fs;
-          kk[e] = k, ff[e] = fl;
-          w4[e] = rtw[k];
-          sc[e] = sc0 * fft_dir_mode_scale(flds[f0 + fl].mode, racthe);
-          za[e] = af[pos(k)], zb[e] = af[pos(k == 0 ? 0 : sz - k)];
-        }
-      }
+    if constexpr (ONE) {
+      const unsigned rowb = (unsigned)ldf * (unsigned)sizeof(real_t);
+      const EmiBuf b_fb = emi_buf(FB + (unsigned long long)(unsigned)fb0 * (unsigned)ldf + 2 * f0, (unsigned)nmen * rowb + SZ2);
+      const EmiBuf b_rtw = emi_buf_all(rtw);
+      const real_t sc = sc0 * fft_dir_mode_scale(gf0.mode, racthe);
+      for (unsigned g0 = (unsigned)EMI_TID; g0 < (unsigned)nk; g0 += 4u * (unsigned)NT) {
+        real2 za[4], zb[4], w4[4];
+#pragma unroll
+        for (int e = 0; e < 4; e++) {
+          const unsigned k = g0 + (unsigned)(e * NT), kc = k < (unsigned)nmen ? k : (unsigned)nmen;
+          w4[e] = emi_buf_ld<real2>(b_rtw, kc * SZ2, 0);
+          za[e] = a[pos(kc)], zb[e] = a[pos(kc == 0 ? 0u : (unsigned)sz - kc)];
+        }
 #if defined(EMI_MR_STAMP) && !defined(EMI_LEG_STAMP) && !defined(EMI_CPU_EMU)
-      if (w4[0].x + za[0].x + zb[0].x + sc[0] == (real_t)1.2345e300) kk[0] = 0;
-      MR_STAMP(7);
+        if (w4[0].x + za[0].x + zb[0].x == (real_t)1.2345e300) w4[0].x = 0;
+        MR_STAMP(7);
 #endif
 #pragma unroll
-      for (int e = 0; e < 4; e++) {
-        if (g0 + e * NT < ntot) {
-          const real2 s1 = cadd(za[e], cconj(zb[e])), d1 = csub(za[e], cconj(zb[e]));
-          const real2 tt = cmuli(cmul(w4[e], d1));
-          *(real2 *)(FB + (unsigned long long)(unsigned)FROW(kk[e]) * (unsigned)ldf + 2 * (f0 + ff[e])) = mk2((s1.x - tt.x) * sc[e], (s1.y - tt.y) * sc[e]);
-        }
-      }
-      MR_STAMP(8);
+        for (int e = 0; e < 4; e++) {
+          const unsigned k = g0 + (unsigned)(e * NT);
+          const real2 x = mr_fout(za[e], zb[e], w4[e], sc);
+          if (!frow)
+            emi_buf_st<real2>(b_fb, k * rowb, 0, x);
+          else if (k < (unsigned)nk)
+            *(real2 *)(FB + (unsigned long long)(unsigned)frow[k] * (unsigned)ldf + 2 * f0) = x;
+        }
+        MR_STAMP(8);
+      }
+    } else {
+      const int ntot = nfl * nk;
+      const unsigned mnf = mr_magic_nf(nfl);
+      for (int g0 = EMI_TID; g0 < ntot; g0 += 4 * NT) {
+        real2 za[4], zb[4], w4[4];
+        int kk[4], ff[4];
+        real_t sc[4];
+#pragma unroll
+        for (int e = 0; e < 4; e++) {
+          const int gi = g0 + e * NT;
+          if (gi < ntot) {
+            const int k = (int)mr_div((unsigned)gi, mnf), fl = gi - k * nfl;
+            EMI_LDS_AS const real2 *af = a + (unsigned)(fl * m.fs);
+            kk[e] = k, ff[e] = fl;
+            w4[e] = rtw[k];
+            sc[e] = sc0 * fft_dir_mode_scale(flds[f0 + fl].mode, racthe);
+            za[e] = af[pos((unsigned)k)], zb[e] = af[pos(k == 0 ? 0u : (unsigned)(sz - k))];
+          }
+        }
+#if defined(EMI_MR_STAMP) && !defined(EMI_LEG_STAMP) && !defined(EMI_CPU_EMU)
+        if (w4[0].x + za[0].x + zb[0].x + sc[0] == (real_t)1.2345e300) kk[0] = 0;
+        MR_STAMP(7);
+#endif
+#pragma unroll
+        for (int e = 0; e < 4; e++) {
+          if (g0 + e * NT < ntot)
+            *(real2 *)(FB + (unsigned long long)(unsigned)FROW(kk[e]) * (unsigned)ldf + 2 * (f0 + ff[e])) = mr_fout(za[e], zb[e], w4[e], sc[e]);
+        }
+        MR_STAMP(8);
+      }
     }
   }
   MR_STAMP(6);
   MR_STAMP_END();
 }
 
-EMI_KERNEL_MR(4) void k_fft_inv_mr(EmiGeomDev g, FftTabDev T, FftLaunchDev Lc, const GridFld *flds, int nfld, const real_t *FB,
-                                                  int ldf, int nproma) {
+template <int ONE>
+EMI_KERNEL_MR(4) void k_fft_inv_mr(EmiGeomDev g, FftTabDev T, FftLaunchDev Lc, const GridFld *flds, int nfld, const real_t *FB, int ldf, int nproma,
+                                   unsigned long long mchunk, unsigned long long mnpr) {
   EMI_LDS_DECL;
-  real2 *a = (real2 *)EMI_LDS_PTR;
-  const int bid = (int)xcd_swizzle(EMI_BID, Lc.nblocks, 8);
-  const int li = bid / Lc.nchunk;
-  const int lat = Lc.lats[li];
-  const FftPlanDev &pl = T.plans[T.planid[lat]];
-  const int fbk = pl.fbk;
-  const int f0 = (bid - li * Lc.nchunk) * fbk;
-  const int nfl = (nfld - f0) < fbk ? (nfld - f0) : fbk;
-  const int n = pl.n, sz = pl.sz, nmen = g.nmen[lat];
-  MrGeom m;
-  m.A = pl.fac[0], m.B = pl.fac[1], m.C = pl.fac[2];
-  m.P1 = (m.B * m.C) | 1;
-  m.fs = m.A * m.P1;
-  const real_t racthe = (real_t)g.racthe[lat];
-  const real_t adjw = (real_t)(g.rw[lat] / (double)pl.n);
-  const int fb0 = g.fbase[lat];
+  EMI_LDS_AS real2 *a = (EMI_LDS_AS real2 *)EMI_LDS_PTR;
+  MrBlock bk = mr_block<ONE>(Lc, mchunk, nfld);
+  const MrRowDev *rp = (const MrRowDev *)Lc.rows + bk.li;
+  const FftRowDev rw_ = emi_ld_const_rec(&rp->r);
+  const MrGeomDev m = emi_ld_const_rec(&rp->m);
+  const int f0 = ONE ? bk.f0 : bk.f0 * m.fbk;
+  const int nfl = ONE ? 1 : ((nfld - f0) < m.fbk ? (nfld - f0) : m.fbk);
+  const int n = rw_.n, sz = rw_.sz, nmen = rw_.nmen;
+  const real_t racthe = (real_t)rw_.racthe;
+  const real_t adjw = (real_t)m.wn;
+  const int fb0 = rw_.fb0;
   const int *frow = g.fftrow ? g.fftrow + fb0 : nullptr;
-  const real2 *rtw = (const real2 *)T.rtw + pl.rtw_off;
-  const real2 *tw1 = (const real2 *)T.ptw + pl.ptw_off[0], *tw2 = (const real2 *)T.ptw + pl.ptw_off[1];
-  const long long gp0 = g.gpoff[lat];
-  const long long blk0 = gp0 / nproma;
-  const unsigned rem0 = (unsigned)(gp0 - blk0 * nproma);
+  const real2 *rtw = (const real2 *)T.rtw + rw_.rtw_off;
+  const real2 *ptw = (const real2 *)T.ptw;
+  mr_block_grid(bk, (unsigned)rw_.gpoff, n, nproma, mnpr);
+  const unsigned blk0 = bk.blk0, rem0 = bk.rem0;
+  const GridFld gf0 = emi_ld_const_rec(flds + (ONE ? f0 : 0));
+  const real_t *row0 = mr_row(gf0, blk0, rem0, nproma);
   {
-    const int bc = m.B * m.C, pad = (bc > 1) ? m.P1 - bc : 0;
-    const unsigned mbc = mr_magic((unsigned)bc);
-    const int npair = sz / 2 + 1, ntot = nfl * npair, NT = EMI_NTHREADS;
-    const unsigned mnf = mr_magic((unsigned)nfl);
-    if (fbk == 1) {
+    const unsigned pad = (unsigned)m.pad, mbc = m.mbc;
+    const int npair = sz / 2 + 1, NT = EMI_NTHREADS;
+    if constexpr (ONE) {
       constexpr unsigned SZ2 = sizeof(real2);
-      const GridFld gf = flds[f0];
+      const GridFld gf = gf0;
       const unsigned rowb = (unsigned)ldf * (unsigned)sizeof(real_t);
       const EmiBuf b_fb = emi_buf(FB + (unsigned long long)(unsigned)fb0 * (unsigned)ldf + 2 * gf.src, (unsigned)nmen * rowb + SZ2);
       const EmiBuf b_rtw = emi_buf(rtw, (unsigned)(sz + 1) * SZ2);
@@ -437,77 +527,83 @@
           if (k < (unsigned)npair) {
             real2 zk, zk2;
             fin_pair(xa[e], xb[e], k, k2, fa, fb, fsc, cconj(w4[e]), mk2((real_t)1.0, (real_t)0.0), mk2((real_t)1.0, (real_t)0.0), zk, zk2);
-            a[k + (pad ? mr_div(k, mbc) * (unsigned)pad : 0u)] = cconj(zk);
-            if (k2 != k && k2 < (unsigned)sz) a[k2 + (pad ? mr_div(k2, mbc) * (unsigned)pad : 0u)] = cconj(zk2);
+            a[k + (pad ? mr_div(k, mbc) * pad : 0u)] = cconj(zk);
+            if (k2 != k && k2 < (unsigned)sz) a[k2 + (pad ? mr_div(k2, mbc) * pad : 0u)] = cconj(zk2);
           }
         }
       }
-    } else
-    for (int g0 = EMI_TID; g0 < ntot; g0 += 4 * NT) {
-      real2 xa[4], xb[4], w4[4];
-      real_t fa4[4], fb4[4];
-      int kk[4], ff[4];
-#pragma unroll
-      for (int e = 0; e < 4; e++) {
-        const int gi = g0 + e * NT;
-        if (gi < ntot) {
-          const int k = nfl > 1 ? (int)mr_div((unsigned)gi, mnf) : gi, fl = gi - k * nfl, k2 = sz - k;
-          const GridFld gf = flds[f0 + fl];
-          kk[e] = k, ff[e] = fl;
-          xa[e] = (k <= nmen) ? fin_raw(FB, FROW(k), ldf, gf.src) : mk2(0, 0);
-          xb[e] = (k2 <= nmen) ? fin_raw(FB, FROW(k2), ldf, gf.src) : mk2(0, 0);
-          w4[e] = rtw[k];
-          fin_factors(gf.mode, racthe, fa4[e], fb4[e]);
-        }
-      }
-#pragma unroll
-      for (int e = 0; e < 4; e++) {
-        if (g0 + e * NT < ntot) {
-          const int k = kk[e], k2 = sz - k;
-          real2 *af = a + (long long)ff[e] * m.fs;
-          real2 zk, zk2;
-          fin_pair(xa[e], xb[e], (unsigned)k, (unsigned)k2, fa4[e], fb4[e], Lc.adj ? adjw : (real_t)1.0, cconj(w4[e]), mk2((real_t)1.0, (real_t)0.0), mk2((real_t)1.0, (real_t)0.0), zk, zk2);
-          af[k + (pad ? (int)mr_div((unsigned)k, mbc) * pad : 0)] = cconj(zk);
-          if (k2 != k && k2 < sz) af[k2 + (pad ? (int)mr_div((unsigned)k2, mbc) * pad : 0)] = cconj(zk2);
+    } else {
+      const int ntot = nfl * npair;
+      const unsigned mnf = mr_magic_nf(nfl);
+      for (int g0 = EMI_TID; g0 < ntot; g0 += 4 * NT) {
+        real2 xa[4], xb[4], w4[4];
+        real_t fa4[4], fb4[4];
+        int kk[4], ff[4];
+#pragma unroll
+        for (int e = 0; e < 4; e++) {
+          const int gi = g0 + e * NT;
+          if (gi < ntot) {
+            const int k = (int)mr_div((unsigned)gi, mnf), fl = gi - k * nfl, k2 = sz - k;
+            const GridFld gf = flds[f0 + fl];
+            kk[e] = k, ff[e] = fl;
+            xa[e] = (k <= nmen) ? fin_raw(FB, FROW(k), ldf, gf.src) : mk2(0, 0);
+            xb[e] = (k2 <= nmen) ? fin_raw(FB, FROW(k2), ldf, gf.src) : mk2(0, 0);
+            w4[e] = rtw[k];
+            fin_factors(gf.mode, racthe, fa4[e], fb4[e]);
+          }
+        }
+#pragma unroll
+        for (int e = 0; e < 4; e++) {
+          if (g0 + e * NT < ntot) {
+            const unsigned k = (unsigned)kk[e], k2 = (unsigned)sz - k;
+            EMI_LDS_AS real2 *af = a + (unsigned)(ff[e] * m.fs);
+            real2 zk, zk2;
+            fin_pair(xa[e], xb[e], k, k2, fa4[e], fb4[e], Lc.adj ? adjw : (real_t)1.0, cconj(w4[e]), mk2((real_t)1.0, (real_t)0.0), mk2((real_t)1.0, (real_t)0.0), zk, zk2);
+            af[k + (pad ? mr_div(k, mbc) * pad : 0u)] = cconj(zk);
+            if (k2 != k && k2 < (unsigned)sz) af[k2 + (pad ? mr_div(k2, mbc) * pad : 0u)] = cconj(zk2);
+          }
         }
       }
     }
   }
   EMI_SYNC();
   bool flat = true;
-  for (int fl = 0; fl < nfl; fl++) flat = flat && mr_row_flat(flds[f0 + fl], blk0, rem0, nproma, n);
-  const int last = m.C > 1 ? 2 : (m.B > 1 ? 1 : 0);
+  if constexpr (ONE)
+    flat = mr_row_flat(gf0, blk0, rem0, nproma, n);
+  else
+    for (int fl = 0; fl < nfl; fl++) flat = flat && mr_row_flat(flds[f0 + fl], blk0, rem0, nproma, n);
+  const int last = m.npass - 1;
   if (last == 0 && flat)
-    mr_pass_any<2>(m.A, a, m.fs, nfl, mr_args(m, 0, tw1, tw2), flds + f0, blk0, rem0, nproma);
+    mr_pass_any<2, ONE>(m.A, a, m.fs, nfl, &rp->p[0], ptw, flds + f0, row0, blk0, rem0, nproma);
   else
-    mr_pass_any<0>(m.A, a, m.fs, nfl, mr_args(m, 0, tw1, tw2), flds + f0, blk0, rem0, nproma);
+    mr_pass_any<0, ONE>(m.A, a, m.fs, nfl, &rp->p[0], ptw, flds + f0, row0, blk0, rem0, nproma);
   if (m.B > 1) {
     EMI_SYNC();
     if (last == 1 && flat)
-      mr_pass_any<2>(m.B, a, m.fs, nfl, mr_args(m, 1, tw1, tw2), flds + f0, blk0, rem0, nproma);
+      mr_pass_any<2, ONE>(m.B, a, m.fs, nfl, &rp->p[1], ptw, flds + f0, row0, blk0, rem0, nproma);
     else
-      mr_pass_any<0>(m.B, a, m.fs, nfl, mr_args(m, 1, tw1, tw2), flds + f0, blk0, rem0, nproma);
+      mr_pass_any<0, ONE>(m.B, a, m.fs, nfl, &rp->p[1], ptw, flds + f0, row0, blk0, rem0, nproma);
   }
   if (m.C > 1) {
     EMI_SYNC();
     if (flat)
-      mr_pass_any<2>(m.C, a, m.fs, nfl, mr_args(m, 2, tw1, tw2), flds + f0, blk0, rem0, nproma);
+      mr_pass_any<2, ONE>(m.C, a, m.fs, nfl, &rp->p[2], ptw, flds + f0, row0, blk0, rem0, nproma);
     else
-      mr_pass_any<0>(m.C, a, m.fs, nfl, mr_args(m, 2, tw1, tw2), flds + f0, blk0, rem0, nproma);
+      mr_pass_any<0, ONE>(m.C, a, m.fs, nfl, &rp->p[2], ptw, flds + f0, row0, blk0, rem0, nproma);
   }
   if (!flat) {
     EMI_SYNC();
-    const unsigned short *perm = T.perm + pl.perm_off;
+    const unsigned short *perm = T.perm + m.perm_off;
     for (int fl = 0; fl < nfl; fl++) {
-      const GridRow gr = grid_row(flds[f0 + fl], gp0, nproma);
-      const real2 *af = a + (long long)fl * m.fs;
+      const GridRow gr = mr_grid_row(flds[f0 + fl], blk0, rem0, nproma);
+      EMI_LDS_AS const real2 *af = a + (unsigned)(fl * m.fs);
       for (int i = EMI_TID; i < sz; i += EMI_NTHREADS) {
         const real2 y = af[perm[i]];
         if (grid_pair_ok(gr, 2u * i)) {
-          *(real2 *)grid_ptr(gr, 2u * i) = mk2(y.x, -y.y);
+          *(real2 *)mr_grid_ptr(gr, 2u * i, mnpr) = mk2(y.x, -y.y);
         } else {
-          *grid_ptr(gr, 2u * i) = y.x;
-          *grid_ptr(gr, 2u * i + 1) = -y.y;
+          *mr_grid_ptr(gr, 2u * i, mnpr) = y.x;
+          *mr_grid_ptr(gr, 2u * i + 1, mnpr) = -y.y;
         }
       }
     }
diff --git a/ectrans_amd/csrc/emi_rt.h b/ectrans_amd/csrc/emi_rt.h
--- a/ectrans_amd/csrc/emi_rt.h
+++ b/ectrans_amd/csrc/emi_rt.h
@@ -27,6 +27,7 @@
     __builtin_amdgcn_fence(__ATOMIC_ACQUIRE, "wavefront"); \
   } while (0)
 #define EMI_GLOBAL_AS __attribute__((address_space(1)))
+#define EMI_LDS_AS __attribute__((address_space(3)))
 #define EMI_LDS_DECL extern __shared__ __attribute__((aligned(16))) char emi_lds_raw[]
 #define EMI_LDS_SYNC() __asm__ volatile("s_waitcnt lgkmcnt(0)\n\ts_barrier" ::: "memory")
 #define EMI_WAVE_FENCE() __asm__ volatile("" ::: "memory")
@@ -71,6 +72,17 @@
   return *(const EMI_GLOBAL_AS V *)((const EMI_GLOBAL_AS char *)ubase + voff);
 }
 EMI_DEVFN int emi_ld_const(const int *tab, int idx) { return ((const __attribute__((address_space(4))) int *)tab)[idx]; }
+template <class T>
+EMI_DEVFN T emi_ld_const_rec(const T *p) {
+  static_assert(sizeof(T) % 4 == 0, "emi_ld_const_rec: records of 4-byte words");
+  struct W {
+    int w[sizeof(T) / 4];
+  } t;
+  const __attribute__((address_space(4))) int *q = (const __attribute__((address_space(4))) int *)p;
+#pragma unroll
+  for (unsigned i = 0; i < sizeof(T) / 4; i++) t.w[i] = q[i];
+  return __builtin_bit_cast(T, t);
+}
 #define EMI_PRIO_HI() __builtin_amdgcn_s_setprio(1)
 #define EMI_PRIO_LO() __builtin_amdgcn_s_setprio(0)
 #define EMI_OPAQUE(x) __asm__ volatile("" : "+v"(x))
@@ -151,6 +163,10 @@
 inline int emi_uniform(int x) { return x; }
 inline const char *emi_uniform_ptr(const void *p) { return (const char *)p; }
 inline int emi_ld_const(const int *tab, int idx) { return tab[idx]; }
+template <class T>
+inline T emi_ld_const_rec(const T *p) {
+  return *p;
+}
 template <class V>
 inline V emi_ld_sv(const char *ubase, unsigned voff) {
   V v;
@@ -158,6 +174,7 @@
   return v;
 }
 #define EMI_GLOBAL_AS
+#define EMI_LDS_AS
 #define EMI_LDS_DECL
 #define EMI_OPAQUE(x) ((void)0)
 #define EMI_PRIO_HI() ((void)0)
diff --git a/ectrans_amd/csrc/emi_types.h b/ectrans_amd/csrc/emi_types.h
--- a/ectrans_amd/csrc/emi_types.h
+++ b/ectrans_amd/csrc/emi_types.h
@@ -116,6 +116,31 @@
   int mr_abc;
   double racthe, rw;
 };
+struct MrPassDev {
+  int cnt, D;
+  unsigned mcnt, mD;
+  int SU, SV, ES;
+  int du, dv;
+  int st, wr;
+  int tw_off;
+  int tw_by_u;
+  int pad_[3];
+};
+struct MrGeomDev {
+  int A, B, C, P1;
+  int fs, fbk;
+  int bc, pad;
+  unsigned mbc, mA, mAB;
+  int npass;
+  int perm_off, nthr;
+  double wn;
+};
+struct MrRowDev {
+  FftRowDev r;
+  MrGeomDev m;
+  MrPassDev p[3];
+};
+static_assert(sizeof(MrPassDev) == 64 && sizeof(MrGeomDev) == 64 && sizeof(MrRowDev) == 320, "MrRowDev layout");
 struct FftLaunchDev {
   const int *lats;
   int nlat;
```

New measurement: 3.013 (median of 4 runs). About the same (+0.2%).
